# luigifreda/plvs

Measured on AMD Instinct MI355X. Metric: Mvoxels/sec TSDF integrate (chisel 5 cm / 5 m, 640x480 RGB-D), higher is better.
Workload: dtype f32; 1 GPU; configs[2] stand-in, STREAMING: see DESIGN.md 4.1 / 4.6; mode=order-free (fixed-point sums; sdf / weight within tolerance), longest_voxel_run=25008, parallelism=chunk-hash shard x1

## Files before the change

include/plvs_hip.h:

```cpp
#ifndef PLVS_HIP_H_
#define PLVS_HIP_H_

#include <stddef.h>
#include <stdint.h>

#ifdef __cplusplus
extern "C" {
#endif

#define PLVS_OK 0
#define PLVS_ERR_INVALID_ARG (-1)
#define PLVS_ERR_HIP (-2)
#define PLVS_ERR_NO_DEVICE (-3)
#define PLVS_ERR_CAPACITY (-4)
#define PLVS_ERR_EMPTY (-5)
#define PLVS_ERR_HALO (-6)
#define PLVS_ERR_COMM_FATAL (-7)

const char* plvs_hip_last_error(void);
int plvs_hip_abi_version(void);
int plvs_hip_device_count(int* count);
int plvs_hip_set_device(int device);
int plvs_hip_synchronize(void);
int plvs_hip_release_thread_buffers(void);
// ... 227 lines not shown
  float dist[8];
  int32_t ndist;
  float mbf;
  float bounds4[4];
  float grid_w_inv, grid_h_inv;
  float min_line_length_3d;
  int32_t use_median_depth;
  float median_fallback;
} plvs_rgbd_calib;
typedef struct plvs_rgbd_frame {
  int32_t kp_cap, line_cap;
  plvs_keypoint* kps;
  plvs_keypoint* kps_un;
  uint8_t* desc;
  float* u_right;
  float* depth;
  int32_t* cell_start;
  int32_t* cell_items;
  plvs_keyline* keylines;
  plvs_keyline* keylines_un;
  uint8_t* line_desc;
  float* u_right_start;
  float* depth_start;
  float* u_right_end;
  float* depth_end;
  int32_t n_kp, mono_index, n_lines, n_items;
  float median_depth;
} plvs_rgbd_frame;
int plvs_hip_frame_rgbd_dev(plvs_orb* orb, plvs_lines* lines, const uint8_t* d_image, int w, int hh, int stride, const float* d_depth,
                            int depth_pitch, const plvs_rgbd_calib* calib, plvs_rgbd_frame* frame, void* stream);

int plvs_hip_frame_compute_stereo_line_matches(const plvs_keyline* keylines_un, const uint8_t* desc, int n,
                                               const plvs_keyline* keylines_right_un, const uint8_t* desc_right, int n_right,
                                               const float* line_level_sigma2, int n_levels, const float* K4, float mbf,
                                               float line_stereo_max_dist, float min_line_length_3d, float nn_ratio,
                                               int check_orientation, int descriptor_dist, float* u_right_start, float* depth_start,
                                               float* u_right_end, float* depth_end, int* n_stereo, void* stream);
int plvs_hip_frame_compute_stereo_line_matches_debug(const plvs_keyline* keylines_un, const uint8_t* desc, int n,
                                                     const plvs_keyline* keylines_right_un, const uint8_t* desc_right, int n_right,
                                                     const float* line_level_sigma2, int n_levels, const float* K4, float mbf,
                                                     float line_stereo_max_dist, float min_line_length_3d, float nn_ratio,
                                                     int check_orientation, int descriptor_dist, float* u_right_start,
                                                     float* depth_start, float* u_right_end, float* depth_end, int* n_stereo,
                                                     int32_t* holders4, void* stream);

struct plvs_stereo;
typedef struct plvs_stereo_calib {
  float K4[4];
  float dist[8];
  int32_t ndist;
  float mbf;
  float bounds4[4];
  float grid_w_inv, grid_h_inv;
  float min_line_length_3d;
  float line_stereo_max_dist;
  float nn_ratio;
  int32_t check_orientation;
  int32_t descriptor_dist;
  int32_t n_line_levels;
  const float* line_level_sigma2;
} plvs_stereo_calib;
typedef struct plvs_stereo_frame {
  int32_t kp_cap, kp_right_cap, line_cap, line_right_cap;
  plvs_keypoint* kps;
  plvs_keypoint* kps_un;
  uint8_t* desc;
  float* u_right;
  float* depth;
  int32_t* cell_start;
  int32_t* cell_items;
  plvs_keypoint* kps_right;
  uint8_t* desc_right;
  plvs_keyline* keylines;
  plvs_keyline* keylines_un;
  uint8_t* line_desc;
  float* u_right_start;
  float* depth_start;
  float* u_right_end;
  float* depth_end;
  plvs_keyline* keylines_right;
  plvs_keyline* keylines_right_un;
  uint8_t* line_desc_right;
  int32_t n_kp, mono_index, n_kp_right, mono_index_right, n_lines, n_lines_right, n_items;
  int32_t n_stereo_points, n_stereo_lines;
} plvs_stereo_frame;
int plvs_hip_frame_stereo_dev(plvs_orb* orb_left, plvs_orb* orb_right, plvs_lines* lines_left, plvs_lines* lines_right,
                              struct plvs_stereo* stereo, const uint8_t* d_left, const uint8_t* d_right, int w, int hh, int stride,
                              const plvs_stereo_calib* calib, plvs_stereo_frame* frame, void* stream);

int plvs_hip_selftest_rcp(int exponent, uint32_t* mismatches);
int plvs_hip_selftest_walk_math(uint32_t seed, uint32_t* mismatches_sqrt_div);
int plvs_hip_selftest_radix_sort(uint32_t n, int bit_lo, int bit_hi, int wide_values, uint32_t seed, uint32_t* mismatches2);

typedef struct plvs_tsdf_chisel_params {
  float resolution;
  float trunc_quad;
  float trunc_linear;
  float trunc_const;
  float trunc_scale;
  float weight;
  int32_t max_chunks;
  int32_t shard_rank;
  int32_t shard_count;
  int32_t order_free;
} plvs_tsdf_chisel_params;

typedef struct plvs_tsdf_chisel plvs_tsdf_chisel;

int plvs_hip_tsdf_chisel_default_params(float resolution, plvs_tsdf_chisel_params* p);
int plvs_hip_tsdf_chisel_create(const plvs_tsdf_chisel_params* p, plvs_tsdf_chisel** out);
int plvs_hip_tsdf_chisel_destroy(plvs_tsdf_chisel* h);
int plvs_hip_tsdf_chisel_clear(plvs_tsdf_chisel* h);

int plvs_hip_tsdf_chisel_integrate(plvs_tsdf_chisel* h, const float* xyz, const uint8_t* rgb,
                                   const uint32_t* kfid, int n, const float* Twc);

int plvs_hip_tsdf_chisel_queue(plvs_tsdf_chisel* h, const float* xyz, const uint8_t* rgb, const uint32_t* kfid, int n,
                               const float* Twc);
int plvs_hip_tsdf_chisel_flush(plvs_tsdf_chisel* h);
int plvs_hip_tsdf_chisel_queued(plvs_tsdf_chisel* h, int* nclouds);
int plvs_hip_tsdf_chisel_integrate_batch_dev(plvs_tsdf_chisel* h, const float* d_xyz,
                                             const uint8_t* d_rgb, const uint32_t* d_kfid,
                                             const int32_t* offsets, int nclouds,
                                             const float* d_Twc, void* stream);

typedef struct plvs_depth_batch {
  const float* d_depth;
  const uint8_t* d_bgr;
  size_t depth_image_stride, bgr_image_stride;
  int depth_pitch, bgr_pitch;
  int width, height, step;
  const float* d_grid_points;
  double min_depth, max_depth;
  const uint32_t* d_kfid;
} plvs_depth_batch;
int plvs_hip_tsdf_chisel_integrate_depth_batch_dev(plvs_tsdf_chisel* h, const plvs_depth_batch* in, int nclouds,
                                                   const float* d_Twc, void* stream);

int plvs_hip_tsdf_chisel_integrate_world_normals(plvs_tsdf_chisel* h, const float* xyz, const uint8_t* rgb,
                                                 const uint32_t* kfid, const float* normals, int n, const float* Twc);
int plvs_hip_tsdf_chisel_integrate_world_normals_dev(plvs_tsdf_chisel* h, const float* d_xyz, const uint8_t* d_rgb,
                                                     const uint32_t* d_kfid, const float* d_normals, int n,
                                                     const float* d_Twc, void* stream);

typedef struct plvs_tsdf_stats {
  int64_t visits;
  int64_t points;
  int32_t new_chunks;
  int32_t updated_chunks;
  int32_t voxels;
  int32_t max_run;
} plvs_tsdf_stats;
int plvs_hip_tsdf_chisel_last_stats(plvs_tsdf_chisel* h, plvs_tsdf_stats* s);

int plvs_hip_tsdf_chisel_set_apply_parts(plvs_tsdf_chisel* h, int part_segments, int min_segments);

int plvs_hip_tsdf_chisel_set_profiling(plvs_tsdf_chisel* h, int enable);
int plvs_hip_tsdf_chisel_stage_ms(plvs_tsdf_chisel* h, double* ms, int cap, int* nstages,
                                  int64_t* calls);
const char* plvs_hip_tsdf_chisel_stage_name(int i);
const char* plvs_hip_tsdf_chisel_stage_name_of(plvs_tsdf_chisel* h, int i);

int plvs_hip_tsdf_chisel_num_chunks(plvs_tsdf_chisel* h, int* n);
int plvs_hip_tsdf_chisel_chunk_ids(plvs_tsdf_chisel* h, int32_t* ids_xyz, int cap, int* n);
int plvs_hip_tsdf_chisel_updated_chunk_ids(plvs_tsdf_chisel* h, int32_t* ids_xyz, int cap, int* n);
int plvs_hip_tsdf_chisel_updated_chunk_ids_dev(plvs_tsdf_chisel* h, int32_t* d_ids_xyz, int cap,
                                               int* n, void* stream);
int plvs_hip_tsdf_chisel_download_chunk(plvs_tsdf_chisel* h, int cx, int cy, int cz, float* sdf,
                                        float* weight, uint32_t* kfid, uint32_t* rgbw);

int plvs_hip_tsdf_chisel_carve(plvs_tsdf_chisel* h, const float* depth, int width, int height, float fx,
                               float fy, float cx, float cy, float near_dist, float far_dist,
                               const float* Twc, float carving_dist, int* carved_chunks);
int plvs_hip_tsdf_chisel_carve_dev(plvs_tsdf_chisel* h, const float* d_depth, int width, int height,
                                   float fx, float fy, float cx, float cy, float near_dist,
                                   float far_dist, const float* Twc, float carving_dist, void* stream,
                                   int* carved_chunks);

int plvs_hip_tsdf_chisel_shard_walk(plvs_tsdf_chisel* h, const float* d_xyz, const int32_t* offsets, int nclouds,
                                    const float* d_Twc, int64_t* send_counts, void* stream);
int plvs_hip_tsdf_chisel_shard_pack(plvs_tsdf_chisel* h, void* d_seg_dst, void* d_rec_dst, void* d_run_dst,
                                    void* stream);
int plvs_hip_tsdf_chisel_shard_apply(plvs_tsdf_chisel* h, const void* d_seg_src, const void* d_rec_src,
                                     const void* d_run_src, const int64_t* recv_counts, const uint8_t* d_rgb,
                                     const uint32_t* d_kfid, void* stream);
int plvs_hip_tsdf_chisel_shard_saturated(plvs_tsdf_chisel* h, int32_t* d_voxels, int cap, int* n, void* stream);
int plvs_hip_tsdf_chisel_shard_note_saturated(plvs_tsdf_chisel* h, const int32_t* d_voxels, int n, void* stream);
int plvs_hip_tsdf_chisel_shard_saturated_message(plvs_tsdf_chisel* h, int32_t* d_msg, int rows, void* stream);
int plvs_hip_tsdf_chisel_shard_note_gathered(plvs_tsdf_chisel* h, const int32_t* d_gathered, int nranks, int rows,
                                             void* stream);
int plvs_hip_tsdf_chisel_integrate_sharded(plvs_tsdf_chisel* h, void* rccl_comm, const float* d_xyz,
                                           const uint8_t* d_rgb, const uint32_t* d_kfid, const int32_t* offsets,
                                           int nclouds, const float* d_Twc, void* stream);
int plvs_hip_exchange_abort_on_fatal(int enable);

int plvs_hip_tsdf_exchange_block_lists(void* rccl_comm, const int32_t* d_local_ids, int local_count, int cap,
                                       int32_t* d_all_ids, int32_t* d_all_counts, void* stream);
int plvs_hip_rccl_world_size(void* rccl_comm, int* world);
typedef struct plvs_block_directory plvs_block_directory;
int plvs_hip_block_directory_create(int max_blocks, plvs_block_directory** out);
int plvs_hip_block_directory_destroy(plvs_block_directory* d);
int plvs_hip_block_directory_merge(plvs_block_directory* d, const int32_t* d_all_ids, const int32_t* d_counts, int world,
                                   int cap, void* stream);
int plvs_hip_block_directory_count(plvs_block_directory* d, int* n);
int plvs_hip_block_directory_list(plvs_block_directory* d, int32_t* ids_xyz, int32_t* owners, int cap, int* n);

typedef struct plvs_stereo plvs_stereo;
int plvs_hip_stereo_create(plvs_orb* left, plvs_orb* right, plvs_stereo** out);
int plvs_hip_stereo_destroy(plvs_stereo* s);
int plvs_hip_stereo_matches(plvs_stereo* s, const plvs_keypoint* keys_left, const uint8_t* desc_left,
                            int n_left, const plvs_keypoint* keys_right, const uint8_t* desc_right,
                            int n_right, float mb, float mbf, float* u_right, float* depth,
                            int* n_matched);

int plvs_hip_tsdf_chisel_mesh_chunks(plvs_tsdf_chisel* h, const int32_t* chunk_ids_xyz, int nchunks,
                                     float* vertices, float* normals, float* colors, uint32_t* kfids,
                                     int capacity, int32_t* chunk_first, int* nvertices);

typedef struct plvs_tsdf_deform_stats {
  int32_t new_chunks;
  int64_t moved;
  int64_t discarded;
  int64_t undefined;
} plvs_tsdf_deform_stats;
int plvs_hip_tsdf_chisel_enable_deform(plvs_tsdf_chisel* h);
int plvs_hip_tsdf_chisel_deform(plvs_tsdf_chisel* h, const uint32_t* kfids, const float* Rt, int n_map,
                                plvs_tsdf_deform_stats* stats);
int plvs_hip_tsdf_chisel_chunk_order(plvs_tsdf_chisel* h, int32_t* ids_xyz, int cap, int* n);
int plvs_hip_tsdf_chisel_deform_mesh(float* vertices, float* normals, const uint32_t* vertex_kfid, int n,
                                     const uint32_t* kfids, const float* Rt, int n_map);
int plvs_hip_tsdf_chisel_deform_mesh_dev(float* d_vertices, float* d_normals, const uint32_t* d_vertex_kfid, int n,
                                         const uint32_t* d_kfids, const float* d_Rt, int n_map, void* stream);

int plvs_hip_tsdf_chisel_upload_chunk(plvs_tsdf_chisel* h, int cx, int cy, int cz, const float* sdf, const float* weight,
                                      const uint32_t* kfid, const uint32_t* rgbw);

int plvs_hip_tsdf_chisel_mesh_probe(plvs_tsdf_chisel* h, const int32_t* chunk_ids_xyz, int nchunks, int* nmissing);
int plvs_hip_tsdf_chisel_halo_gather(plvs_tsdf_chisel* h, void* rccl_comm, const int32_t* chunk_ids_xyz, int nchunks,
                                     int* fetched, void* stream);
int plvs_hip_tsdf_chisel_halo_missing(plvs_tsdf_chisel* h, int32_t* ids_xyz, int cap, int* n);
int plvs_hip_tsdf_chisel_halo_lookup(plvs_tsdf_chisel* h, const int32_t* d_ids_xyz, int n, uint32_t* d_found, void* stream);
int plvs_hip_tsdf_chisel_halo_export(plvs_tsdf_chisel* h, const int32_t* d_ids_xyz, const uint32_t* d_found, int n,
                                     uint32_t* d_payload, void* stream);
int plvs_hip_tsdf_chisel_halo_import(plvs_tsdf_chisel* h, const int32_t* d_ids_xyz, const uint32_t* d_found,
                                     const uint32_t* d_payload, int n, int nfound, void* stream);
int plvs_hip_tsdf_chisel_halo_clear(plvs_tsdf_chisel* h);

typedef struct plvs_elas plvs_elas;
typedef struct {
  int32_t subsampling;
  int32_t grid_size;
  int32_t match_texture;
  float beta;
  float gamma;
  float sigma;
  float sradius;
  int32_t disp_min, disp_max;
  int32_t candidate_stepsize;
  int32_t support_texture;
  int32_t lr_threshold;
  float support_threshold;
  float speckle_sim_threshold;
  int32_t speckle_size;
  int32_t ipol_gap_width;
  int32_t add_corners;
} plvs_elas_params;
int plvs_hip_elas_create(const plvs_elas_params* params, plvs_elas** out);
int plvs_hip_elas_destroy(plvs_elas* e);
int plvs_hip_elas_compute_disparity(plvs_elas* e, const int32_t* support, int n_support, const void* tri, int n_tri,
                                    const int32_t* disparity_grid, const int32_t* grid_dims, const uint8_t* I1_desc,
                                    const uint8_t* I2_desc, int width, int height, int right_image, float* D);
int plvs_hip_elas_adaptive_mean(plvs_elas* e, float* D, int width, int height);
int plvs_hip_elas_support_candidates(plvs_elas* e, const uint8_t* I1_desc, const uint8_t* I2_desc, int width, int height,
                                     int16_t* D_can);
int plvs_hip_elas_set_images(plvs_elas* e, const uint8_t* I1, const uint8_t* I2, int width, int height, int stride);
int plvs_hip_elas_download_descriptors(plvs_elas* e, uint8_t* I1_desc, uint8_t* I2_desc);
int plvs_hip_elas_left_right_check(plvs_elas* e, float* D1, float* D2, int width, int height);
int plvs_hip_elas_remove_small_segments(plvs_elas* e, float* D, int width, int height);
int plvs_hip_elas_gap_interpolation(plvs_elas* e, float* D, int width, int height);
int plvs_hip_elas_postprocess(plvs_elas* e, int width, int height, int postprocess_only_left, int filter_adaptive_mean,
                              float* D1, float* D2);
int plvs_hip_elas_depth_dev(plvs_elas* e, float bf, int step, float* d_depth, int width, int height, void* stream);
int plvs_hip_elas_triangulate(const int32_t* support, int n_support, int right_image, void* tri, int cap, int* n_tri);
int plvs_hip_elas_process(plvs_elas* e, const uint8_t* I1, const uint8_t* I2, const int32_t* dims, int postprocess_only_left,
                          int filter_adaptive_mean, float* D1, float* D2);
int plvs_hip_elas_support_points(plvs_elas* e, const int16_t* D_can, int width, int height, int32_t* support, int cap,
                                 int* n_support);
int plvs_hip_elas_disparity_planes(plvs_elas* e, const int32_t* support, int n_support, void* tri, int n_tri);
int plvs_hip_elas_create_grid(plvs_elas* e, const int32_t* support, int n_support, int width, int height, int right_image,
                              int32_t* disparity_grid, int32_t* grid_dims);

typedef struct plvs_sgm plvs_sgm;
int plvs_hip_sgm_create(int width, int height, int disparity_size, int p1, int p2, float uniqueness,
                        plvs_sgm** out);
int plvs_hip_sgm_destroy(plvs_sgm* s);
int plvs_hip_sgm_execute(plvs_sgm* s, const uint8_t* left, const uint8_t* right, uint8_t* disparity);
int plvs_hip_sgm_execute_dev(plvs_sgm* s, const uint8_t* d_left, const uint8_t* d_right,
                             uint8_t* d_disparity, void* stream);
int plvs_hip_sgm_download(plvs_sgm* s, int which, void* out);


typedef struct plvs_point_surfel {
  float x, y, z;
  uint32_t kfid;
  float normal_x, normal_y, normal_z, normal_pad;
  uint8_t b, g, r, a;
// ... 273 lines not shown
```

plvs_amd/csrc/tsdf_chisel.hip:

```cpp
#include "tsdf_chisel_handle.hpp"
#include "tsdf_chisel_halo.hpp"
#include "tsdf_chisel_ordered.hpp"
#include "tsdf_chisel_order_free.hpp"
#include "tsdf_chisel_carve.hpp"
#include "tsdf_chisel_shard.hpp"
#include "tsdf_chisel_deform.hpp"
#include "tsdf_chisel_scan.hpp"

namespace {

__global__ void pool_init(float* __restrict__ sdf, size_t n) {
  const size_t i = (size_t)blockIdx.x * blockDim.x + threadIdx.x;
  const size_t stride = (size_t)gridDim.x * blockDim.x;
  for (size_t j = i; j < n; j += stride) sdf[j] = 99999.0f;
}

__global__ void selftest_sort_fill(uint32_t* __restrict__ keys, uint32_t* __restrict__ v32, unsigned long long* __restrict__ v64,
                                   uint32_t n, int bits, uint32_t seed) {
  const uint32_t i = blockIdx.x * blockDim.x + threadIdx.x;
  if (i >= n) return;
  uint32_t x = (i + 1u) * 2654435761u + seed;
  x ^= x << 13; x ^= x >> 17; x ^= x << 5;
  x ^= x << 13; x ^= x >> 17; x ^= x << 5;
  keys[i] = bits >= 32 ? x : (x & ((1u << bits) - 1u));
  if (v32) v32[i] = i;
  if (v64) v64[i] = ((unsigned long long)~i << 32) | i;
}
__global__ void selftest_sort_check(const uint32_t* __restrict__ keys_in, const uint32_t* __restrict__ keys,
                                    const uint32_t* __restrict__ v32, const unsigned long long* __restrict__ v64, uint32_t n,
                                    int bit_lo, int bit_hi, uint32_t* __restrict__ mismatches) {
  const uint32_t i = blockIdx.x * blockDim.x + threadIdx.x;
  if (i >= n) return;
  const uint32_t mask = (bit_hi - bit_lo >= 32 ? 0xFFFFFFFFu : ((1u << (bit_hi - bit_lo)) - 1u)) << bit_lo;
  const uint32_t pos = v32 ? v32[i] : (uint32_t)v64[i];
  if (pos >= n || keys_in[pos] != keys[i] || (v64 && (uint32_t)(v64[i] >> 32) != ~pos)) atomicAdd(&mismatches[1], 1u);
  if (i + 1 < n) {
    const uint32_t a = keys[i] & mask, b = keys[i + 1] & mask;
    const uint32_t pn = v32 ? v32[i + 1] : (uint32_t)v64[i + 1];
    if (a > b || (a == b && pos >= pn)) atomicAdd(&mismatches[0], 1u);
  }
}

__global__ void selftest_rcp_kernel(int exponent, uint32_t* __restrict__ mismatches) {
  const uint32_t m = blockIdx.x * blockDim.x + threadIdx.x;
  const float b = __uint_as_float(((uint32_t)(exponent + 127) << 23) | m);
  if (__float_as_uint(rcp_rn(b)) != __float_as_uint(1.0f / b)) atomicAdd(mismatches, 1u);
}

}

__global__ __launch_bounds__(256) void grid_cloud_mark(GridSrc g, int nclouds, uint32_t* __restrict__ flag) {
  const size_t i = (size_t)blockIdx.x * 256 + threadIdx.x, ngrid = (size_t)g.gw * g.gh;
  if (i >= ngrid * (size_t)nclouds) return;
  const uint32_t c = (uint32_t)(i / ngrid), r = (uint32_t)(i - (size_t)c * ngrid), m = r / g.gw, n = r - m * g.gw;
  const float d = g.depth[(size_t)c * g.image_stride + (size_t)(m * g.step) * g.pitch + n * g.step];
  flag[i] = (((double)d > g.min_depth) && ((double)d < g.max_depth)) ? 1u : 0u;
}
__global__ __launch_bounds__(256) void grid_cloud_emit(GridSrc g, int nclouds, const uint32_t* __restrict__ pos ,
                                                       const uint8_t* __restrict__ bgr, const uint32_t* __restrict__ kfid_of_image,
                                                       float* __restrict__ xyz, uint8_t* __restrict__ rgb,
                                                       uint32_t* __restrict__ kfid, uint32_t* __restrict__ offsets) {
  const size_t i = (size_t)blockIdx.x * 256 + threadIdx.x, ngrid = (size_t)g.gw * g.gh, cells = ngrid * (size_t)nclouds;
  if (i > cells) return;
  if (i == cells || i % ngrid == 0) offsets[i / ngrid] = pos[i];
  if (i == cells || pos[i + 1] == pos[i]) return;
  const uint32_t c = (uint32_t)(i / ngrid), r = (uint32_t)(i - (size_t)c * ngrid), m = r / g.gw, n = r - m * g.gw;
  const float d = g.depth[(size_t)c * g.image_stride + (size_t)(m * g.step) * g.pitch + n * g.step];
  const float2 cam = reinterpret_cast<const float2*>(g.cam)[r];
  const size_t o = pos[i];
  xyz[3 * o] = cam.x * d;
  xyz[3 * o + 1] = cam.y * d;
  xyz[3 * o + 2] = d;
  const uint8_t* px = bgr + (size_t)c * g.bgr_image_stride + (size_t)(m * g.step) * g.bgr_pitch + (size_t)(n * g.step) * 3u;
  rgb[3 * o] = px[0];
  rgb[3 * o + 1] = px[1];
  rgb[3 * o + 2] = px[2];
  kfid[o] = kfid_of_image ? kfid_of_image[c] : 0u;
}

extern "C" {

int plvs_hip_selftest_rcp(int exponent, uint32_t* mismatches) {
  PLVS_REQUIRE(mismatches && exponent > -126 && exponent < 127, "bad argument");
  uint32_t* d = nullptr;
  PLVS_HIP_TRY(hipMalloc((void**)&d, sizeof(uint32_t)));
  PLVS_HIP_TRY(hipMemset(d, 0, sizeof(uint32_t)));
  hipLaunchKernelGGL(selftest_rcp_kernel, dim3((1u << 23) / 256), dim3(256), 0, nullptr, exponent, d);
  hipError_t e = hipMemcpy(mismatches, d, sizeof(uint32_t), hipMemcpyDeviceToHost);
  (void)hipFree(d);
  PLVS_HIP_TRY(e);
  return PLVS_OK;
}

int plvs_hip_selftest_radix_sort(uint32_t n, int bit_lo, int bit_hi, int wide_values, uint32_t seed, uint32_t* mismatches2) {
  PLVS_REQUIRE(mismatches2 && n > 0 && bit_lo >= 0 && bit_hi > bit_lo && bit_hi <= 32, "bad argument");
  plvs::DevBuf<uint32_t> k_in, k0, k1, v0, v1, scratch, bad;
  plvs::DevBuf<unsigned long long> w0, w1;
  const bool bound_mode = wide_values == 2;
  if (bound_mode) wide_values = 0;
  const uint32_t n_alloc = bound_mode ? n + n / 2 + 4097u : n;
  PLVS_HIP_TRY(k_in.reserve(n_alloc));
  PLVS_HIP_TRY(k0.reserve(n_alloc));
  PLVS_HIP_TRY(k1.reserve(n_alloc));
  if (wide_values) {
    PLVS_HIP_TRY(w0.reserve(n));
    PLVS_HIP_TRY(w1.reserve(n));
  } else {
    PLVS_HIP_TRY(v0.reserve(n_alloc));
    PLVS_HIP_TRY(v1.reserve(n_alloc));
  }
  PLVS_HIP_TRY(scratch.reserve(radix_scratch_words(n_alloc) + 1));
  PLVS_HIP_TRY(bad.reserve(2));
  PLVS_HIP_TRY(hipMemset(bad.p, 0, 2 * sizeof(uint32_t)));
  const dim3 grid(ceil_div((size_t)n, 256)), block(256);
  hipLaunchKernelGGL(selftest_sort_fill, grid, block, 0, nullptr, k0.p, v0.p, w0.p, n, bit_hi, seed);
  PLVS_HIP_TRY(hipMemcpyAsync(k_in.p, k0.p, (size_t)n * sizeof(uint32_t), hipMemcpyDeviceToDevice, nullptr));
  bool second = false;
  if (bound_mode) {
    PLVS_HIP_TRY(hipMemsetAsync(k0.p + n, 0x5A, (size_t)(n_alloc - n) * sizeof(uint32_t), nullptr));
    uint32_t* d_n = scratch.p + radix_scratch_words(n_alloc);
    PLVS_HIP_TRY(hipMemcpyAsync(d_n, &n, sizeof(uint32_t), hipMemcpyHostToDevice, nullptr));
    PLVS_HIP_TRY(hipStreamSynchronize(nullptr));
    PLVS_HIP_TRY(radix_sort_pairs_bound(k0.p, v0.p, k1.p, v1.p, n_alloc, d_n, bit_lo, bit_hi, scratch.p, nullptr, &second));
  } else if (wide_values) PLVS_HIP_TRY(radix_sort_pairs_u64(k0.p, w0.p, k1.p, w1.p, n, bit_lo, bit_hi, scratch.p, nullptr, &second));
  else PLVS_HIP_TRY(radix_sort_pairs(k0.p, v0.p, k1.p, v1.p, n, bit_lo, bit_hi, scratch.p, nullptr, &second));
  hipLaunchKernelGGL(selftest_sort_check, grid, block, 0, nullptr, k_in.p, second ? k1.p : k0.p,
                     wide_values ? (const uint32_t*)nullptr : (second ? v1.p : v0.p),
                     wide_values ? (second ? w1.p : w0.p) : (const unsigned long long*)nullptr, n, bit_lo, bit_hi, bad.p);
  hipError_t e = hipMemcpy(mismatches2, bad.p, 2 * sizeof(uint32_t), hipMemcpyDeviceToHost);
  k_in.release(); k0.release(); k1.release(); v0.release(); v1.release(); w0.release(); w1.release(); scratch.release(); bad.release();
  PLVS_HIP_TRY(e);
  return PLVS_OK;
}

#ifdef PLVS_WALK_PROF
int plvs_hip_debug_walk_prof(unsigned long long* out16, int reset) {
  if (out16) PLVS_HIP_TRY(hipMemcpyFromSymbol(out16, HIP_SYMBOL(g_walk_prof), 16 * sizeof(unsigned long long)));
  if (reset) {
    unsigned long long z[16] = {};
    PLVS_HIP_TRY(hipMemcpyToSymbol(HIP_SYMBOL(g_walk_prof), z, sizeof z));
  }
  return PLVS_OK;
}
#endif

int plvs_hip_selftest_walk_math(uint32_t seed, uint32_t* mismatches_sqrt_div) {
  PLVS_REQUIRE(mismatches_sqrt_div, "null argument");
  uint32_t* d = nullptr;
  PLVS_HIP_TRY(hipMalloc((void**)&d, 2 * sizeof(uint32_t)));
  PLVS_HIP_TRY(hipMemset(d, 0, 2 * sizeof(uint32_t)));
  hipLaunchKernelGGL(selftest_walk_math_kernel, dim3(16384), dim3(256), 0, nullptr, seed, d);
  hipError_t e = hipMemcpy(mismatches_sqrt_div, d, 2 * sizeof(uint32_t), hipMemcpyDeviceToHost);
  (void)hipFree(d);
  PLVS_HIP_TRY(e);
  return PLVS_OK;
}

int plvs_hip_tsdf_chisel_default_params(float resolution, plvs_tsdf_chisel_params* p) {
  PLVS_REQUIRE(p, "params is null");
  PLVS_REQUIRE(resolution > 0.0f, "resolution must be positive");
  p->resolution = resolution;
  p->trunc_quad = 0.0019f;
  p->trunc_linear = -0.00152f;
  p->trunc_const = 0.001504f;
  p->trunc_scale = 6.0f;
  p->weight = 1.0f;
  p->max_chunks = 32768;
  p->shard_rank = 0;
  p->shard_count = 1;
  p->order_free = 0;
  return PLVS_OK;
}

int plvs_hip_tsdf_chisel_create(const plvs_tsdf_chisel_params* p, plvs_tsdf_chisel** out) {
  PLVS_REQUIRE(p && out, "null argument");
  PLVS_REQUIRE(p->resolution > 0.0f, "resolution must be positive");
  PLVS_REQUIRE(p->max_chunks > 0 && p->max_chunks <= (1 << 20), "max_chunks must be in (0, 2^20]");
  PLVS_REQUIRE(p->shard_count <= 1 || (p->shard_rank >= 0 && p->shard_rank < p->shard_count),
               "shard_rank out of range");
  plvs_tsdf_chisel* h = new plvs_tsdf_chisel();
  h->prm = *p;
  Params& P = h->P;
  P.resolution = p->resolution;
  P.round_to_voxel = 1.0f / p->resolution;
  P.half_voxel = p->resolution * 0.5f;
  P.rounding = 1.0f / ((float)16 * p->resolution);
  P.diag = (float)(2.0 * std::sqrt((double)3.0f) * (double)p->resolution);
  P.tq = p->trunc_quad; P.tl = p->trunc_linear; P.tc = p->trunc_const; P.ts = p->trunc_scale;
  P.weight = p->weight;
  P.shard_rank = p->shard_rank;
  P.shard_count = p->shard_count < 1 ? 1 : p->shard_count;

  uint32_t cap = 1024;
  while (cap < 2u * (uint32_t)p->max_chunks) cap <<= 1;
  h->dir.mask = cap - 1;
  h->dir.max_blocks = p->max_chunks;
  const size_t nvox = (size_t)p->max_chunks * kChunkVox;
#define CREATE_TRY(call)                                                        \
  do {                                                                          \
    hipError_t _e = (call);                                                     \
    if (_e != hipSuccess) {                                                     \
      plvs::set_error("%s failed: %s", #call, hipGetErrorString(_e));          \
      plvs_hip_tsdf_chisel_destroy(h);                                          \
      return PLVS_ERR_HIP;                                                      \
    }                                                                           \
  } while (0)
  CREATE_TRY(hipMalloc((void**)&h->dir.keys, (size_t)cap * sizeof(unsigned long long)));
  CREATE_TRY(hipMalloc((void**)&h->dir.slots, (size_t)cap * sizeof(int32_t)));
  CREATE_TRY(hipMalloc((void**)&h->dir.slot_ids, (size_t)p->max_chunks * 3 * sizeof(int32_t)));
  CREATE_TRY(hipMalloc((void**)&h->sdf, nvox * sizeof(float)));
  CREATE_TRY(hipMalloc((void**)&h->weight, nvox * sizeof(float)));
  CREATE_TRY(hipMalloc((void**)&h->kfid, nvox * sizeof(uint32_t)));
  CREATE_TRY(hipMalloc((void**)&h->rgbw, nvox * sizeof(uint32_t)));
  CREATE_TRY(hipMalloc((void**)&h->d_ctr, sizeof(Counters)));
  CREATE_TRY(hipHostMalloc((void**)&h->h_ctr, sizeof(Counters), hipHostMallocCoherent));
  CREATE_TRY(hipMalloc((void**)&h->d_wctr, 2 * sizeof(WalkCounters)));
  CREATE_TRY(hipHostMalloc((void**)&h->h_wctr, 2 * sizeof(WalkCounters), hipHostMallocCoherent));
  CREATE_TRY(hipHostMalloc((void**)&h->h_seq, 64, hipHostMallocCoherent));
  h->h_seq[0] = 0u;
  {
    const double wu_max = (double)p->weight / (2.0 * (double)P.diag), wuu_max = 0.5 * (double)p->weight;
    h->scale_u = (float)std::exp2(std::floor(std::log2(1073741824.0 / (kWalkRays * wuu_max))));
    h->scale_w = (float)std::exp2(std::floor(std::log2(1073741824.0 / (kWalkRays * wu_max))));
  }
  {
    int least = 0, greatest = 0;
    CREATE_TRY(hipDeviceGetStreamPriorityRange(&least, &greatest));
    CREATE_TRY(hipStreamCreateWithPriority(&h->side, hipStreamNonBlocking, greatest));
  }
  CREATE_TRY(hipEventCreateWithFlags(&h->ev_fork, hipEventDisableTiming));
  CREATE_TRY(hipEventCreateWithFlags(&h->ev_join, hipEventDisableTiming));
  CREATE_TRY(hipEventCreateWithFlags(&h->ev_seg, hipEventDisableTiming));
  CREATE_TRY(hipEventCreateWithFlags(&h->ev_zero, hipEventDisableTiming));
#undef CREATE_TRY
  *out = h;
  int rc = plvs_hip_tsdf_chisel_clear(h);
  if (rc != PLVS_OK) {
    plvs_hip_tsdf_chisel_destroy(h);
    *out = nullptr;
  }
  return rc;
}

int plvs_hip_tsdf_chisel_destroy(plvs_tsdf_chisel* h) {
  if (!h) return PLVS_OK;
  if (h->ext != nullptr && h->ext_free != nullptr) h->ext_free(h->ext);
  deform_state_free(h);
  (void)hipFree(h->dir.keys);
  (void)hipFree(h->dir.slots);
  (void)hipFree(h->dir.slot_ids);
  (void)hipFree(h->sdf);
  (void)hipFree(h->weight);
  (void)hipFree(h->kfid);
  (void)hipFree(h->rgbw);
  (void)hipFree(h->d_ctr);
  if (h->h_ctr) (void)hipHostFree(h->h_ctr);
  (void)hipFree(h->d_wctr);
  if (h->h_wctr) (void)hipHostFree(h->h_wctr);
  if (h->h_seq) (void)hipHostFree(h->h_seq);
  if (h->h_offsets) (void)hipHostFree(h->h_offsets);
  (void)hipFree(h->gdir.keys);
  (void)hipFree(h->gdir.slots);
  (void)hipFree(h->miss_keys);
  (void)hipFree(h->miss_ids);
  (void)hipFree(h->miss_count);
  (void)hipFree(h->xdir.keys);
  (void)hipFree(h->xdir.slots);
  (void)hipFree(h->xdir.slot_ids);
  (void)hipFree(h->d_xcount);
  (void)hipFree(h->x_sat);
  if (h->h_sh_counts) (void)hipHostFree(h->h_sh_counts);
  if (h->h_sh_ctl) (void)hipHostFree(h->h_sh_ctl);
  if (h->h_sh_off) (void)hipHostFree(h->h_sh_off);
  h->q_xyz.release(); h->q_rgb.release(); h->q_kfid.release();
  h->w_rec.release(); h->w_seg.release(); h->w_sorted_seg.release(); h->w_seg_ticket.release(); h->w_chunk_nseg.release();
  h->w_chunk_off.release(); h->w_chunk_fill.release(); h->w_active_off.release(); h->w_masks.release();
  h->w_dummy.release(); h->w_runkey.release(); h->w_run_cnt.release(); h->w_run_off.release(); h->w_val0.release();
  h->w_val1.release(); h->w_seg_cnt.release(); h->w_tile_visits.release(); h->w_deferred.release(); h->w_part_off.release(); h->w_multi_idx.release();
  h->pa_wuu.release(); h->pa_w.release(); h->pa_last.release(); h->pa_cnt.release(); h->pa_done.release();
  h->sh_nrec.release(); h->sh_owner.release(); h->halo_row.release();
  h->sh_ctl.release(); h->sh_seg_reg.release(); h->sh_rec_reg.release(); h->sh_src_off.release(); h->sh_slot_owner.release(); h->sh_run_ctr.release(); h->sh_vkey.release(); h->sh_sat.release(); h->sh_wait.release(); h->sh_run_first.release();
  if (h->ev_fork) (void)hipEventDestroy(h->ev_fork);
  if (h->ev_join) (void)hipEventDestroy(h->ev_join);
  if (h->ev_seg) (void)hipEventDestroy(h->ev_seg);
  if (h->ev_zero) (void)hipEventDestroy(h->ev_zero);
  h->w_rseg.release(); h->w_rpre.release(); h->w_run_matrix.release(); h->w_active_idx.release(); h->w_item_base.release();
  h->w_item_cnt.release(); h->w_item_part0.release(); h->w_part_item.release(); h->w_phist.release();
  h->w_row_heads.release(); h->w_row_tot.release();
  if (h->side) (void)hipStreamDestroy(h->side);
  for (int i = 0; i <= kNumStages; ++i)
    if (h->ev[i]) (void)hipEventDestroy(h->ev[i]);
  h->counts.release();
  h->rec.release(); h->rec_t.release(); h->recc_t.release();
  h->dkey0.release(); h->dkey1.release(); h->didx0.release(); h->didx1.release();
  h->last_pt.release(); h->run_cnt.release(); h->run_dst.release();
  h->tile_first.release(); h->block_first.release(); h->tile_state.release();
  h->heads.release(); h->updated.release(); h->scratch.release(); h->poses.release();
  h->offsets.release(); h->st_xyz.release(); h->st_Twc.release(); h->st_nrm.release(); h->st_rgb.release();
  h->st_kfid.release();
  h->st_pos.release(); h->st_scan.release(); h->st_off.release();
  delete h;
  return PLVS_OK;
}

int plvs_hip_tsdf_chisel_clear(plvs_tsdf_chisel* h) {
  if (h) {
    h->q_offsets.clear();
    h->q_Twc.clear();
  }
  PLVS_REQUIRE(h, "null handle");
  {
    int rc = halo_drop(h, nullptr);
    if (rc != PLVS_OK) return rc;
  }
  {
    int rc = shard_state_clear(h);
    if (rc != PLVS_OK) return rc;
  }
  const size_t cap = (size_t)h->dir.mask + 1;
  const size_t nvox = (size_t)h->prm.max_chunks * kChunkVox;
  PLVS_HIP_TRY(hipMemset(h->dir.keys, 0xFF, cap * sizeof(unsigned long long)));
  PLVS_HIP_TRY(hipMemset(h->dir.slots, 0xFF, cap * sizeof(int32_t)));
  PLVS_HIP_TRY(hipMemset(h->weight, 0, nvox * sizeof(float)));
  PLVS_HIP_TRY(hipMemset(h->kfid, 0, nvox * sizeof(uint32_t)));
  PLVS_HIP_TRY(hipMemset(h->rgbw, 0, nvox * sizeof(uint32_t)));
  PLVS_HIP_TRY(hipMemset(h->d_ctr, 0, sizeof(Counters)));
  hipLaunchKernelGGL(pool_init, dim3(2048), dim3(256), 0, nullptr, h->sdf, nvox);
  PLVS_KERNEL_CHECK();
  PLVS_HIP_TRY(hipDeviceSynchronize());
  h->num_chunks = 0;
  h->walk.small_runs_known = false;
  h->poisoned = false;
  h->stats = plvs_tsdf_stats{};
  h->last_updated = 0;
  deform_state_clear(h);
  return PLVS_OK;
}

}

static int integrate_batch_core(plvs_tsdf_chisel* h, const float* d_xyz, const uint8_t* d_rgb, const uint32_t* d_kfid,
                                const int32_t* offsets, int nclouds, const float* d_Twc, void* stream,
                                const float* d_normals) {
  PLVS_REQUIRE(h, "null handle");
  PLVS_REQUIRE(!h->poisoned, "handle is in a failed state (clear it)");
  PLVS_REQUIRE(offsets && nclouds >= 0, "bad offsets");
  hipStream_t s = static_cast<hipStream_t>(stream);
  h->stats = plvs_tsdf_stats{};
  h->last_updated = 0;
  int n = 0;
  int rc = check_offsets(offsets, nclouds, &n);
  if (rc != PLVS_OK || nclouds == 0) return rc;
  h->stats.points = n;
  if (n == 0) return PLVS_OK;
  PLVS_REQUIRE(d_xyz && d_rgb && d_Twc, "null device pointer");
  if ((rc = halo_drop(h, s)) != PLVS_OK) return rc;
  PLVS_HIP_TRY(h->offsets.reserve(2 * ((size_t)nclouds + 1)));
  PLVS_HIP_TRY(h->poses.reserve((size_t)nclouds));
  if (h->prm.order_free != 0 && d_normals == nullptr) return integrate_walk_acc(h, d_xyz, d_rgb, d_kfid, n, nclouds, offsets, d_Twc, s);
  return integrate_ordered(h, d_xyz, d_rgb, d_kfid, n, nclouds, offsets, d_Twc, s, d_normals);
}

static int integrate_batch_impl(plvs_tsdf_chisel* h, const float* d_xyz, const uint8_t* d_rgb, const uint32_t* d_kfid,
                                const int32_t* offsets, int nclouds, const float* d_Twc, void* stream,
                                const float* d_normals) {
  PLVS_REQUIRE(h, "null handle");
  const bool track = h->dfm != nullptr && !h->poisoned && offsets && nclouds >= 1 && offsets[nclouds] - offsets[0] > 0 && d_xyz &&
                     d_Twc;
  if (track) {
    int rc = halo_drop(h, static_cast<hipStream_t>(stream));
    if (rc == PLVS_OK) rc = deform_track_begin(h, d_xyz, d_normals, offsets[nclouds] - offsets[0], nclouds, d_Twc, static_cast<hipStream_t>(stream));
    if (rc != PLVS_OK) return rc;
  }
  int rc = integrate_batch_core(h, d_xyz, d_rgb, d_kfid, offsets, nclouds, d_Twc, stream, d_normals);
  if (track && rc == PLVS_OK) rc = deform_track_end(h, static_cast<hipStream_t>(stream));
  return rc;
}

extern "C" {

int plvs_hip_tsdf_chisel_integrate_batch_dev(plvs_tsdf_chisel* h, const float* d_xyz,
                                             const uint8_t* d_rgb, const uint32_t* d_kfid,
                                             const int32_t* offsets, int nclouds,
                                             const float* d_Twc, void* stream) {
  PLVS_FLUSH_QUEUE(h);
  return integrate_batch_impl(h, d_xyz, d_rgb, d_kfid, offsets, nclouds, d_Twc, stream, nullptr);
}

int plvs_hip_tsdf_chisel_integrate_depth_batch_dev(plvs_tsdf_chisel* h, const plvs_depth_batch* in, int nclouds,
                                                   const float* d_Twc, void* stream) {
  PLVS_FLUSH_QUEUE(h);
  PLVS_REQUIRE(h && in, "null argument");
  PLVS_REQUIRE(!h->poisoned, "handle is in a failed state (clear it)");
  PLVS_REQUIRE(nclouds >= 0, "bad image count");
  h->stats = plvs_tsdf_stats{};
  h->last_updated = 0;
  if (nclouds == 0) return PLVS_OK;
  PLVS_REQUIRE(in->d_depth && in->d_bgr && in->d_grid_points && d_Twc, "null device pointer");
  PLVS_REQUIRE(in->width > 0 && in->height > 0 && in->step > 0, "image size / step");
  PLVS_REQUIRE(in->depth_pitch >= in->width && in->bgr_pitch >= 3 * in->width, "row pitch smaller than a row");
  PLVS_REQUIRE(in->depth_image_stride >= (size_t)in->depth_pitch * (size_t)(in->height - 1) + (size_t)in->width &&
               in->bgr_image_stride >= (size_t)in->bgr_pitch * (size_t)(in->height - 1) + 3 * (size_t)in->width,
               "image stride smaller than an image");
  hipStream_t s = static_cast<hipStream_t>(stream);
  GridSrc g{};
  g.depth = in->d_depth;
  g.cam = in->d_grid_points;
  g.image_stride = in->depth_image_stride;
  g.pitch = (uint32_t)in->depth_pitch;
  g.step = (uint32_t)in->step;
  g.gw = (uint32_t)((in->width + in->step - 1) / in->step);
  g.gh = (uint32_t)((in->height + in->step - 1) / in->step);
  g.ntx = (g.gw + kGridTileW - 1) / kGridTileW;
  g.nty = (g.gh + kGridTileH - 1) / kGridTileH;
  g.inv_ntx = 1.0f / (float)g.ntx;
  g.inv_nty = 1.0f / (float)g.nty;
  g.key_bits = 1;
  while ((1ull << g.key_bits) < (unsigned long long)g.gw * g.gh) ++g.key_bits;
  g.min_depth = in->min_depth;
  g.max_depth = in->max_depth;
  g.bgr_image_stride = in->bgr_image_stride;
  g.bgr_pitch = (uint32_t)in->bgr_pitch;
  PLVS_REQUIRE(g.key_bits < 31 && (unsigned long long)nclouds <= (1ull << (32 - g.key_bits)),
               "too many images in one call for the order keys (split the batch)");
  const size_t ngrid = (size_t)g.gw * g.gh;
  h->stats.points = 0;
  {
    int rc = halo_drop(h, s);
    if (rc != PLVS_OK) return rc;
  }
  const bool walk2d = h->prm.order_free != 0 && std::max(1, h->prm.shard_count) == 1 && h->dfm == nullptr;
  if (walk2d) {
    std::vector<int32_t> zeros((size_t)nclouds + 1, 0);
    PLVS_HIP_TRY(h->offsets.reserve(2 * ((size_t)nclouds + 1)));
    PLVS_HIP_TRY(h->poses.reserve((size_t)nclouds));
    return integrate_walk_acc(h, nullptr, in->d_bgr, in->d_kfid, 0, nclouds, zeros.data(), d_Twc, s, &g);
  }
  const size_t cells = ngrid * (size_t)nclouds;
  PLVS_REQUIRE(cells < 0x7FFFFFFFull, "too many grid pixels in one call (split the batch)");
  plvs::DevBuf<uint32_t>&pos = h->st_pos, &scan_scratch = h->st_scan, &d_off = h->st_off;
  PLVS_HIP_TRY(pos.reserve(cells + 1));
// ... 54 lines not shown
int plvs_hip_tsdf_chisel_queue(plvs_tsdf_chisel* h, const float* xyz, const uint8_t* rgb, const uint32_t* kfid, int n,
                               const float* Twc) {
  PLVS_REQUIRE(h, "null handle");
  PLVS_REQUIRE(n >= 0 && Twc, "bad arguments");
  if (n == 0) return PLVS_OK;
  PLVS_REQUIRE(xyz && rgb, "null cloud pointer");
  const bool first = h->q_offsets.empty();
  PLVS_REQUIRE(first || h->q_kfid_given == (kfid != nullptr), "queued clouds must all carry key-frame ids, or none");
  const size_t at = first ? 0 : (size_t)h->q_offsets.back();
  PLVS_REQUIRE(at + (size_t)n < 0x7FFFFFFFull, "too many queued points");
  PLVS_HIP_TRY(grow_keep(h->q_xyz, 3 * at, 3 * (at + (size_t)n)));
  PLVS_HIP_TRY(grow_keep(h->q_rgb, 3 * at, 3 * (at + (size_t)n)));
  PLVS_HIP_TRY(hipMemcpy(h->q_xyz.p + 3 * at, xyz, (size_t)n * 3 * sizeof(float), hipMemcpyHostToDevice));
  PLVS_HIP_TRY(hipMemcpy(h->q_rgb.p + 3 * at, rgb, (size_t)n * 3, hipMemcpyHostToDevice));
  if (kfid) {
    PLVS_HIP_TRY(grow_keep(h->q_kfid, at, at + (size_t)n));
    PLVS_HIP_TRY(hipMemcpy(h->q_kfid.p + at, kfid, (size_t)n * sizeof(uint32_t), hipMemcpyHostToDevice));
  }
  if (first) h->q_offsets.push_back(0);
  h->q_kfid_given = kfid != nullptr;
  h->q_offsets.push_back((int32_t)(at + (size_t)n));
  h->q_Twc.insert(h->q_Twc.end(), Twc, Twc + 12);
  return PLVS_OK;
}

int plvs_hip_tsdf_chisel_queued(plvs_tsdf_chisel* h, int* nclouds) {
  PLVS_REQUIRE(h && nclouds, "null argument");
  *nclouds = h->q_offsets.empty() ? 0 : (int)h->q_offsets.size() - 1;
  return PLVS_OK;
}

int plvs_hip_tsdf_chisel_flush(plvs_tsdf_chisel* h) {
  PLVS_REQUIRE(h, "null handle");
  if (h->q_offsets.empty()) return PLVS_OK;
  const int nclouds = (int)h->q_offsets.size() - 1;
  std::vector<int32_t> offsets;
  std::vector<float> Twc;
  offsets.swap(h->q_offsets);
  Twc.swap(h->q_Twc);
  PLVS_HIP_TRY(h->st_Twc.reserve((size_t)12 * nclouds));
  PLVS_HIP_TRY(hipMemcpy(h->st_Twc.p, Twc.data(), (size_t)12 * nclouds * sizeof(float), hipMemcpyHostToDevice));
  int rc = plvs_hip_tsdf_chisel_integrate_batch_dev(h, h->q_xyz.p, h->q_rgb.p, h->q_kfid_given ? h->q_kfid.p : nullptr,
                                                    offsets.data(), nclouds, h->st_Twc.p, nullptr);
  if (rc != PLVS_OK) {
    char own[400];
    snprintf(own, sizeof own, "%s", plvs::last_error_buf());
    plvs::set_error("%s — raised by the flush of %d queued key-frame cloud%s (plvs_hip_tsdf_chisel_queue): NONE of them was "
                    "integrated and they are dropped; queue them again after clearing / enlarging the map", own, nclouds,
                    nclouds == 1 ? "" : "s");
    return rc;
  }
  PLVS_HIP_TRY(hipDeviceSynchronize());
  return PLVS_OK;
}
int plvs_hip_tsdf_chisel_integrate(plvs_tsdf_chisel* h, const float* xyz, const uint8_t* rgb,
                                   const uint32_t* kfid, int n, const float* Twc) {
  PLVS_REQUIRE(h, "null handle");
  PLVS_REQUIRE(n >= 0 && Twc, "bad arguments");
  PLVS_FLUSH_QUEUE(h);
  if (n == 0) {
    h->stats = plvs_tsdf_stats{};
    h->last_updated = 0;
    return PLVS_OK;
  }
  PLVS_REQUIRE(xyz && rgb, "null cloud pointer");
  PLVS_HIP_TRY(h->st_xyz.reserve((size_t)n * 3));
  PLVS_HIP_TRY(h->st_rgb.reserve((size_t)n * 3));
  PLVS_HIP_TRY(h->st_Twc.reserve(12));
  PLVS_HIP_TRY(hipMemcpy(h->st_xyz.p, xyz, (size_t)n * 3 * sizeof(float), hipMemcpyHostToDevice));
  PLVS_HIP_TRY(hipMemcpy(h->st_rgb.p, rgb, (size_t)n * 3, hipMemcpyHostToDevice));
  PLVS_HIP_TRY(hipMemcpy(h->st_Twc.p, Twc, 12 * sizeof(float), hipMemcpyHostToDevice));
  const uint32_t* dk = nullptr;
  if (kfid) {
    PLVS_HIP_TRY(h->st_kfid.reserve((size_t)n));
    PLVS_HIP_TRY(hipMemcpy(h->st_kfid.p, kfid, (size_t)n * sizeof(uint32_t), hipMemcpyHostToDevice));
    dk = h->st_kfid.p;
  }
  const int32_t offsets[2] = {0, n};
  int rc = plvs_hip_tsdf_chisel_integrate_batch_dev(h, h->st_xyz.p, h->st_rgb.p, dk, offsets, 1,
                                                    h->st_Twc.p, nullptr);
  if (rc != PLVS_OK) return rc;
  PLVS_HIP_TRY(hipDeviceSynchronize());
  return PLVS_OK;
}

int plvs_hip_tsdf_chisel_set_apply_parts(plvs_tsdf_chisel* h, int part_segments, int min_segments) {
  PLVS_REQUIRE(h && part_segments >= 1 && min_segments >= 1, "bad argument");
  h->part_segs = (uint32_t)part_segments;
  h->part_min = (uint32_t)min_segments;
  return PLVS_OK;
}

int plvs_hip_tsdf_chisel_set_profiling(plvs_tsdf_chisel* h, int enable) {
  PLVS_REQUIRE(h, "null handle");
  if (enable && !h->ev[0])
    for (int i = 0; i <= kNumStages; ++i) PLVS_HIP_TRY(hipEventCreate(&h->ev[i]));
  h->profiling = enable != 0;
  for (int i = 0; i < kNumStages; ++i) h->stage_ms[i] = 0.0;
  h->prof_calls = 0;
  return PLVS_OK;
}

int plvs_hip_tsdf_chisel_stage_ms(plvs_tsdf_chisel* h, double* ms, int cap, int* nstages,
                                  int64_t* calls) {
  PLVS_REQUIRE(h && nstages, "null argument");
  *nstages = h->stage_set == 1 ? kWalkStages : kNumStages;
  if (calls) *calls = h->prof_calls;
  for (int i = 0; i < kNumStages && i < cap; ++i) ms[i] = h->stage_ms[i];
  return PLVS_OK;
}

const char* plvs_hip_tsdf_chisel_stage_name(int i) {
  return (i >= 0 && i < kNumStages) ? kStageNames[i] : "";
}

const char* plvs_hip_tsdf_chisel_stage_name_of(plvs_tsdf_chisel* h, int i) {
  if (h == nullptr || i < 0) return "";
  if (h->stage_set == 1) return i < kWalkStages ? kWalkStageNames[i] : "";
  return i < kNumStages ? kStageNames[i] : "";
}

__global__ void gather_slot_ids(const uint32_t* __restrict__ slots, int n,
                                const int32_t* __restrict__ slot_ids, int32_t* __restrict__ out) {
  const int i = blockIdx.x * blockDim.x + threadIdx.x;
  if (i < n) {
    const uint32_t s = slots[i];
    out[3 * i] = slot_ids[3 * s];
    out[3 * i + 1] = slot_ids[3 * s + 1];
    out[3 * i + 2] = slot_ids[3 * s + 2];
  }
}

int plvs_hip_tsdf_chisel_updated_chunk_ids_dev(plvs_tsdf_chisel* h, int32_t* d_ids_xyz, int cap,
                                               int* n, void* stream) {
  PLVS_FLUSH_QUEUE(h);
  PLVS_REQUIRE(h && n, "null argument");
  *n = (int)h->last_updated;
  const int m = (int)h->last_updated < cap ? (int)h->last_updated : cap;
  if (m <= 0) return PLVS_OK;
  PLVS_REQUIRE(d_ids_xyz, "null output");
  hipLaunchKernelGGL(gather_slot_ids, dim3(ceil_div((size_t)m, 256)), dim3(256), 0,
                     static_cast<hipStream_t>(stream), h->updated.p, m, h->dir.slot_ids, d_ids_xyz);
  PLVS_KERNEL_CHECK();
  return PLVS_OK;
}

int plvs_hip_tsdf_chisel_last_stats(plvs_tsdf_chisel* h, plvs_tsdf_stats* s) {
  PLVS_FLUSH_QUEUE(h);
  PLVS_REQUIRE(h && s, "null argument");
  *s = h->stats;
  return PLVS_OK;
}

int plvs_hip_tsdf_chisel_num_chunks(plvs_tsdf_chisel* h, int* n) {
  PLVS_FLUSH_QUEUE(h);
  PLVS_REQUIRE(h && n, "null argument");
  *n = h->num_chunks;
  return PLVS_OK;
}

int plvs_hip_tsdf_chisel_chunk_ids(plvs_tsdf_chisel* h, int32_t* ids_xyz, int cap, int* n) {
  PLVS_FLUSH_QUEUE(h);
  PLVS_REQUIRE(h && n, "null argument");
  *n = h->num_chunks;
  const int m = h->num_chunks < cap ? h->num_chunks : cap;
  if (m > 0) {
    PLVS_REQUIRE(ids_xyz, "null output");
    PLVS_HIP_TRY(hipMemcpy(ids_xyz, h->dir.slot_ids, (size_t)m * 3 * sizeof(int32_t),
                           hipMemcpyDeviceToHost));
  }
  return PLVS_OK;
}

int plvs_hip_tsdf_chisel_updated_chunk_ids(plvs_tsdf_chisel* h, int32_t* ids_xyz, int cap, int* n) {
  PLVS_FLUSH_QUEUE(h);
  PLVS_REQUIRE(h && n, "null argument");
  *n = (int)h->last_updated;
  const int m = (int)h->last_updated < cap ? (int)h->last_updated : cap;
  if (m <= 0) return PLVS_OK;
  PLVS_REQUIRE(ids_xyz, "null output");
  uint32_t* slots = new uint32_t[h->last_updated];
  int32_t* all = new int32_t[(size_t)h->num_chunks * 3];
  hipError_t e1 = hipMemcpy(slots, h->updated.p, (size_t)h->last_updated * sizeof(uint32_t),
                            hipMemcpyDeviceToHost);
  hipError_t e2 = hipMemcpy(all, h->dir.slot_ids, (size_t)h->num_chunks * 3 * sizeof(int32_t),
                            hipMemcpyDeviceToHost);
  if (e1 == hipSuccess && e2 == hipSuccess)
    for (int i = 0; i < m; ++i) memcpy(ids_xyz + 3 * i, all + 3 * (size_t)slots[i], 3 * sizeof(int32_t));
  delete[] slots;
  delete[] all;
  PLVS_HIP_TRY(e1);
  PLVS_HIP_TRY(e2);
  return PLVS_OK;
}

int plvs_hip_tsdf_chisel_download_chunk(plvs_tsdf_chisel* h, int cx, int cy, int cz, float* sdf,
                                        float* weight, uint32_t* kfid, uint32_t* rgbw) {
  PLVS_FLUSH_QUEUE(h);
  PLVS_REQUIRE(h && sdf && weight && kfid && rgbw, "null argument");
  int32_t* all = new int32_t[(size_t)(h->num_chunks > 0 ? h->num_chunks : 1) * 3];
  hipError_t e = hipSuccess;
  if (h->num_chunks > 0)
    e = hipMemcpy(all, h->dir.slot_ids, (size_t)h->num_chunks * 3 * sizeof(int32_t),
                  hipMemcpyDeviceToHost);
  int slot = -1;
  if (e == hipSuccess)
    for (int i = 0; i < h->num_chunks; ++i)
      if (all[3 * i] == cx && all[3 * i + 1] == cy && all[3 * i + 2] == cz) { slot = i; break; }
  delete[] all;
  PLVS_HIP_TRY(e);
  if (slot < 0) {
    plvs::set_error("chunk (%d,%d,%d) does not exist", cx, cy, cz);
    return PLVS_ERR_INVALID_ARG;
  }
  const size_t off = (size_t)slot * kChunkVox;
  PLVS_HIP_TRY(hipMemcpy(sdf, h->sdf + off, kChunkVox * sizeof(float), hipMemcpyDeviceToHost));
  PLVS_HIP_TRY(hipMemcpy(weight, h->weight + off, kChunkVox * sizeof(float), hipMemcpyDeviceToHost));
  PLVS_HIP_TRY(hipMemcpy(kfid, h->kfid + off, kChunkVox * sizeof(uint32_t), hipMemcpyDeviceToHost));
  PLVS_HIP_TRY(hipMemcpy(rgbw, h->rgbw + off, kChunkVox * sizeof(uint32_t), hipMemcpyDeviceToHost));
  return PLVS_OK;
}

}

namespace plvs {
namespace tsdf {

bool chisel_map_view(plvs_tsdf_chisel* h, ChiselMapView* v) {
  if (h == nullptr || v == nullptr || h->poisoned) return false;
  v->resolution = h->P.resolution;
  v->dir = h->dir;
  v->sdf = h->sdf;
  v->weight = h->weight;
  v->kfid = h->kfid;
  v->rgbw = h->rgbw;
  v->num_chunks = h->num_chunks;
  v->shard_count = h->P.shard_count;
  v->shard_rank = h->P.shard_rank;
  v->ext = &h->ext;
  v->ext_free = &h->ext_free;
  if (h->P.shard_count > 1) {
    if (h->miss_keys == nullptr) {
      const size_t want = std::max<size_t>(std::min<size_t>((size_t)h->prm.max_chunks * (size_t)h->P.shard_count, (size_t)1 << 22),
                                           (size_t)1 << 18);
      size_t cap = 1024;
      while (cap < 2 * want) cap <<= 1;
      if (hipMalloc(&h->miss_keys, cap * sizeof(unsigned long long)) != hipSuccess) return false;
      if (hipMalloc(&h->miss_ids, want * 3 * sizeof(int32_t)) != hipSuccess) return false;
      if (hipMalloc(&h->miss_count, sizeof(uint32_t)) != hipSuccess) return false;
      h->miss_cap = (uint32_t)want;
      h->miss_mask = (uint32_t)(cap - 1);
    }
    if (hipMemsetAsync(h->miss_keys, 0xFF, ((size_t)h->miss_mask + 1) * sizeof(unsigned long long), nullptr) != hipSuccess) return false;
    if (hipMemsetAsync(h->miss_count, 0, sizeof(uint32_t), nullptr) != hipSuccess) return false;
    v->ghost = h->gdir;
    v->miss_keys = h->miss_keys;
    v->miss_mask = h->miss_mask;
    v->miss_ids = h->miss_ids;
    v->miss_count = h->miss_count;
    v->miss_cap = h->miss_cap;
  }
  return true;
}

}
}

__global__ void chunk_slot_of(Directory dir, int x, int y, int z, int32_t* __restrict__ num_chunks, uint32_t* __restrict__ err,
                              int32_t* __restrict__ slot_out) {
  if (threadIdx.x == 0 && blockIdx.x == 0) *slot_out = dir_find_or_insert(dir, x, y, z, num_chunks, err);
}

extern "C" {

int plvs_hip_tsdf_chisel_upload_chunk(plvs_tsdf_chisel* h, int cx, int cy, int cz, const float* sdf, const float* weight,
                                      const uint32_t* kfid, const uint32_t* rgbw) {
  PLVS_FLUSH_QUEUE(h);
  PLVS_REQUIRE(h && sdf && weight && kfid && rgbw, "null argument");
  PLVS_REQUIRE(!h->poisoned, "handle is in a failed state (clear it)");
  if (std::max(1, h->prm.shard_count) > 1)
    PLVS_REQUIRE(shard_of(chunk_hash(cx, cy, cz), h->prm.shard_count) == h->prm.shard_rank, "the chunk belongs to another rank");
  int rc = halo_drop(h, nullptr);
  if (rc != PLVS_OK) return rc;
  PLVS_HIP_TRY(hipMemset(&h->d_ctr->err, 0, sizeof(uint32_t)));
  int32_t* d_slot = reinterpret_cast<int32_t*>(&h->d_ctr->total_visits);
  hipLaunchKernelGGL(chunk_slot_of, dim3(1), dim3(64), 0, nullptr, h->dir, cx, cy, cz, &h->d_ctr->num_chunks, &h->d_ctr->err,
                     d_slot);
  PLVS_KERNEL_CHECK();
  rc = read_counters(h, nullptr);
  if (rc != PLVS_OK) return rc;
  if (h->h_ctr->err) {
    h->poisoned = true;
    plvs::set_error("upload_chunk: %s", (h->h_ctr->err & kErrPoolFull) ? "chunk pool full (raise max_chunks)" : "chunk id out of range");
    return PLVS_ERR_CAPACITY;
  }
  const int slot = (int)h->h_ctr->total_visits;
  h->num_chunks = h->h_ctr->num_chunks;
  if (h->dfm) deform_note_created(h, cx, cy, cz);
  const size_t off = (size_t)slot * kChunkVox;
  PLVS_HIP_TRY(hipMemcpy(h->sdf + off, sdf, kChunkVox * sizeof(float), hipMemcpyHostToDevice));
  PLVS_HIP_TRY(hipMemcpy(h->weight + off, weight, kChunkVox * sizeof(float), hipMemcpyHostToDevice));
  PLVS_HIP_TRY(hipMemcpy(h->kfid + off, kfid, kChunkVox * sizeof(uint32_t), hipMemcpyHostToDevice));
  PLVS_HIP_TRY(hipMemcpy(h->rgbw + off, rgbw, kChunkVox * sizeof(uint32_t), hipMemcpyHostToDevice));
  return PLVS_OK;
}

// ... 2 lines not shown
```

plvs_amd/csrc/tsdf_chisel_handle.hpp:

```cpp
#pragma once
#include <vector>

#include "common.hpp"
#include "device_utils.hpp"
#include "tsdf_chisel_core.hpp"
#include "tsdf_directory.hpp"
#include "tsdf_chisel_view.hpp"
#include "tsdf_walk.hpp"
#include "tsdf_walk_plan.hpp"

using namespace plvs;
using namespace plvs::chisel;
using namespace plvs::tsdf;

namespace {

constexpr int kNumStages = 6;
const char* const kStageNames[kNumStages] = {"ray_count", "scan", "ray_tiles", "sort_runs",
                                             "gather_runs", "chain_runs"};
constexpr int kWalkStages = 4;
const char* const kWalkStageNames[kWalkStages] = {"walk_tiles", "sort_segments", "apply_chunks", "fold_colours"};

struct Counters {
  uint32_t total_visits;
  int32_t num_chunks;
  uint32_t err;
  uint32_t num_heads;
  uint32_t num_updated;
  uint32_t max_run;
  uint32_t num_desc;
};

__global__ void pose_prep(const float* __restrict__ Twc, int nclouds, Pose* __restrict__ poses) {
  const int c = blockIdx.x * blockDim.x + threadIdx.x;
  if (c < nclouds) make_pose(Twc + 12 * c, &poses[c]);
}

__global__ void publish_counters(const WalkCounters* __restrict__ wctr, const Counters* __restrict__ ctr,
                                 WalkCounters* __restrict__ host_wctr, Counters* __restrict__ host_ctr,
                                 uint32_t* __restrict__ host_seq = nullptr, uint32_t seq = 0u) {
  if (wctr) {
    const uint32_t* a = reinterpret_cast<const uint32_t*>(wctr);
    uint32_t* b = reinterpret_cast<uint32_t*>(host_wctr);
    for (int k = threadIdx.x; k < (int)(2 * sizeof(WalkCounters) / sizeof(uint32_t)); k += blockDim.x) b[k] = a[k];
  }
  if (ctr) {
    const uint32_t* c = reinterpret_cast<const uint32_t*>(ctr);
    uint32_t* d = reinterpret_cast<uint32_t*>(host_ctr);
    for (int k = threadIdx.x; k < (int)(sizeof(Counters) / sizeof(uint32_t)); k += blockDim.x) d[k] = c[k];
  }
  __threadfence_system();
  if (host_seq != nullptr) {
    __syncthreads();
    if (threadIdx.x == 0) __hip_atomic_store(host_seq, seq, __ATOMIC_RELEASE, __HIP_MEMORY_SCOPE_SYSTEM);
  }
}

__global__ void publish_words(const uint32_t* __restrict__ a, uint32_t* __restrict__ ha, int na, const uint32_t* __restrict__ b,
                              uint32_t* __restrict__ hb, int nb, const uint32_t* __restrict__ c, uint32_t* __restrict__ hc, int nc) {
  for (int k = threadIdx.x; k < na; k += blockDim.x) ha[k] = a[k];
  for (int k = threadIdx.x; k < nb; k += blockDim.x) hb[k] = b[k];
  for (int k = threadIdx.x; k < nc; k += blockDim.x) hc[k] = c[k];
  __threadfence_system();
}

}

struct ChiselDeformState;

struct plvs_tsdf_chisel {
  plvs_tsdf_chisel_params prm;
  Params P;
  Directory dir;
  float* sdf = nullptr;
  float* weight = nullptr;
  uint32_t* kfid = nullptr;
  uint32_t* rgbw = nullptr;
  Counters* d_ctr = nullptr;
  Counters* h_ctr = nullptr;
  int num_chunks = 0;
  bool poisoned = false;
  DevBuf<uint32_t> counts, heads, updated, scratch;
  DevBuf<float2> rec, rec_t;
  DevBuf<uint32_t> recc_t;
  DevBuf<uint32_t> dkey0, dkey1, run_cnt, run_dst, last_pt;
  DevBuf<unsigned long long> didx0, didx1;
  DevBuf<uint32_t> tile_first, block_first;
  DevBuf<unsigned long long> tile_state;
  DevBuf<Pose> poses;
  ChiselDeformState* dfm = nullptr;
  void* ext = nullptr;
  void (*ext_free)(void*) = nullptr;
  Directory gdir{};
  int ghost_count = 0;
  long long ghost_entries = 0;
  DevBuf<uint32_t> halo_row;
  unsigned long long* miss_keys = nullptr;
  int32_t* miss_ids = nullptr;
  uint32_t* miss_count = nullptr;
  uint32_t miss_cap = 0, miss_mask = 0;
  DevBuf<int32_t> offsets;
  DevBuf<float> st_xyz, st_Twc, st_nrm;
  DevBuf<uint8_t> st_rgb;
  DevBuf<uint32_t> st_kfid;
  DevBuf<uint32_t> st_pos, st_scan, st_off;
  plvs_tsdf_stats stats{};
  uint32_t last_updated = 0;
  DevBuf<float> q_xyz;
  DevBuf<uint8_t> q_rgb;
  DevBuf<uint32_t> q_kfid;
  std::vector<int32_t> q_offsets;
  std::vector<float> q_Twc;
  bool q_kfid_given = false;
  WalkCounters* d_wctr = nullptr;
  WalkCounters* h_wctr = nullptr;
  uint32_t* h_seq = nullptr;
  uint32_t seq_next = 0;
  double wait_ema_us[3][3] = {{0.0, 0.0, 0.0}, {0.0, 0.0, 0.0}, {0.0, 0.0, 0.0}};
  DevBuf<uint4> w_rec, w_seg, w_sorted_seg;
  DevBuf<uint32_t> w_seg_ticket;
  DevBuf<uint4> w_rseg, w_rpre;
  DevBuf<uint32_t> w_run_matrix, w_active_idx, w_item_base, w_item_cnt, w_item_part0, w_part_item, w_phist, w_row_heads, w_row_tot;
  hipEvent_t ev_zero = nullptr;
  hipEvent_t ev_seg = nullptr;
  int last_chain = 0;
  bool last_chain_skipped = false;
  DevBuf<uint32_t> w_chunk_nseg, w_chunk_off, w_chunk_fill, w_active_off, w_masks, w_dummy, w_seg_cnt, w_tile_visits, w_deferred;
  DevBuf<uint32_t> w_part_off, w_multi_idx;
  DevBuf<long long> pa_wuu;
  DevBuf<unsigned long long> pa_w;
  DevBuf<uint32_t> pa_last, pa_cnt, pa_done;
  uint32_t multi_cap = 0;
  uint32_t part_segs = kPartSegs, part_min = kPartMin;
  plvs::tsdf::WalkHistory walk;
  DevBuf<uint32_t> w_runkey, w_run_cnt, w_run_off, w_val0, w_val1;
  int32_t* h_offsets = nullptr;
  size_t h_offsets_cap = 0;
  uint32_t run_r1_log2 = 11;
  float scale_u = 1.f, scale_w = 1.f;
  int stage_set = 0;
  Directory xdir{};
  int32_t* d_xcount = nullptr;
  uint32_t* x_sat = nullptr;
  DevBuf<uint32_t> sh_ctl;
  uint32_t* h_sh_ctl = nullptr;
  uint32_t* h_sh_off = nullptr;
  DevBuf<uint4> sh_seg_reg, sh_rec_reg;
  DevBuf<uint32_t> sh_nrec, sh_owner, sh_slot_owner, sh_src_off, sh_run_ctr, sh_vkey, sh_sat;
  DevBuf<uint4> sh_run_first;
  uint32_t sh_nt = 0, sh_runs = 0, sh_nsat = 0;
  DevBuf<int32_t> sh_wait;
  uint32_t sh_wait_first = 0, sh_wait_count = 0;
  long long* h_sh_counts = nullptr;
  int sh_n = 0, sh_nclouds = 0;
  uint32_t sh_ntiles = 0;
  std::vector<int32_t> sh_tiletab;
  int sh_phase = 0;
  plvs_tsdf_stats sh_stats{};
  hipStream_t side = nullptr;
  hipEvent_t ev_fork = nullptr, ev_join = nullptr;
  bool profiling = false;
  hipEvent_t ev[kNumStages + 1] = {};
  double stage_ms[kNumStages] = {};
  int64_t prof_calls = 0;
};

extern "C" int plvs_hip_tsdf_chisel_flush(plvs_tsdf_chisel* h);
#define PLVS_FLUSH_QUEUE(h)                                        \
  do {                                                             \
    if ((h) && !(h)->q_offsets.empty()) {                          \
      const int rc_flush_ = plvs_hip_tsdf_chisel_flush(h);         \
      if (rc_flush_ != PLVS_OK) return rc_flush_;                  \
    }                                                              \
  } while (0)


static int read_counters(plvs_tsdf_chisel* h, hipStream_t s) {
  hipLaunchKernelGGL(publish_counters, dim3(1), dim3(64), 0, s, (const WalkCounters*)nullptr, h->d_ctr, (WalkCounters*)nullptr,
                     h->h_ctr);
  PLVS_KERNEL_CHECK();
  PLVS_HIP_TRY(hipStreamSynchronize(s));
  return PLVS_OK;
}

static inline void cpu_relax() {
#if defined(__x86_64__) || defined(__i386__)
  __builtin_ia32_pause();
#elif defined(__aarch64__) || defined(__arm__)
  __asm__ __volatile__("yield");
#endif
}

static int wait_published(plvs_tsdf_chisel* h, uint32_t seq, hipStream_t q, int kind = 0, int size_class = 0) {
  double& ema = h->wait_ema_us[kind][size_class];
  static const int spin_us = plvs::env_int("PLVS_TSDF_SPIN_US", 400, 0, 10000000);
  if (spin_us > 0 && h->h_seq != nullptr) {
    const volatile uint32_t* const word = h->h_seq;
    timespec t0, t1;
    clock_gettime(CLOCK_MONOTONIC, &t0);
    auto elapsed_us = [&]() {
      clock_gettime(CLOCK_MONOTONIC, &t1);
      return (double)(t1.tv_sec - t0.tv_sec) * 1e6 + (double)(t1.tv_nsec - t0.tv_nsec) * 1e-3;
    };
    bool done = *word == seq;
    if (!done && ema > 200.0) {
      timespec nap;
      const double us = std::min(std::min(ema - 120.0, 0.7 * ema), 5000.0);
      nap.tv_sec = 0;
      nap.tv_nsec = (long)(us * 1e3);
      nanosleep(&nap, nullptr);
      done = *word == seq;
    }
    const double spin_from = done ? 0.0 : elapsed_us();
    for (uint32_t spins = 0; !done; ++spins) {
      done = *word == seq;
      if (done) break;
      cpu_relax();
      if ((spins & 255u) == 255u && elapsed_us() - spin_from > (double)spin_us) break;
    }
    if (done) {
      __atomic_thread_fence(__ATOMIC_ACQUIRE);
      ema = 0.75 * ema + 0.25 * elapsed_us();
      return PLVS_OK;
    }
    ema = 0.75 * ema + 0.25 * (elapsed_us() + 200.0);
  }
  PLVS_HIP_TRY(hipStreamSynchronize(q));
  return PLVS_OK;
}

static int read_walk_counters(plvs_tsdf_chisel* h, hipStream_t s, int size_class = 0, int kind = 0) {
  const uint32_t seq = ++h->seq_next;
  hipLaunchKernelGGL(publish_counters, dim3(1), dim3(64), 0, s, h->d_wctr, h->d_ctr, h->h_wctr, h->h_ctr, h->h_seq, seq);
  PLVS_KERNEL_CHECK();
  return wait_published(h, seq, s, kind, size_class);
}


static int poisoned(plvs_tsdf_chisel* h) {
  h->poisoned = true;
  return PLVS_ERR_CAPACITY;
}

static int walk_fail(plvs_tsdf_chisel* h, uint32_t err) {
  plvs::set_error("tsdf_chisel integrate: %s%s(err=%u)", (err & kErrPoolFull) ? "chunk pool full (raise max_chunks) " : "",
                  (err & kErrCoordRange) ? "voxel coordinates beyond +-2^20 (outside the supported map extent) " : "", err);
  return poisoned(h);
}


static hipError_t stage_mark(plvs_tsdf_chisel* h, int i, hipStream_t q) {
  return h->profiling ? hipEventRecord(h->ev[i], q) : hipSuccess;
}

static hipError_t stage_elapsed(float* ms, hipEvent_t a, hipEvent_t b) {
  hipError_t e = hipEventElapsedTime(ms, a, b);
  if (e == hipErrorNotReady) {
    (void)hipGetLastError();
    e = hipEventSynchronize(a);
    if (e == hipSuccess) e = hipEventSynchronize(b);
    if (e == hipSuccess) e = hipEventElapsedTime(ms, a, b);
  }
  return e;
}

static int add_stage_times(plvs_tsdf_chisel* h, int first, int n) {
  for (int i = first; i < first + n; ++i) {
    float ms = 0.f;
    PLVS_HIP_TRY(stage_elapsed(&ms, h->ev[i], h->ev[i + 1]));
    h->stage_ms[i] += ms;
  }
  return PLVS_OK;
}
```

plvs_amd/csrc/tsdf_chisel_order_free.hpp:

```cpp
#pragma once
#include "tsdf_chisel_handle.hpp"

namespace {

__global__ void walk_prologue(const float* __restrict__ Twc, int nclouds, Pose* __restrict__ poses,
                              const int32_t* __restrict__ host_offsets, int32_t* __restrict__ offsets,
                              WalkCounters* __restrict__ wctr, Counters* __restrict__ ctr, uint32_t* __restrict__ chunk_nseg,
                              int nseg, int ntile_first = 0) {
  const int i0 = blockIdx.x * blockDim.x + threadIdx.x, stride = gridDim.x * blockDim.x;
  for (int c = i0; c < nclouds; c += stride) make_pose(Twc + 12 * c, &poses[c]);
  for (int c = i0; c < 2 * (nclouds + 1) + ntile_first; c += stride) offsets[c] = host_offsets[c];
  for (int k = i0; k < nseg; k += stride) chunk_nseg[k] = 0u;
  uint32_t* w = reinterpret_cast<uint32_t*>(wctr);
  for (int k = i0; k < (int)(2 * sizeof(WalkCounters) / sizeof(uint32_t)); k += stride) w[k] = 0u;
  if (i0 == 0) {
    ctr->total_visits = 0;
    ctr->err = 0;
    ctr->num_heads = 0;
    ctr->num_updated = 0;
    ctr->max_run = 0;
    ctr->num_desc = 0;
  }
}

// ... 77 lines not shown
template <bool kScatter>
static void launch_seg_pass(plvs_tsdf_chisel* h, const SegSrc& src, hipStream_t q) {
  hipLaunchKernelGGL((seg_pass<kScatter>), dim3(ceil_div(src.slots, kSegSpan)), dim3(256), 0, q, h->w_seg.p, src.seg_cap,
                     src.ntiles, src.seg_cnt, h->w_chunk_nseg.p, h->w_chunk_off.p, h->w_chunk_fill.p, h->w_sorted_seg.p,
                     h->d_wctr);
}
static SegPlace seg_place_args(const plvs_tsdf_chisel* h, uint32_t seg_cap) {
  return SegPlace{h->w_seg_ticket.p, h->w_chunk_off.p, h->w_sorted_seg.p, (uint32_t)std::min<size_t>(h->w_sorted_seg.cap / 2, 0xFFFFFFFFu),
                  seg_cap};
}
static void launch_seg_place(plvs_tsdf_chisel* h, const SegSrc& src, hipStream_t q) {
  const SegPlace a = seg_place_args(h, src.seg_cap);
  hipLaunchKernelGGL(seg_place, dim3(ceil_div(src.slots, 256)), dim3(256), 0, q, h->w_seg.p, a.ticket, src.seg_cap, src.ntiles,
                     src.seg_cnt, a.chunk_off, a.sorted, a.sorted_cap, h->d_wctr);
}

struct SegScan {
  const int32_t* num_chunks;
  int chunk_cap;
  const uint32_t *tile_visits, *run_cnt;
  uint32_t ntiles;
  uint32_t* active_idx;
};
static void launch_seg_scan(plvs_tsdf_chisel* h, const SegScan& a, hipStream_t q) {
  hipLaunchKernelGGL(seg_scan, dim3(1), dim3(1024), 0, q, h->w_chunk_nseg.p, h->w_chunk_off.p, h->w_chunk_fill.p, h->updated.p,
                     h->w_active_off.p, h->d_wctr, a.num_chunks, a.chunk_cap, a.tile_visits, a.run_cnt, a.ntiles,
                     h->w_part_off.p, h->w_multi_idx.p, h->multi_cap, h->part_segs, h->part_min, a.active_idx);
}

static void sort_segments(plvs_tsdf_chisel* h, const SegSrc& src, const SegScan& scan, hipStream_t q) {
  launch_seg_pass<false>(h, src, q);
  launch_seg_scan(h, scan, q);
  launch_seg_pass<true>(h, src, q);
}

template <bool kWide, bool kEmit>
static void launch_apply(plvs_tsdf_chisel* h, const uint4* rec, const uint32_t* d_kfid, const EmitOut& emit, uint32_t last_shift,
                         hipStream_t q) {
  hipLaunchKernelGGL((apply_chunks<kWide, kEmit>), dim3(4096), dim3(kApplyThreads), 0, q, h->w_sorted_seg.p, h->updated.p,
                     h->w_active_off.p, h->w_part_off.p, h->w_multi_idx.p, h->part_segs,
                     PartAcc{h->pa_wuu.p, h->pa_w.p, h->pa_last.p, h->pa_cnt.p, h->pa_done.p}, rec,
                     kEmit ? 0.0 : 1.0 / (double)h->scale_u, kEmit ? 0.0 : 1.0 / (double)h->scale_w, d_kfid,
                     kEmit ? (float*)nullptr : h->sdf, kEmit ? (float*)nullptr : h->weight, kEmit ? (uint32_t*)nullptr : h->kfid,
                     h->d_wctr, emit, last_shift);
}

struct WalkScratch {
  size_t rec_own, seg_own, rec_spill, seg_spill;
};
static WalkScratch walk_scratch(const plvs_tsdf_chisel* h, uint32_t ntiles) {
  WalkScratch w;
  w.rec_own = (size_t)ntiles * kRecStride;
  w.seg_own = (size_t)ntiles * kWalkChunks;
  w.rec_spill = std::max<size_t>(h->w_rec.cap > w.rec_own ? h->w_rec.cap - w.rec_own : 0, (size_t)1 << 16);
  w.seg_spill = std::max<size_t>(h->w_seg.cap / 2 > w.seg_own ? h->w_seg.cap / 2 - w.seg_own : 0, (size_t)1 << 12);
  return w;
}
static int reserve_walk_scratch(plvs_tsdf_chisel* h, uint32_t ntiles, const WalkScratch& w) {
  if (h->w_rec.cap < w.rec_own + w.rec_spill) PLVS_HIP_TRY(h->w_rec.reserve(2 * w.rec_own + w.rec_spill));
  if (h->w_seg.cap < 2 * (w.seg_own + w.seg_spill)) PLVS_HIP_TRY(h->w_seg.reserve(2 * (2 * w.seg_own + w.seg_spill)));
  PLVS_HIP_TRY(h->w_sorted_seg.reserve(h->w_seg.cap));
  PLVS_HIP_TRY(h->w_seg_ticket.reserve(h->w_seg.cap / 2));
  const size_t run_slots = (size_t)ntiles << h->run_r1_log2;
  if (h->w_runkey.cap < run_slots) {
    PLVS_HIP_TRY(h->w_runkey.reserve(2 * run_slots));
    PLVS_HIP_TRY(h->w_masks.reserve(2 * run_slots * kMaskWords));
  }
  PLVS_HIP_TRY(h->w_masks.reserve(run_slots * kMaskWords));
  return PLVS_OK;
}
static AccOut walk_out(const plvs_tsdf_chisel* h, const WalkScratch& w, uint32_t* chunk_nseg) {
  return AccOut{h->w_rec.p, (uint32_t)std::min<size_t>(w.rec_own + w.rec_spill, 0xFFFFFFFFu), h->w_seg.p,
                (uint32_t)std::min<size_t>(w.seg_own + w.seg_spill, 0xFFFFFFFFu), h->w_seg_cnt.p, h->w_tile_visits.p, chunk_nseg,
                chunk_nseg ? h->w_seg_ticket.p : nullptr};
}
static bool grow_walk_scratch(plvs_tsdf_chisel* h, uint32_t ntiles, WalkScratch& w) {
  w.rec_spill = std::max<size_t>(w.rec_spill, (size_t)h->h_wctr->rec_top * 2);
  w.seg_spill = std::max<size_t>(w.seg_spill, (size_t)h->h_wctr->seg_top * 2);
  while ((1u << h->run_r1_log2) < h->h_wctr->run_need) ++h->run_r1_log2;
  return ((size_t)ntiles << h->run_r1_log2) < 0xFFFFFFFFull;
}


struct WalkCall {
  const float* d_xyz;
  const uint8_t* d_rgb;
  const uint32_t* d_kfid;
  int n, nclouds;
  uint32_t ntiles;
  int max_chunks;
  const GridSrc* gsrc;
  const GridSrc* d_grid;
  size_t seg_slots;
  AccOut out;
  RunOut runs;
  const uint32_t* last_count;
  uint32_t collect_seq;
};

template <int E>
static void launch_walk_fast(plvs_tsdf_chisel* h, const WalkCall& c, const WalkPass& pass, hipStream_t s) {
  uint32_t* const counts[3] = {&h->d_wctr->ndeferred, &h->d_wctr->ndeferred2, &h->d_wctr->ndeferred3};
  const uint32_t* const list = pass.src < 0 ? nullptr : h->w_deferred.p + (size_t)pass.src * c.ntiles;
  const uint32_t* const nlist = pass.src < 0 ? nullptr : counts[pass.src];
  const auto kernel = c.d_grid ? walk_fast<E, true> : walk_fast<E, false>;
  hipLaunchKernelGGL(kernel, dim3(pass.grid), dim3(kWalkRays), 0, s, h->P, h->scale_u, h->scale_w, c.d_xyz, c.n, h->offsets.p,
                     c.nclouds, h->poses.p, h->dir, &h->d_ctr->num_chunks, h->d_wctr, h->rgbw, (const uint32_t*)nullptr, c.out,
                     c.runs, TileMap{1u, 0u, 1u}, kRecStride, list, nlist, h->w_deferred.p + (size_t)pass.dst * c.ntiles,
                     counts[pass.dst], c.d_grid);
}

static void launch_walk_passes(plvs_tsdf_chisel* h, const WalkPlan& plan, const WalkCall& c, hipStream_t s) {
  for (int i = 0; i < plan.npasses; ++i) {
    const WalkPass& pass = plan.pass[i];
    if (pass.entries == kPlanSmallClass) launch_walk_fast<kFastEntriesSmall>(h, c, pass, s);
    else if (pass.entries == kFastEntries) launch_walk_fast<kFastEntries>(h, c, pass, s);
    else launch_walk_fast<kFastEntriesBig>(h, c, pass, s);
  }
  hipLaunchKernelGGL((walk_tiles<true, true>), dim3(kDeferGrid), dim3(kWalkRays), 0, s, h->P, h->scale_u, h->scale_w, c.d_xyz,
                     c.n, h->offsets.p, c.nclouds, h->poses.p, h->dir, &h->d_ctr->num_chunks, h->d_wctr, h->rgbw,
                     (const uint32_t*)nullptr, c.out, c.runs, TileMap{1u, 0u, 1u}, c.ntiles,
                     (const uint32_t*)(h->w_deferred.p + (size_t)plan.last_list * c.ntiles), c.last_count, kRecStride,
                     plan.pieces, c.d_grid);
}

static int segments_and_apply(plvs_tsdf_chisel* h, const WalkPlan& plan, const WalkCall& c, hipStream_t q) {
  launch_seg_scan(h, SegScan{&h->d_ctr->num_chunks, c.max_chunks, h->w_tile_visits.p, h->w_run_cnt.p, c.ntiles,
                             plan.collect_ready ? h->w_active_idx.p : nullptr}, q);
  if (plan.collect_ready) {
    const bool queued = plan.chain == kChainCollected;
    PLVS_HIP_TRY(hipStreamWaitEvent(q, h->ev_zero, 0));
    hipLaunchKernelGGL(runs_count, dim3(plan.collect_blocks), dim3(kSegSpan), 0, q, h->w_seg.p, h->w_rseg.p, c.ntiles, h->w_seg_cnt.p,
                       h->w_active_idx.p, plan.collect_rows, plan.collect_blocks, h->w_run_matrix.p, h->w_rpre.p, h->d_wctr, c.last_count,
                       seg_place_args(h, c.out.seg_cap));
    hipLaunchKernelGGL(runs_rowscan, dim3(std::min<uint32_t>(ceil_div(plan.collect_rows, 4), 1024u)), dim3(256), 0, q,
                       h->w_run_matrix.p, plan.collect_rows, plan.collect_blocks, h->d_wctr, h->w_item_cnt.p);
    hipLaunchKernelGGL(rows_place, dim3(1), dim3(1024), 0, q, h->w_item_cnt.p, plan.collect_rows, plan.collect_bound,
                       (uint32_t)std::min<size_t>(plan.parts_cap, 0xFFFFFFFFu), h->d_wctr,
                       h->w_item_base.p, h->w_item_part0.p, h->w_part_item.p, reinterpret_cast<const uint32_t*>(h->d_ctr),
                       reinterpret_cast<uint32_t*>(h->h_wctr), reinterpret_cast<uint32_t*>(h->h_ctr),
                       (uint32_t)(sizeof(Counters) / sizeof(uint32_t)), queued ? h->h_seq : (uint32_t*)nullptr,
                       queued ? c.collect_seq : 0u);
    PLVS_HIP_TRY(hipEventRecord(h->ev_seg, q));
  }
  if (!plan.collect_ready) launch_seg_place(h, SegSrc{c.seg_slots, c.out.seg_cap, c.ntiles, h->w_seg_cnt.p}, q);
  PLVS_HIP_TRY(stage_mark(h, 2, q));
  launch_apply<false, false>(h, h->w_rec.p, c.d_kfid, EmitOut{}, c.gsrc ? c.gsrc->key_bits : 0u, q);
  PLVS_KERNEL_CHECK();
  PLVS_HIP_TRY(stage_mark(h, 3, q));
  return PLVS_OK;
}

static int launch_fold(plvs_tsdf_chisel* h, const WalkCall& c, uint32_t D, const uint32_t* skeys, const uint32_t* sval,
                       const uint32_t* skip, hipStream_t q) {
  const RunSrc rsrc{h->w_masks.p, (uint32_t)kMaskWords, h->run_r1_log2, TileMap{1u, 0u}, h->offsets.p, c.nclouds,
                    reinterpret_cast<const uint32_t*>(h->offsets.p) + 2 * ((size_t)c.nclouds + 1)};
  const auto kernel = c.gsrc ? fold_colours_masks<true> : fold_colours_masks<false>;
  hipLaunchKernelGGL(kernel, dim3(std::min<size_t>(ceil_div(D, kFoldWaves), 8192)), dim3(64 * kFoldWaves), 0, q, skeys, sval,
                     &h->d_wctr[1].num_desc, rsrc, h->heads.p, c.d_rgb, h->rgbw, &h->d_wctr[1].num_heads, (uint32_t*)nullptr,
                     (uint32_t*)nullptr, skip, c.gsrc ? *c.gsrc : GridSrc{});
  PLVS_KERNEL_CHECK();
  return PLVS_OK;
}

template <int BITS>
static void launch_sort_medium(plvs_tsdf_chisel* h, uint32_t ntiles, int passes, const RunGuard* guard, hipStream_t q) {
  hipLaunchKernelGGL(sort_runs_medium<BITS>, dim3(1), dim3(1024), 0, q, h->w_runkey.p, h->w_run_cnt.p, ntiles, h->run_r1_log2,
                     h->d_wctr + 1, h->dkey0.p, h->w_val0.p, h->dkey1.p, h->w_val1.p, h->w_run_off.p, h->heads.p, passes,
                     guard ? guard->limit : 0xFFFFFFFFu, &h->d_ctr->num_chunks, guard ? guard->chunk_limit : 0,
                     guard ? guard->skip : (uint32_t*)nullptr);
}

static int colour_chain(plvs_tsdf_chisel* h, const WalkCall& c, uint32_t D, int chunks, const RunGuard* guard, hipStream_t q) {
  const uint32_t* skeys = h->dkey0.p;
  const uint32_t* sval = h->w_val0.p;
  switch (sort_kind(D, c.ntiles)) {
    case kSortSmall:
      hipLaunchKernelGGL(sort_runs_small, dim3(1), dim3(1024), 0, q, h->w_runkey.p, h->w_run_cnt.p, c.ntiles,
                         h->run_r1_log2, h->d_wctr + 1, h->dkey0.p, h->w_val0.p, h->heads.p, guard ? guard->skip : (uint32_t*)nullptr);
      break;
    case kSortMedium: {
      PLVS_HIP_TRY(h->dkey0.reserve(D));
      PLVS_HIP_TRY(h->dkey1.reserve(D));
      PLVS_HIP_TRY(h->w_val0.reserve(D));
      PLVS_HIP_TRY(h->w_val1.reserve(D));
      PLVS_HIP_TRY(h->heads.reserve(D));
      const int key_bits = voxel_key_bits(chunks);
      const bool ten = key_bits <= 20;
      const int passes = ten ? 2 : (key_bits + 7) / 8;
      if (ten) launch_sort_medium<10>(h, c.ntiles, passes, guard, q);
      else launch_sort_medium<8>(h, c.ntiles, passes, guard, q);
      skeys = (passes & 1) ? h->dkey1.p : h->dkey0.p;
      sval = (passes & 1) ? h->w_val1.p : h->w_val0.p;
      break;
    }
    case kSortGeneral: {
      int rc = sort_runs(h, D, c.ntiles, chunks, q, &skeys, &sval, guard);
      if (rc != PLVS_OK) return rc;
      PLVS_HIP_TRY(h->heads.reserve(D));
      PLVS_HIP_TRY(h->w_dummy.reserve((size_t)c.max_chunks + 1));
      hipLaunchKernelGGL(voxel_heads, dim3(ceil_div(D, 256 * kHeadTiles)), dim3(256), 0, q, skeys, D, h->heads.p, h->w_dummy.p,
                         h->d_wctr + 1, guard ? (const uint32_t*)&h->d_wctr[1].num_desc : (const uint32_t*)nullptr);
      break;
    }
  }
  return launch_fold(h, c, D, skeys, sval, guard ? (const uint32_t*)guard->skip : (const uint32_t*)nullptr, q);
}

static int collect_chain(plvs_tsdf_chisel* h, const WalkPlan& plan, const WalkCall& c, uint32_t D, hipStream_t q) {
  const uint32_t rows = plan.collect_rows, blocks = plan.collect_blocks;
  PLVS_HIP_TRY(hipStreamWaitEvent(q, h->ev_seg, 0));
  hipLaunchKernelGGL(runs_scatter, dim3(blocks * (kSegSpan / 256)), dim3(256), 0, q, h->w_seg.p, h->w_rseg.p, c.ntiles, h->w_seg_cnt.p,
                     h->w_active_idx.p, rows, blocks, h->w_run_matrix.p, h->w_rpre.p, h->w_item_base.p, h->d_wctr, h->w_val0.p);
  const unsigned part_grid = (unsigned)std::min<size_t>(plan.parts_cap, 4096);
  hipLaunchKernelGGL(parts_count, dim3(part_grid), dim3(256), 0, q, h->w_part_item.p, h->w_item_part0.p, h->w_item_base.p,
                     h->w_item_cnt.p, h->w_runkey.p, h->d_wctr, h->w_val0.p, h->dkey0.p, h->w_phist.p);
  hipLaunchKernelGGL(rows_heads, dim3(std::min<uint32_t>(ceil_div(rows, 4), 1024u)), dim3(256), 0, q, h->w_item_part0.p,
                     h->w_item_cnt.p, h->w_phist.p, h->d_wctr, rows, h->w_row_heads.p, h->w_row_tot.p);
  hipLaunchKernelGGL(parts_place, dim3(part_grid), dim3(512), 0, q, h->w_part_item.p, h->w_item_part0.p, h->w_item_base.p,
                     h->w_item_cnt.p, h->w_phist.p, h->d_wctr, h->dkey0.p, h->w_val0.p, h->dkey1.p, h->w_val1.p, h->heads.p,
                     h->w_row_heads.p, rows, h->w_row_tot.p);
  return launch_fold(h, c, D, h->dkey1.p, h->w_val1.p, &h->d_wctr[1].skip, q);
}

static int reserve_collect(plvs_tsdf_chisel* h, const WalkPlan& plan, const WalkScratch& w, int max_chunks) {
  const uint32_t rows = plan.collect_rows;
  PLVS_HIP_TRY(h->w_rseg.reserve(h->w_seg.cap));
  PLVS_HIP_TRY(h->w_rpre.reserve(w.seg_own));
  PLVS_HIP_TRY(h->w_active_idx.reserve((size_t)max_chunks));
  PLVS_HIP_TRY(h->w_run_matrix.reserve((size_t)rows * plan.collect_blocks));
  PLVS_HIP_TRY(h->w_item_base.reserve(rows));
  PLVS_HIP_TRY(h->w_item_cnt.reserve(rows));
  PLVS_HIP_TRY(h->w_item_part0.reserve(rows));
  PLVS_HIP_TRY(h->w_row_heads.reserve(rows));
  PLVS_HIP_TRY(h->w_row_tot.reserve((size_t)rows * kSlabVox));
  PLVS_HIP_TRY(h->dkey0.reserve(plan.collect_bound));
  PLVS_HIP_TRY(h->dkey1.reserve(plan.collect_bound));
  PLVS_HIP_TRY(h->w_val0.reserve(plan.collect_bound));
  PLVS_HIP_TRY(h->w_val1.reserve(plan.collect_bound));
  PLVS_HIP_TRY(h->heads.reserve(plan.collect_bound));
  PLVS_HIP_TRY(h->w_part_item.reserve(plan.parts_cap));
  PLVS_HIP_TRY(h->w_phist.reserve(plan.parts_cap * kSlabVox));
  PLVS_HIP_TRY(hipMemsetAsync(h->w_run_matrix.p, 0, (size_t)rows * plan.collect_blocks * sizeof(uint32_t), h->side));
  PLVS_HIP_TRY(hipEventRecord(h->ev_zero, h->side));
  return PLVS_OK;
}

constexpr size_t kGridWords = (sizeof(GridSrc) + 3) / 4;
static_assert(sizeof(GridSrc) % 4 == 0 && alignof(GridSrc) <= 8, "GridSrc travels as words behind the offsets");
static int fill_call_tables(plvs_tsdf_chisel* h, const int32_t* offsets, int nclouds, const GridSrc* gsrc, uint32_t* ntiles_out,
                            size_t* table_words_out) {
  size_t tiles_of_call = 0;
  for (int c = 0; c < nclouds; ++c) tiles_of_call += ((size_t)(offsets[c + 1] - offsets[c]) + kWalkRays - 1) / kWalkRays;
  const size_t grid_tiles = gsrc ? (size_t)nclouds * gsrc->ntx * gsrc->nty : 0;
  if (gsrc) PLVS_REQUIRE(grid_tiles < 0x7FFFFFFFull, "too many images in one call");
  const size_t table_words = 2 * ((size_t)nclouds + 1) + 2 * tiles_of_call + (gsrc ? kGridWords : 0);
  if (h->h_offsets_cap < table_words) {
    if (h->h_offsets) (void)hipHostFree(h->h_offsets);
    h->h_offsets = nullptr;
    h->h_offsets_cap = 0;
    PLVS_HIP_TRY(hipHostMalloc((void**)&h->h_offsets, (2 * table_words + 64) * sizeof(int32_t)));
    h->h_offsets_cap = 2 * table_words + 64;
  }
  const uint32_t cloud_tiles = plvs::tsdf::fill_tile_table(offsets, nclouds, h->h_offsets, kWalkRays);
  const uint32_t ntiles = gsrc ? (uint32_t)grid_tiles : cloud_tiles;
  int32_t* tf = h->h_offsets + 2 * ((size_t)nclouds + 1);
  if (gsrc) memcpy(tf, gsrc, sizeof(GridSrc));
  size_t t = 0;
  for (int c = 0; c < nclouds; ++c)
    for (int32_t p = offsets[c]; p < offsets[c + 1]; p += kWalkRays) {
      tf[ntiles + t] = c;
      tf[t++] = p;
    }
  *ntiles_out = ntiles;
  *table_words_out = table_words;
  return PLVS_OK;
}

static int reserve_call(plvs_tsdf_chisel* h, uint32_t ntiles, size_t table_words) {
  const size_t max_chunks = (size_t)h->prm.max_chunks;
  PLVS_HIP_TRY(h->offsets.reserve(table_words));
  PLVS_HIP_TRY(h->tile_state.reserve((size_t)ntiles + 1));
  int rc = reserve_chunk_tables(h, max_chunks, std::min<uint32_t>((uint32_t)max_chunks, 64u));
  if (rc != PLVS_OK) return rc;
  PLVS_HIP_TRY(h->w_seg_cnt.reserve(ntiles));
  PLVS_HIP_TRY(h->w_tile_visits.reserve(ntiles));
  PLVS_HIP_TRY(h->w_deferred.reserve(3 * (size_t)ntiles));
  PLVS_HIP_TRY(h->w_run_cnt.reserve(ntiles));
  PLVS_HIP_TRY(h->dkey0.reserve(kSmallRuns));
  PLVS_HIP_TRY(h->w_val0.reserve(kSmallRuns));
  PLVS_HIP_TRY(h->heads.reserve(kSmallRuns));
  PLVS_HIP_TRY(h->w_run_off.reserve((size_t)ntiles + 1));
  PLVS_HIP_TRY(h->scratch.reserve(scan_scratch_words(ntiles)));
  return PLVS_OK;
}

static int finish_call(plvs_tsdf_chisel* h, uint32_t ntiles, int chunks_before, const timespec& t0, bool trace) {
  const WalkCounters& c = *h->h_wctr;
  h->num_chunks = h->h_ctr->num_chunks;
  adapt_after_call(h->walk, WalkOutcome{h->h_wctr[1].num_desc, c.ndeferred, c.ndeferred2, c.over_small}, ntiles);
  if (trace) {
    timespec t1;
    clock_gettime(CLOCK_MONOTONIC, &t1);
    fprintf(stderr, "[tsdf_chisel] %.0f us ", (double)(t1.tv_sec - t0.tv_sec) * 1e6 + (double)(t1.tv_nsec - t0.tv_nsec) * 1e-3);
    fprintf(stderr, "[tsdf_chisel] tiles %u deferred %u split %u visits %llu runs %u updated %u parts %u multi %u "
            "rec_top %u seg_top %u voxels %u max_run %u chunks %d chain %d%s\n", ntiles, c.ndeferred * 1000u + c.ndeferred2 + c.ndeferred3 * 1000000u, c.split_tiles,
            (unsigned long long)c.total_visits, h->h_wctr[1].num_desc, c.num_updated, c.num_parts, c.num_multi, c.rec_top,
            c.seg_top, c.num_heads, c.max_run, h->num_chunks, h->last_chain, h->last_chain_skipped ? " REPEATED" : "");
  }
  h->stats.visits = (int64_t)c.total_visits;
  h->stats.new_chunks = h->num_chunks - chunks_before;
  h->stats.updated_chunks = (int32_t)c.num_updated;
  h->stats.voxels = (int32_t)c.num_heads;
  h->stats.max_run = (int32_t)c.max_run;
  h->last_updated = c.num_updated;
  const uint32_t max_chunks = (uint32_t)h->prm.max_chunks;
  const uint32_t want = std::min<uint32_t>(max_chunks, std::max(c.num_multi + c.num_multi / 2, 2u * c.num_updated));
  if (want > h->multi_cap) {
    int rc = ensure_part_acc(h, std::min<uint32_t>(max_chunks, std::max(want, 2u * h->multi_cap)));
    if (rc != PLVS_OK) return rc;
  }
  if (h->profiling) {
    int rc = add_stage_times(h, 0, kWalkStages);
    if (rc != PLVS_OK) return rc;
    h->prof_calls++;
  }
  return PLVS_OK;
}

static int integrate_walk_acc(plvs_tsdf_chisel* h, const float* d_xyz, const uint8_t* d_rgb, const uint32_t* d_kfid,
                              int n, int nclouds, const int32_t* offsets, const float* d_Twc, hipStream_t s,
                              const GridSrc* gsrc = nullptr) {
  static const int collect_mode = plvs::env_int("PLVS_TSDF_COLLECT", 1, 0, 2);
  static const int max_row_chunks = plvs::env_int("PLVS_TSDF_COLLECT_MAX_ROWS", 0, 0, 1 << 20);
  static const bool trace = plvs::env_int("PLVS_HIP_TSDF_TRACE", 0, 0, 1) != 0;
  const int max_chunks = h->prm.max_chunks;
  uint32_t ntiles = 0;
  size_t table_words = 0;
  int rc = fill_call_tables(h, offsets, nclouds, gsrc, &ntiles, &table_words);
  if (rc != PLVS_OK) return rc;
  if ((size_t)ntiles * kRecStride + (1 << 16) >= 0xFFFFFFFFull) {
    plvs::set_error("tsdf_chisel integrate: %d points in one call exceed the record index range (split the batch)", n);
    return PLVS_ERR_CAPACITY;
  }
  if ((rc = reserve_call(h, ntiles, table_words)) != PLVS_OK) return rc;
  WalkScratch scratch = walk_scratch(h, ntiles);
  h->stage_set = 1;
  const int chunks_before = h->num_chunks;
  timespec trace_t0;
  clock_gettime(CLOCK_MONOTONIC, &trace_t0);
  uint32_t* const counts[3] = {&h->d_wctr->ndeferred, &h->d_wctr->ndeferred2, &h->d_wctr->ndeferred3};
  uint32_t* const side_ctr = &h->d_wctr[1].num_desc;
  for (int attempt = 0;; ++attempt) {
    if ((rc = reserve_walk_scratch(h, ntiles, scratch)) != PLVS_OK) return rc;
    const WalkPlan plan = plan_walk_call(WalkPlanInput{ntiles, attempt, max_chunks, chunks_before, h->run_r1_log2, h->walk,
                                                       h->last_updated, collect_mode, max_row_chunks});
    if (plan.collect_ready && (rc = reserve_collect(h, plan, scratch, max_chunks)) != PLVS_OK) return rc;
    hipLaunchKernelGGL(walk_prologue, dim3(ceil_div((size_t)std::max(max_chunks, nclouds + 1), 256)), dim3(256), 0, s, d_Twc,
                       nclouds, h->poses.p, (const int32_t*)h->h_offsets, h->offsets.p, h->d_wctr, h->d_ctr, h->w_chunk_nseg.p,
                       max_chunks, gsrc ? (int)kGridWords : (int)(2 * ntiles));
    PLVS_HIP_TRY(stage_mark(h, 0, s));
    const WalkCall call{d_xyz, d_rgb, d_kfid, n, nclouds, ntiles, max_chunks, gsrc,
                        gsrc ? reinterpret_cast<const GridSrc*>(h->offsets.p + 2 * ((size_t)nclouds + 1)) : nullptr,
                        scratch.seg_own + scratch.seg_spill, walk_out(h, scratch, h->w_chunk_nseg.p),
                        RunOut{h->w_runkey.p, h->w_masks.p, h->w_run_cnt.p, h->run_r1_log2, plan.collect_ready ? h->w_rseg.p : nullptr},
                        counts[plan.last_list], plan.chain == kChainCollected ? ++h->seq_next : 0u};
    launch_walk_passes(h, plan, call, s);
    if (plan.record_fork) PLVS_HIP_TRY(hipEventRecord(h->ev_fork, s));
    PLVS_HIP_TRY(stage_mark(h, 1, s));
    bool collected = false, scanned = false;
    if (plan.chain == kChainPredicted) {
      if (plan.serial_small && (rc = segments_and_apply(h, plan, call, s)) != PLVS_OK) return rc;
      if ((scanned = plan.scan_first))
        PLVS_HIP_TRY(exclusive_scan_u32(h->w_run_cnt.p, h->w_run_off.p, ntiles, side_ctr, h->scratch.p, s));
      const RunGuard guard{plan.run_bound, side_ctr, &h->d_ctr->num_chunks, plan.chunk_bound, &h->d_wctr[0].err,
                           &h->d_wctr[1].skip, 1u, nullptr, 0u};
      if ((rc = colour_chain(h, call, plan.run_bound, plan.chunk_bound, &guard, s)) != PLVS_OK) return rc;
      if (plan.apply_on_side) {
        PLVS_HIP_TRY(hipStreamWaitEvent(h->side, h->ev_fork, 0));
        if ((rc = segments_and_apply(h, plan, call, h->side)) != PLVS_OK) return rc;
      }
    } else {
      if ((rc = segments_and_apply(h, plan, call, s)) != PLVS_OK) return rc;
      const size_t last_count_word = call.last_count - reinterpret_cast<const uint32_t*>(h->d_wctr);
      if (plan.chain == kChainCollected) {
        if ((rc = collect_chain(h, plan, call, plan.collect_bound, h->side)) != PLVS_OK) return rc;
        if ((rc = wait_published(h, call.collect_seq, h->side, 1, plan.size_class)) != PLVS_OK) return rc;
        const uint32_t left_to_walk_tiles = reinterpret_cast<const uint32_t*>(h->h_wctr)[last_count_word];
        collected = !(h->h_wctr[0].err == 0 && (left_to_walk_tiles != 0u || h->h_wctr[0].seg_top != 0u));
        if (!collected) {
          scanned = true;
          PLVS_HIP_TRY(exclusive_scan_u32(h->w_run_cnt.p, h->w_run_off.p, ntiles, side_ctr, h->scratch.p, h->side));
          if ((rc = read_walk_counters(h, h->side, plan.size_class, 2)) != PLVS_OK) return rc;
// ... 42 lines not shown
```

plvs_amd/csrc/tsdf_chisel_shard.hpp:

```cpp
#pragma once
#include "tsdf_chisel_order_free.hpp"
#include "tsdf_chisel_halo.hpp"
#include "tsdf_shard.hpp"

namespace {

__global__ void shard_apply_begin(Counters* ctr, WalkCounters* wctr, int32_t* xcount_sat, uint32_t* __restrict__ chunk_nseg,
                                  uint32_t max_chunks, uint32_t total_seg, uint32_t total_runs) {
  const uint32_t i = blockIdx.x * blockDim.x + threadIdx.x;
  for (uint32_t c = i; c < max_chunks; c += gridDim.x * blockDim.x) chunk_nseg[c] = 0u;
  if (i == 0) {
    ctr->total_visits = 0u;
    ctr->err = 0u; ctr->num_heads = 0u; ctr->num_updated = 0u; ctr->max_run = 0u; ctr->num_desc = 0u;
    wctr[0] = WalkCounters{};
    wctr[1] = WalkCounters{};
    wctr[0].seg_top = total_seg;
    wctr[1].num_desc = total_runs;
    *xcount_sat = 0;
  }
}

}

static int shard_state_init(plvs_tsdf_chisel* h) {
// ... 137 lines not shown
                     (const uint32_t*)&h->d_wctr->ndeferred, (uint32_t)kWalkLimit,
                     1u, (const GridSrc*)nullptr);
  return PLVS_OK;
}

static int shard_walk_plan(plvs_tsdf_chisel* h, const ShardWalk& c, uint32_t* h_plan, hipStream_t s) {
  const int N = c.N;
  const uint32_t nt = c.nt;
  hipLaunchKernelGGL(shard_chunk_totals, dim3(1024), dim3(256), 0, s, h->w_sorted_seg.p, h->updated.p,
                     h->w_active_off.p, h->xdir.slot_ids, N, h->d_wctr, h->sh_nrec.p, h->sh_owner.p, h->sh_slot_owner.p);
  hipLaunchKernelGGL(shard_plan, dim3(1), dim3(1024), 0, s, h->sh_nrec.p, h->sh_owner.p, N, h->d_wctr, h->sh_ctl.p,
                     h->sh_ctl.p + 256);
  PLVS_HIP_TRY(exclusive_scan_u32(h->w_run_cnt.p, h->w_run_off.p, nt, nullptr, h->scratch.p, s));
  hipLaunchKernelGGL(compact_runs, dim3(ceil_div(nt, 4)), dim3(256), 0, s, h->w_runkey.p, h->w_run_cnt.p,
                     h->w_run_off.p, nt, h->run_r1_log2, h->dkey0.p, h->w_val0.p, no_guard());
  hipLaunchKernelGGL(shard_run_count, dim3(2048), dim3(256), 0, s, h->dkey0.p, h->w_val0.p, &h->d_wctr[0].num_desc,
                     h->w_masks.p, h->sh_slot_owner.p, N, h->sh_run_ctr.p, h->sh_run_first.p, h->d_wctr);
  hipLaunchKernelGGL(shard_run_plan, dim3(1), dim3(64), 0, s, h->sh_run_ctr.p, N, h->d_wctr);
  PLVS_KERNEL_CHECK();
  hipLaunchKernelGGL(publish_words, dim3(1), dim3(64), 0, s, (const uint32_t*)(h->sh_ctl.p + 256), h_plan, 2,
                     reinterpret_cast<const uint32_t*>(h->d_wctr), reinterpret_cast<uint32_t*>(h->h_wctr),
                     (int)(sizeof(WalkCounters) / sizeof(uint32_t)), (const uint32_t*)nullptr, (uint32_t*)nullptr, 0);
  PLVS_KERNEL_CHECK();
  PLVS_HIP_TRY(hipStreamSynchronize(s));
  return PLVS_OK;
}

static int shard_walk_aggregate(plvs_tsdf_chisel* h, const uint32_t* h_plan, hipStream_t s) {
  PLVS_HIP_TRY(h->sh_seg_reg.reserve(2 * (size_t)h_plan[0] + 2));
  PLVS_HIP_TRY(h->sh_rec_reg.reserve(2 * (size_t)h_plan[1] + 2));
  uint32_t* const ctl = h->sh_ctl.p;
  launch_apply<false, true>(h, h->w_rec.p, nullptr,
                            EmitOut{h->xdir.slot_ids, h->sh_owner.p, ctl, ctl + 64, ctl + 128, ctl + 192, h->sh_seg_reg.p,
                                    h->sh_rec_reg.p}, 0u, s);
  PLVS_KERNEL_CHECK();
  hipLaunchKernelGGL(publish_words, dim3(1), dim3(256), 0, s, (const uint32_t*)h->sh_ctl.p, h->h_sh_ctl, 256,
                     (const uint32_t*)h->sh_run_ctr.p, h->h_sh_ctl + 256, 64, (const uint32_t*)nullptr, (uint32_t*)nullptr, 0);
  PLVS_KERNEL_CHECK();
  PLVS_HIP_TRY(hipStreamSynchronize(s));
  return PLVS_OK;
}

static int shard_walk_finish(plvs_tsdf_chisel* h, const ShardWalk& c, int64_t* send_counts) {
  for (int p = 0; p < c.N; ++p) {
    h->h_sh_counts[3 * p] = (long long)h->h_sh_ctl[128 + p];
    h->h_sh_counts[3 * p + 1] = (long long)h->h_sh_ctl[192 + p];
    h->h_sh_counts[3 * p + 2] = (long long)h->h_sh_ctl[256 + p];
  }
  if (h->h_wctr->num_multi > h->multi_cap) {
    int rc = ensure_part_acc(h, (uint32_t)std::min<size_t>(c.xmax, (size_t)h->h_wctr->num_multi + h->h_wctr->num_multi / 2));
    if (rc != PLVS_OK) return rc;
  }
  h->sh_runs = h->h_wctr->num_desc;
  for (int p = 0; p < 3 * c.N; ++p) send_counts[p] = (int64_t)h->h_sh_counts[p];
  h->sh_stats.visits = (int64_t)h->h_wctr->total_visits;
  return PLVS_OK;
}


struct ShardApply {
  const void *d_seg_src, *d_rec_src, *d_run_src;
  const uint8_t* d_rgb;
  const uint32_t* d_kfid;
  int N, max_chunks;
  size_t tseg, trec, trun;
  int chunks_before;
  uint32_t* d_src_off;
};

static int shard_apply_check(plvs_tsdf_chisel* h, const int64_t* recv_counts, ShardApply* c) {
  const int N = c->N;
  PLVS_REQUIRE(h->h_sh_off != nullptr, "shard_apply follows shard_walk");
  uint32_t* const src_off = h->h_sh_off + 128;
  size_t tseg = 0, trec = 0, trun = 0;
  for (int q = 0; q < N; ++q) {
    PLVS_REQUIRE(recv_counts[3 * q] >= 0 && recv_counts[3 * q + 1] >= 0 && recv_counts[3 * q + 2] >= 0, "negative receive count");
    src_off[q] = (uint32_t)tseg;
    src_off[N + 1 + q] = (uint32_t)trec;
    tseg += (size_t)recv_counts[3 * q];
    trec += (size_t)recv_counts[3 * q + 1];
    trun += (size_t)recv_counts[3 * q + 2];
  }
  src_off[N] = (uint32_t)tseg;
  src_off[2 * N + 1] = (uint32_t)trec;
  PLVS_REQUIRE(tseg < 0x7FFFFFFFull && trec < 0xFFFFFFFFull && trun < 0x7FFFFFFFull,
               "receive buffers beyond the index range (split the batch)");
  c->tseg = tseg;
  c->trec = trec;
  c->trun = trun;
  return PLVS_OK;
}

static int shard_apply_reserve(plvs_tsdf_chisel* h, const ShardApply& c) {
  const uint32_t total = (uint32_t)c.tseg;
  PLVS_HIP_TRY(h->sh_src_off.reserve(128 + 132));
  PLVS_HIP_TRY(h->w_seg.reserve(2 * (size_t)total));
  PLVS_HIP_TRY(h->w_sorted_seg.reserve(2 * (size_t)total));
  return reserve_chunk_tables(h, (size_t)c.max_chunks,
                              std::min<uint32_t>((uint32_t)c.max_chunks, total / std::max(1u, h->part_min) + 1u));
}

static int shard_apply_sort(plvs_tsdf_chisel* h, ShardApply& c, hipStream_t s) {
  const uint32_t total = (uint32_t)c.tseg;
  c.chunks_before = h->num_chunks;
  c.d_src_off = h->sh_src_off.p + 128;
  PLVS_HIP_TRY(hipMemcpyAsync(c.d_src_off, h->h_sh_off + 128, 2 * ((size_t)c.N + 1) * sizeof(uint32_t), hipMemcpyHostToDevice, s));
  hipLaunchKernelGGL(shard_apply_begin, dim3(ceil_div((size_t)c.max_chunks, 1024)), dim3(256), 0, s, h->d_ctr, h->d_wctr,
                     h->d_xcount + 2, h->w_chunk_nseg.p, (uint32_t)c.max_chunks, total, (uint32_t)c.trun);
  PLVS_HIP_TRY(stage_mark(h, 0, s));
  PLVS_HIP_TRY(stage_mark(h, 1, s));
  hipLaunchKernelGGL(shard_translate, dim3(ceil_div((size_t)total, 256)), dim3(256), 0, s,
                     static_cast<const uint4*>(c.d_seg_src), total, c.d_src_off, c.N, h->dir, &h->d_ctr->num_chunks,
                     &h->d_wctr[0].err, h->w_seg.p);
  sort_segments(h, SegSrc{(size_t)total, total, 0u, nullptr},
                SegScan{&h->d_ctr->num_chunks, c.max_chunks, nullptr, nullptr, 0u, nullptr}, s);
  PLVS_HIP_TRY(stage_mark(h, 2, s));
  return PLVS_OK;
}

static int shard_apply_colours(plvs_tsdf_chisel* h, const ShardApply& c, hipStream_t s) {
  const uint32_t R = (uint32_t)c.trun;
  const uint32_t* runs = static_cast<const uint32_t*>(c.d_run_src);
  PLVS_HIP_TRY(h->dkey0.reserve(R));
  PLVS_HIP_TRY(h->dkey1.reserve(R));
  PLVS_HIP_TRY(h->w_val0.reserve(R));
  PLVS_HIP_TRY(h->w_val1.reserve(R));
  PLVS_HIP_TRY(h->sh_vkey.reserve(R));
  PLVS_HIP_TRY(h->heads.reserve(R));
  PLVS_HIP_TRY(h->sh_sat.reserve(R));
  PLVS_HIP_TRY(h->w_dummy.reserve((size_t)c.max_chunks + 1));
  PLVS_HIP_TRY(h->scratch.reserve(radix_scratch_words(R)));
  uint32_t* const err = &h->d_wctr[0].err;
  hipLaunchKernelGGL(shard_run_translate, dim3(ceil_div((size_t)R, 256)), dim3(256), 0, s, runs, R, h->dir, err,
                     h->sh_vkey.p, h->dkey0.p, h->w_val0.p);
  int tile_bits = 1;
  while ((1ull << tile_bits) < (unsigned long long)h->sh_ntiles) ++tile_bits;
  bool second = false;
  PLVS_HIP_TRY(radix_sort_pairs(h->dkey0.p, h->w_val0.p, h->dkey1.p, h->w_val1.p, R, 0, tile_bits, h->scratch.p, s, &second));
  uint32_t* order = second ? h->w_val1.p : h->w_val0.p;
  uint32_t* other = second ? h->w_val0.p : h->w_val1.p;
  uint32_t* k_in = second ? h->dkey0.p : h->dkey1.p;
  uint32_t* k_out = second ? h->dkey1.p : h->dkey0.p;
  hipLaunchKernelGGL(shard_gather_keys, dim3(ceil_div((size_t)R, 256)), dim3(256), 0, s, h->sh_vkey.p, order, R, k_in);
  const long long slot_bound = std::min<long long>(c.max_chunks, (long long)c.chunks_before + (long long)c.tseg);
  PLVS_HIP_TRY(radix_sort_pairs(k_in, order, k_out, other, R, 0, voxel_key_bits(slot_bound), h->scratch.p, s, &second));
  const uint32_t* skeys = second ? k_out : k_in;
  const uint32_t* sval = second ? other : order;
  hipLaunchKernelGGL(voxel_heads, dim3(ceil_div(R, 256 * kHeadTiles)), dim3(256), 0, s, skeys, R, h->heads.p,
                     h->w_dummy.p, h->d_wctr + 1);
  hipLaunchKernelGGL(fold_colours_masks<false>, dim3(std::min<size_t>(ceil_div(R, kFoldWaves), 8192)), dim3(64 * kFoldWaves), 0, s,
                     skeys, sval, &h->d_wctr[1].num_desc,
                     RunSrc{runs, kWireRun, 0u, TileMap{1u, 0u}, h->offsets.p, h->sh_nclouds, nullptr}, h->heads.p, c.d_rgb,
                     h->rgbw, &h->d_wctr[1].num_heads, h->sh_sat.p, reinterpret_cast<uint32_t*>(h->d_xcount + 2),
                     (const uint32_t*)nullptr, GridSrc{});
  PLVS_KERNEL_CHECK();
  return PLVS_OK;
}

static int shard_apply_finish(plvs_tsdf_chisel* h, const ShardApply& c, hipStream_t s) {
  hipLaunchKernelGGL(publish_words, dim3(1), dim3(64), 0, s, reinterpret_cast<const uint32_t*>(h->d_xcount + 2),
                     reinterpret_cast<uint32_t*>(h->h_sh_counts), 1, (const uint32_t*)nullptr, (uint32_t*)nullptr, 0,
                     (const uint32_t*)nullptr, (uint32_t*)nullptr, 0);
  int rc = read_walk_counters(h, s);
  if (rc != PLVS_OK) return rc;
  if (h->h_wctr->err) return walk_fail(h, h->h_wctr->err);
  h->sh_nsat = (uint32_t)(*reinterpret_cast<int32_t*>(h->h_sh_counts));
  h->num_chunks = h->h_ctr->num_chunks;
  h->stats.new_chunks = h->num_chunks - c.chunks_before;
  h->stats.updated_chunks = (int32_t)h->h_wctr->num_updated;
  h->stats.voxels = (int32_t)h->h_wctr->num_heads;
  h->stats.max_run = (int32_t)h->h_wctr->max_run;
  h->last_updated = h->h_wctr->num_updated;
  if (h->profiling) {
    if ((rc = add_stage_times(h, 0, kWalkStages)) != PLVS_OK) return rc;
    h->prof_calls++;
  }
  return PLVS_OK;
}

extern "C" {

int plvs_hip_tsdf_chisel_shard_walk(plvs_tsdf_chisel* h, const float* d_xyz, const int32_t* offsets, int nclouds,
                                    const float* d_Twc, int64_t* send_counts, void* stream) {
  PLVS_REQUIRE(h && send_counts, "null argument");
  PLVS_REQUIRE(!h->poisoned, "handle is in a failed state (clear it)");
  PLVS_REQUIRE(h->prm.order_free != 0 && h->prm.shard_count >= 1 && h->prm.shard_count <= 64,
               "the ray-sharded integrate needs order_free = 1 and 1 <= shard_count <= 64");
  PLVS_REQUIRE(offsets && nclouds >= 0, "bad offsets");
  hipStream_t s = static_cast<hipStream_t>(stream);
  ShardWalk c{};
  c.d_xyz = d_xyz;
  int rc = shard_walk_begin(h, offsets, nclouds, send_counts, s, &c);
  if (rc != PLVS_OK || c.nt == 0) return rc;
  PLVS_REQUIRE(d_xyz && d_Twc, "null device pointer");
  h->sh_nt = c.nt;
  if ((rc = shard_walk_reserve(h, c, d_Twc, s)) != PLVS_OK) return rc;
  uint32_t* const h_plan = reinterpret_cast<uint32_t*>(h->h_sh_counts + 3 * 64);
  for (int attempt = 0;; ++attempt) {
    if ((rc = shard_walk_launch(h, c, s)) != PLVS_OK) return rc;
    sort_segments(h, SegSrc{c.scratch.seg_own + c.scratch.seg_spill, c.out.seg_cap, c.nt, h->w_seg_cnt.p},
                  SegScan{h->d_xcount, (int)c.xmax, h->w_tile_visits.p, h->w_run_cnt.p, c.nt, nullptr}, s);
    if ((rc = shard_walk_plan(h, c, h_plan, s)) != PLVS_OK) return rc;
    const uint32_t err = h->h_wctr->err;
    if (err & kErrPoolFull) {
      plvs::set_error("tsdf_chisel shard_walk: the walk directory is full (max_chunks x shard_count chunks)");
      return poisoned(h);
    }
    if (err & ~kErrScratch) return walk_fail(h, err);
    if (!(err & kErrScratch)) break;
    if (attempt >= 8 || !grow_walk_scratch(h, c.nt, c.scratch)) return walk_fail(h, err);
  }
  if ((rc = shard_walk_aggregate(h, h_plan, s)) != PLVS_OK) return rc;
  return shard_walk_finish(h, c, send_counts);
}

int plvs_hip_tsdf_chisel_shard_pack(plvs_tsdf_chisel* h, void* d_seg_dst, void* d_rec_dst, void* d_run_dst, void* stream) {
  PLVS_REQUIRE(h, "null handle");
  PLVS_REQUIRE(h->sh_phase == 1, "shard_pack follows shard_walk");
  hipStream_t s = static_cast<hipStream_t>(stream);
  h->sh_phase = 2;
  const int N = std::max(1, h->prm.shard_count);
  long long nseg = 0;
  for (int p = 0; p < N; ++p) nseg += h->h_sh_counts ? h->h_sh_counts[3 * p] : 0;
  if (nseg == 0) return PLVS_OK;
  PLVS_REQUIRE(d_seg_dst && d_rec_dst && (h->sh_runs == 0 || d_run_dst), "null send buffer");
  uint32_t* const dst_off = h->h_sh_off;
  for (int p = 0; p < 128; ++p) dst_off[p] = 0;
  for (int p = 1; p < N; ++p) {
    dst_off[p] = dst_off[p - 1] + (uint32_t)h->h_sh_counts[3 * (p - 1)];
    dst_off[64 + p] = dst_off[64 + p - 1] + (uint32_t)h->h_sh_counts[3 * (p - 1) + 1];
  }
  PLVS_HIP_TRY(h->sh_src_off.reserve(128 + 132));
  PLVS_HIP_TRY(hipMemcpyAsync(h->sh_src_off.p, dst_off, 128 * sizeof(uint32_t), hipMemcpyHostToDevice, s));
  hipLaunchKernelGGL(shard_copy_regions, dim3(512), dim3(256), 0, s, h->sh_seg_reg.p, h->sh_rec_reg.p, h->sh_ctl.p,
                     h->sh_src_off.p, N, static_cast<uint4*>(d_seg_dst), static_cast<uint4*>(d_rec_dst));
  if (h->sh_runs > 0)
    hipLaunchKernelGGL(shard_run_pack, dim3(std::min<size_t>(ceil_div((size_t)h->sh_runs, kRunSpan), 4096)), dim3(256), 0, s,
                       h->dkey0.p, h->w_val0.p, &h->d_wctr[0].num_desc, h->w_masks.p, h->sh_run_first.p, h->run_r1_log2,
                       shard_tile_map(h), h->xdir.slot_ids, h->sh_slot_owner.p, h->sh_run_ctr.p + 64, h->sh_run_ctr.p + 128, static_cast<uint32_t*>(d_run_dst));
  PLVS_KERNEL_CHECK();
  return PLVS_OK;
}

int plvs_hip_tsdf_chisel_shard_apply(plvs_tsdf_chisel* h, const void* d_seg_src, const void* d_rec_src,
                                     const void* d_run_src, const int64_t* recv_counts, const uint8_t* d_rgb,
                                     const uint32_t* d_kfid, void* stream) {
  PLVS_REQUIRE(h && recv_counts, "null argument");
  PLVS_REQUIRE(!h->poisoned, "handle is in a failed state (clear it)");
  PLVS_REQUIRE(h->sh_phase == 2, "shard_apply follows shard_pack");
  hipStream_t s = static_cast<hipStream_t>(stream);
  int rc = halo_drop(h, s);
  if (rc != PLVS_OK) return rc;
  h->sh_phase = 0;
  h->sh_nsat = 0;
  ShardApply c{d_seg_src, d_rec_src, d_run_src, d_rgb, d_kfid, std::max(1, h->prm.shard_count), h->prm.max_chunks};
  if ((rc = shard_apply_check(h, recv_counts, &c)) != PLVS_OK) return rc;
  h->stats = h->sh_stats;
  h->last_updated = 0;
  h->stage_set = 1;
  if (c.tseg == 0) return PLVS_OK;
  PLVS_REQUIRE(d_seg_src && d_rec_src && d_rgb && (c.trun == 0 || d_run_src), "null device pointer");
  if ((rc = shard_apply_reserve(h, c)) != PLVS_OK) return rc;
  if ((rc = shard_apply_sort(h, c, s)) != PLVS_OK) return rc;
  launch_apply<true, false>(h, static_cast<const uint4*>(d_rec_src), d_kfid, EmitOut{}, 0u, s);
  PLVS_KERNEL_CHECK();
  PLVS_HIP_TRY(stage_mark(h, 3, s));
  if (c.trun > 0 && (rc = shard_apply_colours(h, c, s)) != PLVS_OK) return rc;
  PLVS_HIP_TRY(stage_mark(h, 4, s));
  return shard_apply_finish(h, c, s);
}

int plvs_hip_tsdf_chisel_shard_saturated(plvs_tsdf_chisel* h, int32_t* d_voxels, int cap, int* n, void* stream) {
  PLVS_REQUIRE(h && n, "null argument");
  *n = (int)h->sh_nsat;
  if (h->sh_nsat == 0) return PLVS_OK;
  if (cap < (int)h->sh_nsat) {
    plvs::set_error("shard_saturated: %u voxels, room for %d", h->sh_nsat, cap);
    return PLVS_ERR_CAPACITY;
  }
  PLVS_REQUIRE(d_voxels, "null output");
  hipStream_t s = static_cast<hipStream_t>(stream);
  hipLaunchKernelGGL(shard_saturated_ids, dim3(ceil_div((size_t)h->sh_nsat, 256)), dim3(256), 0, s, h->sh_sat.p, h->sh_nsat,
                     h->dir.slot_ids, d_voxels);
  PLVS_KERNEL_CHECK();
  return PLVS_OK;
}

int plvs_hip_tsdf_chisel_shard_saturated_message(plvs_tsdf_chisel* h, int32_t* d_msg, int rows, void* stream) {
  PLVS_REQUIRE(h && d_msg && rows > 0, "bad argument");
  hipStream_t s = static_cast<hipStream_t>(stream);
  if (h->sh_nsat > 0) {
    const size_t need = 4 * ((size_t)h->sh_wait_first + h->sh_wait_count + h->sh_nsat);
    if (need > h->sh_wait.cap) {
      DevBuf<int32_t> grown;
      PLVS_HIP_TRY(grown.reserve(need));
      if (h->sh_wait_count)
        PLVS_HIP_TRY(hipMemcpyAsync(grown.p, h->sh_wait.p + 4 * (size_t)h->sh_wait_first, 16 * (size_t)h->sh_wait_count,
                                    hipMemcpyDeviceToDevice, s));
      PLVS_HIP_TRY(hipStreamSynchronize(s));
      h->sh_wait.release();
      h->sh_wait = grown;
      h->sh_wait_first = 0;
    }
    hipLaunchKernelGGL(shard_saturated_ids, dim3(ceil_div((size_t)h->sh_nsat, 256)), dim3(256), 0, s, h->sh_sat.p, h->sh_nsat,
                       h->dir.slot_ids, h->sh_wait.p + 4 * ((size_t)h->sh_wait_first + h->sh_wait_count));
    h->sh_wait_count += h->sh_nsat;
    h->sh_nsat = 0;
// ... 39 lines not shown
```

plvs_amd/csrc/tsdf_walk.hpp:

```cpp
#pragma once
#include <hip/hip_runtime.h>

#include <cstdint>

#include "tsdf_chisel_core.hpp"
#include "tsdf_directory.hpp"
#include "tsdf_tiles.hpp"
#include "tsdf_walk_table.hpp"

namespace {

using namespace plvs::chisel;
using plvs::tsdf::cloud_of;
using plvs::tsdf::tile_span;
using plvs::tsdf::tile_span_tables;
using plvs::tsdf::TileSpan;
using plvs::tsdf::kCoordBias;
using plvs::tsdf::kErrCoordRange;
using plvs::tsdf::kErrDirectoryMiss;
using plvs::tsdf::kErrPoolFull;
using plvs::tsdf::home_bucket;
using plvs::tsdf::next_bucket;

constexpr int kWalkRays = 512;
constexpr int kMaskWords = kWalkRays / 32;
#ifndef PLVS_WALK_ENTRIES
#define PLVS_WALK_ENTRIES 4096
#endif
constexpr int kWalkEntries = PLVS_WALK_ENTRIES;
constexpr int kWalkLimit = kWalkEntries * 7 / 8;
constexpr int kWalkWindow = kWalkLimit / 2;
constexpr int kWalkChunks = 64;
constexpr uint32_t kErrScratch = 8u;

#ifdef PLVS_WALK_PROF
__device__ unsigned long long g_walk_prof[16];
__device__ unsigned long long g_apply_items[8192][4];
#define WALK_PROF_BEGIN()                                         \
  long long prof_t = (long long)clock64();                        \
  unsigned long long prof_acc[9] = {0, 0, 0, 0, 0, 0, 0, 0, 0}
#define WALK_PROF(k)                                               \
  do {                                                             \
    const long long now = (long long)clock64();                    \
    prof_acc[k] += (unsigned long long)(now - prof_t);             \
    prof_t = now;                                                  \
  } while (0)
#define WALK_PROF_END()                                            \
  do {                                                             \
    if (threadIdx.x == 0)                                          \
      for (int k = 0; k < 9; ++k) atomicAdd(&g_walk_prof[k], prof_acc[k]); \
  } while (0)
#else
#define WALK_PROF_BEGIN() do {} while (0)
#define WALK_PROF(k) do {} while (0)
#define WALK_PROF_END() do {} while (0)
#endif

struct WalkCounters {
  unsigned long long total_visits;
  uint32_t err;
  uint32_t num_heads;
  uint32_t num_updated;
  uint32_t max_run;
  uint32_t num_desc;
  uint32_t run_need;
  uint32_t rec_top, seg_top;
  uint32_t ncold;
  uint32_t split_tiles;
  uint32_t num_parts;
  uint32_t num_multi;
  uint32_t ndeferred;
  uint32_t ndeferred2;
  uint32_t over_small;
  uint32_t skip;
  uint32_t collect_top;
  uint32_t collect_parts;
  uint32_t ndeferred3;
};

constexpr int kLogLen = 16;
constexpr int kSlabs = 8;
constexpr int kSlabVox = kChunkVox / kSlabs;

struct SubTile {
  uint16_t lo, hi;
  uint32_t vlo, vhi;
  int32_t cloud;
};

constexpr uint32_t kKeyEmpty = 0xFFFFFFFFu;
constexpr int kBuckets = kWalkEntries / 4;
constexpr int kOriginBias = 512;

constexpr int log2_of(int v) { return v <= 1 ? 0 : 1 + log2_of(v / 2); }
struct WalkShared {
  static constexpr int kEntries = kWalkEntries, kBucketCount = kWalkEntries / 4, kLogLen = ::kLogLen;
  alignas(16) uint32_t ekey[kWalkEntries];
  int32_t org[3];
  uint32_t cand[kWalkRays / 64];
  int32_t worg[kWalkRays / 64][3];
  uint32_t run_total, vis_total;
  uint32_t ccode[kWalkChunks];
  int32_t cslot[kWalkChunks];
  uint32_t ccnt[kWalkChunks * kSlabs];
  uint16_t cbase[kWalkChunks * kSlabs];
  uint32_t rbase;
  SubTile stack[16];
  int sp;
  uint32_t nent;
  uint32_t overflow;
  uint32_t wsum[kWalkRays / 64];
  uint32_t next, nrays;
};
template <int E>
struct FastShared {
  static constexpr int kEntries = E, kBucketCount = E / 4, kLogLen = E == 1536 ? ::kLogLen - 1 : ::kLogLen;
  static_assert(E % kWalkRays == 0 && E >= 1024, "every thread owns E / kWalkRays entries (and a bucket four)");
  alignas(16) uint32_t ekey[E];
  uint32_t cand[kWalkRays / 64];
  int32_t worg[kWalkRays / 64][3];
  uint32_t run_total, vis_total;
  uint32_t ccode[kWalkChunks];
  int32_t cslot[kWalkChunks];
  uint32_t ccnt[kWalkChunks * kSlabs];
  uint16_t cbase[kWalkChunks * kSlabs];
  uint32_t rcnt[kWalkChunks * kSlabs];
  uint16_t rcbase[kWalkChunks * kSlabs];
  uint32_t any_cold;
  uint32_t nent, overflow;
};


__device__ __forceinline__ bool rel_key(int vx, int vy, int vz, int ox, int oy, int oz, uint32_t* key) {
  const uint32_t dx = (uint32_t)(vx - ox), dy = (uint32_t)(vy - oy), dz = (uint32_t)(vz - oz);
  *key = dx | (dy << 10) | (dz << 20);
  return ((dx | dy | dz) >> 10) == 0u;
}
__device__ __forceinline__ int origin_of(int v) { return (v - kOriginBias) & ~15; }
constexpr uint32_t kChunkCodeMask = 0x3F0FC3F0u;
__device__ __forceinline__ uint32_t chunk_code(uint32_t key) { return key & kChunkCodeMask; }
__device__ __forceinline__ uint32_t voxel_in_chunk(uint32_t key) {
  return (key & 15u) | ((key >> 6) & 0xF0u) | ((key >> 12) & 0xF00u);
}
__device__ __forceinline__ void chunk_of_code(uint32_t code, int ox, int oy, int oz, int* cx, int* cy, int* cz) {
  *cx = (ox >> 4) + (int)((code >> 4) & 63u);
  *cy = (oy >> 4) + (int)((code >> 14) & 63u);
  *cz = (oz >> 4) + (int)((code >> 24) & 63u);
}
constexpr uint32_t kKeyMul = plvs::tsdf::kTableKeyMul, kKeyMulInv = plvs::tsdf::kTableKeyMulInv;
__device__ __forceinline__ uint32_t table_key(uint32_t key) { return key * kKeyMul; }
__device__ __forceinline__ uint32_t voxel_key(uint32_t tkey) { return tkey * kKeyMulInv; }
template <class SH>
__device__ __forceinline__ uint32_t key_bucket(uint32_t tkey) { return home_bucket<SH::kBucketCount>(tkey); }

__device__ __forceinline__ uint32_t wave_scan_incl(uint32_t x) {
  x += (uint32_t)__builtin_amdgcn_update_dpp(0, (int)x, 0x111, 0xf, 0xf, false);
  x += (uint32_t)__builtin_amdgcn_update_dpp(0, (int)x, 0x112, 0xf, 0xf, false);
  x += (uint32_t)__builtin_amdgcn_update_dpp(0, (int)x, 0x114, 0xf, 0xf, false);
  x += (uint32_t)__builtin_amdgcn_update_dpp(0, (int)x, 0x118, 0xf, 0xf, false);
  x += (uint32_t)__builtin_amdgcn_update_dpp(0, (int)x, 0x142, 0xa, 0xf, false);
  x += (uint32_t)__builtin_amdgcn_update_dpp(0, (int)x, 0x143, 0xc, 0xf, false);
  return x;
}
__device__ __forceinline__ uint32_t wave_sum(uint32_t x) {
  return (uint32_t)__builtin_amdgcn_readlane((int)wave_scan_incl(x), 63);
}

__device__ __forceinline__ int bucket_match(const uint4 k4, uint32_t want) {
  const bool c0 = k4.x == want, c1 = k4.y == want, c2 = k4.z == want, c3 = k4.w == want;
  const int j = c3 ? 3 : (c2 ? 2 : (c1 ? 1 : 0));
  return (c0 | c1 | c2 | c3) ? j : -1;
}

constexpr int kProbeCap = plvs::tsdf::kTableProbeCap;
template <class SH>
// ... 2074 lines not shown
    const uint32_t r = r0 + tid;
    const uint32_t T = r < nrows ? item_cnt[r] : 0u, np = (T + kCollectPart - 1u) / kCollectPart;
    const uint32_t ti = wave_scan_incl(T), pi = wave_scan_incl(np);
    if (lane == 63) { wt[wid] = ti; wp[wid] = pi; }
    __syncthreads();
    uint32_t tb = ct, pb = cp, tt = 0, pt = 0;
#pragma unroll
    for (uint32_t w = 0; w < 16; ++w) {
      if (w < wid) { tb += wt[w]; pb += wp[w]; }
      tt += wt[w];
      pt += wp[w];
    }
    if (r < nrows) {
      const uint32_t p0 = pb + pi - np;
      item_base[r] = tb + ti - T;
      item_part0[r] = p0;
      for (uint32_t i = 0; i < np && p0 + i < parts_cap; ++i) part_item[p0 + i] = r;
    }
    __syncthreads();
    if (tid == 0) { ct += tt; cp += pt; }
    __syncthreads();
  }
  if (tid == 0 && go) {
    ctr[1].collect_top = ct;
    ctr[1].collect_parts = cp;
    if (ct > run_bound || cp > parts_cap) ctr[1].skip = 1u;
  }
  if (host_seq != nullptr) {
    __syncthreads();
    const uint32_t* a = reinterpret_cast<const uint32_t*>(ctr);
    for (uint32_t k = tid; k < (uint32_t)(2 * sizeof(WalkCounters) / sizeof(uint32_t)); k += 1024) host_a[k] = a[k];
    for (uint32_t k = tid; k < nb; k += 1024) host_b[k] = pub_b[k];
    __threadfence_system();
    __syncthreads();
    if (tid == 0) __hip_atomic_store(host_seq, seq, __ATOMIC_RELEASE, __HIP_MEMORY_SCOPE_SYSTEM);
  }
}

__global__ __launch_bounds__(256) void runs_scatter(const uint4* __restrict__ seg, const uint4* __restrict__ rseg, uint32_t ntiles,
                                                    const uint32_t* __restrict__ seg_cnt, const uint32_t* __restrict__ active_idx,
                                                    uint32_t rows_cap, uint32_t nblocks, const uint32_t* __restrict__ M,
                                                    const uint4* __restrict__ rpre, const uint32_t* __restrict__ item_base,
                                                    const WalkCounters* __restrict__ ctr, uint32_t* __restrict__ tv) {
  if (ctr[1].skip != 0u) return;
  const uint32_t lane = threadIdx.x & 63;
  const uint32_t j = blockIdx.x * 256u + threadIdx.x;
  const uint32_t tile = j / kWalkChunks, block = j / (uint32_t)kSegSpan;
  uint32_t f[kSlabs], c[kSlabs], at[kSlabs];
#pragma unroll
  for (int s = 0; s < kSlabs; ++s) f[s] = c[s] = at[s] = 0u;
  uint4 r0 = make_uint4(0u, 0u, 0u, 0u);
  if (tile < ntiles && (j % kWalkChunks) < seg_cnt[tile]) r0 = rseg[2 * (size_t)j];
  if (r0.y != 0u) {
    const uint4 r1 = rseg[2 * (size_t)j + 1], pre = rpre[j];
    const uint32_t row0 = active_idx[seg[2 * (size_t)j].x] * (uint32_t)kSlabs;
#pragma unroll
    for (int s = 0; s < kSlabs; ++s) slab_runs(r0, r1, s, &f[s], &c[s]);
    const uint4 ib0 = *reinterpret_cast<const uint4*>(item_base + row0), ib1 = *reinterpret_cast<const uint4*>(item_base + row0 + 4);
    const uint32_t ib[kSlabs] = {ib0.x, ib0.y, ib0.z, ib0.w, ib1.x, ib1.y, ib1.z, ib1.w};
    uint32_t m[kSlabs];
#pragma unroll
    for (int s = 0; s < kSlabs; ++s) m[s] = c[s] ? M[(size_t)(row0 + (uint32_t)s) * nblocks + block] : 0u;
#pragma unroll
    for (int s = 0; s < kSlabs; ++s) at[s] = ib[s] + m[s] + suboffset_of(pre, s);
  }
#pragma unroll
  for (int s = 0; s < kSlabs; ++s) {
    const bool big = c[s] >= 32u;
    if (!big)
      for (uint32_t k = 0; k < c[s]; ++k) tv[at[s] + k] = f[s] + k;
    unsigned long long todo = __ballot(big);
    while (todo) {
      const int src = __ffsll((long long)todo) - 1;
      todo &= todo - 1ull;
      const uint32_t bp = (uint32_t)__shfl((int)at[s], src), bf = (uint32_t)__shfl((int)f[s], src);
      const uint32_t bc = (uint32_t)__shfl((int)c[s], src);
      for (uint32_t k = lane; k < bc; k += 64) tv[bp + k] = bf + k;
    }
  }
}

constexpr int kCollectFlight = 4;
__global__ __launch_bounds__(256) void parts_count(const uint32_t* __restrict__ part_item, const uint32_t* __restrict__ item_part0,
                                                   const uint32_t* __restrict__ item_base, const uint32_t* __restrict__ item_cnt,
                                                   const uint32_t* __restrict__ runkey, const WalkCounters* __restrict__ ctr,
                                                   const uint32_t* __restrict__ tv, uint32_t* __restrict__ tk,
                                                   uint32_t* __restrict__ phist) {
  __shared__ uint32_t hist[kSlabVox];
  if (ctr[1].skip != 0u) return;
  const uint32_t tid = threadIdx.x, nparts = ctr[1].collect_parts;
  for (uint32_t p = blockIdx.x; p < nparts; p += gridDim.x) {
    const uint32_t row = part_item[p], lo = (p - item_part0[row]) * kCollectPart, hi = min(item_cnt[row], lo + kCollectPart);
    const uint32_t base = item_base[row];
    for (uint32_t k = tid; k < (uint32_t)kSlabVox; k += 256) hist[k] = 0u;
    __syncthreads();
    for (uint32_t e0 = lo; e0 < hi; e0 += 256 * kCollectFlight) {
      uint32_t slot[kCollectFlight], k[kCollectFlight];
#pragma unroll
      for (int b = 0; b < kCollectFlight; ++b) {
        const uint32_t e = e0 + 256u * (uint32_t)b + tid;
        slot[b] = e < hi ? tv[base + e] : 0xFFFFFFFFu;
      }
#pragma unroll
      for (int b = 0; b < kCollectFlight; ++b) k[b] = slot[b] != 0xFFFFFFFFu ? runkey[slot[b]] : 0u;
#pragma unroll
      for (int b = 0; b < kCollectFlight; ++b) {
        if (slot[b] == 0xFFFFFFFFu) continue;
        tk[base + e0 + 256u * (uint32_t)b + tid] = k[b];
        atomicAdd(&hist[k[b] % (uint32_t)kSlabVox], 1u);
      }
    }
    __syncthreads();
    for (uint32_t k = tid; k < (uint32_t)kSlabVox; k += 256) phist[(size_t)p * kSlabVox + k] = hist[k];
    __syncthreads();
  }
}

__global__ __launch_bounds__(256) void rows_heads(const uint32_t* __restrict__ item_part0, const uint32_t* __restrict__ item_cnt,
                                                  uint32_t* __restrict__ phist, const WalkCounters* __restrict__ ctr,
                                                  uint32_t rows_cap, uint32_t* __restrict__ row_heads,
                                                  uint32_t* __restrict__ row_tot) {
  if (ctr[1].skip != 0u) return;
  const uint32_t lane = threadIdx.x & 63, wid = threadIdx.x >> 6;
  const uint32_t nrows = min(rows_cap, ctr->num_updated * (uint32_t)kSlabs);
  for (uint32_t row = blockIdx.x * 4u + wid; row < nrows; row += gridDim.x * 4u) {
    const uint32_t T = item_cnt[row], P = (T + kCollectPart - 1u) / kCollectPart, p0 = item_part0[row];
    uint32_t nz = 0;
    if (P) {
      uint32_t h[kSlabVox / 64];
#pragma unroll
      for (int k = 0; k < kSlabVox / 64; ++k) h[k] = 0;
      for (uint32_t q = 0; q < P; ++q)
#pragma unroll
        for (int k = 0; k < kSlabVox / 64; ++k) {
          uint32_t* const cell = &phist[(size_t)(p0 + q) * kSlabVox + (uint32_t)k * 64u + lane];
          const uint32_t c = *cell;
          *cell = h[k];
          h[k] += c;
        }
#pragma unroll
      for (int k = 0; k < kSlabVox / 64; ++k) {
        row_tot[(size_t)row * kSlabVox + (uint32_t)k * 64u + lane] = h[k];
        nz += (uint32_t)__popcll(__ballot(h[k] != 0u));
      }
    }
    if (lane == 0) row_heads[row] = nz;
  }
}

__global__ __launch_bounds__(512) void parts_place(const uint32_t* __restrict__ part_item, const uint32_t* __restrict__ item_part0,
                                                   const uint32_t* __restrict__ item_base, const uint32_t* __restrict__ item_cnt,
                                                   const uint32_t* __restrict__ phist, WalkCounters* __restrict__ ctr,
                                                   const uint32_t* __restrict__ tk, const uint32_t* __restrict__ tv,
                                                   uint32_t* __restrict__ ok, uint32_t* __restrict__ ov,
                                                   uint32_t* __restrict__ heads, const uint32_t* __restrict__ row_heads,
                                                   uint32_t rows_cap, const uint32_t* __restrict__ row_tot) {
  constexpr int kWaves = 8, kBatches = kCollectPart / (64 * kWaves);
  __shared__ uint32_t hist[kWaves][kSlabVox];
  __shared__ uint32_t wtot[kWaves], wflag[kWaves], wsum[kWaves];
  static_assert(kSlabVox == 512, "a thread per voxel of the slab");
  if (ctr[1].skip != 0u) return;
  const uint32_t tid = threadIdx.x, lane = tid & 63, wid = tid >> 6;
  const uint32_t nparts = ctr[1].collect_parts;
  const uint32_t nrows = min(rows_cap, ctr->num_updated * (uint32_t)kSlabs);
  for (uint32_t p = blockIdx.x; p < nparts; p += gridDim.x) {
    const uint32_t row = part_item[p], p0 = item_part0[row], pi = p - p0, T = item_cnt[row];
    const uint32_t base = item_base[row], lo = pi * kCollectPart, hi = min(T, lo + kCollectPart);
#pragma unroll
    for (int w = 0; w < kWaves; ++w) hist[w][tid] = 0u;
    __syncthreads();
    const uint32_t wlo = lo + wid * (kCollectPart / kWaves);
    uint32_t k[kBatches], v[kBatches];
#pragma unroll
    for (int b = 0; b < kBatches; ++b) {
      const uint32_t e = wlo + 64u * (uint32_t)b + lane;
      k[b] = e < hi ? tk[base + e] : 0u;
      v[b] = e < hi ? tv[base + e] : 0u;
    }
#pragma unroll
    for (int b = 0; b < kBatches; ++b)
      if (wlo + 64u * (uint32_t)b + lane < hi) atomicAdd(&hist[wid][k[b] % (uint32_t)kSlabVox], 1u);
    __syncthreads();
    {
      uint32_t tot = 0;
#pragma unroll
      for (int w = 0; w < kWaves; ++w) {
        const uint32_t c = hist[w][tid];
        hist[w][tid] = tot;
        tot += c;
      }
      const uint32_t all = row_tot[(size_t)row * kSlabVox + tid], before = phist[(size_t)p * kSlabVox + tid];
      const uint32_t flag = (pi == 0u && all) ? 1u : 0u;
      const uint32_t inc = wave_scan_incl(all), finc = wave_scan_incl(flag);
      uint32_t hsum = 0;
      if (pi == 0u) {
        for (uint32_t r = tid; r < row; r += 512) hsum += row_heads[r];
        uint32_t all_rows = 0;
        if (p == 0u) {
          for (uint32_t r = tid; r < nrows; r += 512) all_rows += row_heads[r];
          all_rows = wave_sum(all_rows);
        }
        hsum = wave_sum(hsum);
        if (lane == 0) wsum[wid] = hsum;
        if (p == 0u && lane == 0 && all_rows) atomicAdd(&ctr[1].num_heads, all_rows);
      }
      if (lane == 63) {
        wtot[wid] = inc;
        wflag[wid] = finc;
      }
      __syncthreads();
      uint32_t wb = 0, fb = 0, hbase = 0;
#pragma unroll
      for (uint32_t w = 0; w < (uint32_t)kWaves; ++w) {
        if (w < wid) {
          wb += wtot[w];
          fb += wflag[w];
        }
        hbase += pi == 0u ? wsum[w] : 0u;
      }
      const uint32_t start = wb + inc - all;
#pragma unroll
      for (int w = 0; w < kWaves; ++w) hist[w][tid] += start + before;
      __syncthreads();
      if (flag) heads[hbase + fb + finc - 1u] = base + start;
    }
#pragma unroll
    for (int b = 0; b < kBatches; ++b) {
      const bool valid = wlo + 64u * (uint32_t)b + lane < hi;
      const uint32_t d = k[b] % (uint32_t)kSlabVox;
      unsigned long long same = __ballot(valid);
#pragma unroll
      for (int bit = 0; bit < 9; ++bit) {
        const unsigned long long bb = __ballot((d >> bit) & 1u);
        same &= ((d >> bit) & 1u) ? bb : ~bb;
      }
      if (valid) {
        const uint32_t rank = (uint32_t)__popcll(same & ((1ull << lane) - 1ull));
        const uint32_t pos = hist[wid][d] + rank;
        ok[base + pos] = k[b];
        ov[base + pos] = v[b];
        if ((same >> lane) == 1ull) hist[wid][d] = pos + 1u;
      }
    }
    __syncthreads();
  }
}

template <typename Emit>
__device__ __forceinline__ uint32_t mask_spans(const uint32_t* m, Emit emit) {
  uint32_t n = 0;
  int start = -1;
  auto close = [&](uint32_t end) {
    uint32_t first = (uint32_t)start, len = end - first;
    for (; len > 128u; first += 128u, len -= 128u, ++n) emit(first, 128u);
    emit(first, len);
    ++n;
    start = -1;
  };
#pragma unroll
  for (int w = 0; w < kMaskWords; ++w) {
    const uint32_t bits = m[w];
    uint32_t pos = 0;
    while (pos < 32u) {
      if (start < 0) {
        const uint32_t rest = bits >> pos;
        if (rest == 0u) break;
        pos += (uint32_t)__ffs((int)rest) - 1u;
        start = w * 32 + (int)pos;
      } else {
        const uint32_t rest = ~bits >> pos;
        if (rest == 0u) break;
        pos += (uint32_t)__ffs((int)rest) - 1u;
        close((uint32_t)w * 32u + pos);
      }
    }
  }
  if (start >= 0) close((uint32_t)kMaskWords * 32u);
  return n;
}
struct RunSrc {
  const uint32_t* base;
  uint32_t words, r1_log2;
  TileMap tmap;
  const int32_t* offsets;
  int nclouds;
  const uint32_t* tile_first;
};
constexpr int kFoldGroup = 8;
constexpr int kFoldSteps = 256;
template <bool kGrid>
__global__ __launch_bounds__(64 * kFoldWaves) void fold_colours_masks(
    const uint32_t* __restrict__ skeys, const uint32_t* __restrict__ sorted_val, const uint32_t* __restrict__ nd_dev,
    RunSrc src, const uint32_t* __restrict__ vj0, const uint8_t* __restrict__ rgb, uint32_t* __restrict__ rgbw,
    const uint32_t* __restrict__ num_heads, uint32_t* __restrict__ sat_list, uint32_t* __restrict__ sat_count,
    const uint32_t* __restrict__ skip, const GridSrc grid) {
  if (skip != nullptr && *skip != 0u) return;
  __shared__ uint32_t stage[kFoldWaves][kFoldGroup][kFoldSteps];
  __shared__ float rcp[256];
  __shared__ uint32_t have[kFoldWaves][kFoldGroup];
  for (int k = threadIdx.x; k < 256; k += blockDim.x) rcp[k] = 1.f / (float)(1u + (uint32_t)k);
  __syncthreads();
  const int lane = threadIdx.x & 63, wid = threadIdx.x >> 6;
  const uint32_t nvox = *num_heads, nd = *nd_dev;
  const uint32_t ngroups = (nvox + kFoldGroup - 1) / kFoldGroup, nwaves = gridDim.x * kFoldWaves;
  for (uint32_t grp = blockIdx.x * kFoldWaves + wid; grp < ngroups; grp += nwaves) {
    const uint32_t v0 = grp * kFoldGroup, nv = min((uint32_t)kFoldGroup, nvox - v0);
    uint32_t my_j0 = nd, my_key = 0, my_col = 0xFF000000u;
    if ((uint32_t)lane < nv) {
      my_j0 = vj0[v0 + lane];
      my_key = skeys[my_j0];
      my_col = rgbw[my_key];
    }
    if constexpr (kGrid) {
      const int vl = lane >> 3, sub = lane & 7;
      const uint32_t j0v = (uint32_t)__shfl((int)my_j0, vl), keyv = (uint32_t)__shfl((int)my_key, vl);
      const uint32_t cwv = (uint32_t)__shfl((int)my_col, vl) >> 24;
      const uint32_t needv = cwv >= 254u ? 0u : 254u - cwv;
      uint32_t havev = 0, jn = j0v;
      bool open = (uint32_t)vl < nv && needv > 0u;
      const uint32_t gshift = 8u * (uint32_t)vl;
      auto run_tile = [&](uint32_t j) { return src.tmap.tile_of(sorted_val[j] >> src.r1_log2); };
      auto stage_row = [&](uint32_t bits, const GridTile& t, uint32_t w) {
        const uint32_t cnt = (uint32_t)__popc(bits);
        uint32_t inc = cnt;
#pragma unroll
        for (int d = 1; d < 8; d <<= 1) {
          const uint32_t up = (uint32_t)__shfl_up((int)inc, d, 8);
          if (sub >= d) inc += up;
        }
        uint32_t at = havev + inc - cnt;
        const uint32_t key0 = (t.cloud << grid.key_bits) | ((t.row0 + w) * grid.gw + t.col0);
        while (bits && at < needv) {
          const int bpos = __ffs((int)bits) - 1;
          bits &= bits - 1u;
          stage[wid][vl][at++] = key0 + (uint32_t)bpos;
        }
        havev += (uint32_t)__shfl((int)inc, 7, 8);
      };
      while (__any(open)) {
        const uint32_t j = jn + (uint32_t)sub;
        const uint32_t jc = min(j, nd - 1u), j8 = min(jn + 8u, nd - 1u);
        const uint32_t key_j = skeys[jc], val_j = sorted_val[jc], key_8 = skeys[j8], val_8 = sorted_val[j8];
        const bool mine = open && j < nd && key_j == keyv;
        const uint32_t val = mine ? val_j : 0u;
        const uint32_t gtile = mine ? src.tmap.tile_of(val >> src.r1_log2) : 0u;
        const uint32_t band = mine ? grid_band(grid, gtile) : 0xFFFFFFFFu;
        uint32_t band8 = 0xFFFFFFFEu;
        if (open && jn + 8u < nd && key_8 == keyv) band8 = grid_band(grid, src.tmap.tile_of(val_8 >> src.r1_log2));
        const uint32_t bprev = (uint32_t)__shfl_up((int)band, 1, 8);
        const bool start = mine && (sub == 0 || band != bprev);
        const uint32_t minem = (uint32_t)(__ballot(mine) >> gshift) & 0xFFu, startm = (uint32_t)(__ballot(start) >> gshift) & 0xFFu;
        const uint32_t nvalid = (uint32_t)__popc(minem);
        const bool tail_open = nvalid == 8u && band8 == (uint32_t)__shfl((int)band, 7, 8);
        uint32_t take = tail_open ? 31u - (uint32_t)__clz((int)startm) : nvalid;
        const uint32_t above = startm & ~((2u << sub) - 1u);
        const uint32_t nb = (above ? (uint32_t)__ffs((int)above) - 1u : nvalid) - (uint32_t)sub;
        const uint32_t bigm = (uint32_t)(__ballot(start && (uint32_t)sub < take && nb > 3u) >> gshift) & 0xFFu;
        if (bigm) take = min(take, (uint32_t)__ffs((int)bigm) - 1u);
        if (!open) {
        } else if (minem == 0u) {
          open = false;
        } else if (take > 0u) {
          const bool lead = start && (uint32_t)sub < take;
          const uint32_t val1 = (uint32_t)__shfl_down((int)val, 1, 8), val2 = (uint32_t)__shfl_down((int)val, 2, 8);
          const uint32_t gt1 = (uint32_t)__shfl_down((int)gtile, 1, 8), gt2 = (uint32_t)__shfl_down((int)gtile, 2, 8);
          uint32_t mA[kMaskWords], mB[kMaskWords], mC[kMaskWords];
#pragma unroll
          for (int w = 0; w < kMaskWords; ++w) mA[w] = mB[w] = mC[w] = 0u;
          auto load_mask = [&](uint32_t v, uint32_t* m) {
            const uint4* m4 = reinterpret_cast<const uint4*>(src.base + (size_t)v * src.words);
#pragma unroll
            for (int q = 0; q < kMaskWords / 4; ++q) {
              const uint4 a = m4[q];
              m[4 * q] = a.x; m[4 * q + 1] = a.y; m[4 * q + 2] = a.z; m[4 * q + 3] = a.w;
            }
          };
          if (lead) load_mask(val, mA);
          const bool wide = __any(lead && nb > 1u);
          if (wide) {
            if (lead && nb > 1u) load_mask(val1, mB);
            if (lead && nb > 2u) load_mask(val2, mC);
          }
          uint32_t cnt = 0;
#pragma unroll
          for (int w = 0; w < kMaskWords; ++w) cnt += (uint32_t)__popc(mA[w]);
          if (wide) {
#pragma unroll
            for (int w = 0; w < kMaskWords; ++w) cnt += (uint32_t)(__popc(mB[w]) + __popc(mC[w]));
          }
          uint32_t inc = cnt;
#pragma unroll
          for (int d = 1; d < 8; d <<= 1) {
            const uint32_t up = (uint32_t)__shfl_up((int)inc, d, 8);
            if (sub >= d) inc += up;
          }
          uint32_t at = havev + inc - cnt;
          const GridTile tA = grid_tile_of_band(grid, gtile, band);
          const uint32_t colB = (gt1 - band * grid.ntx) * (uint32_t)kGridTileW, colC = (gt2 - band * grid.ntx) * (uint32_t)kGridTileW;
          uint32_t rowkey = (tA.cloud << grid.key_bits) | (tA.row0 * grid.gw);
          auto put = [&](uint32_t bits, uint32_t key0) {
            while (bits && at < needv) {
              const int bpos = __ffs((int)bits) - 1;
              bits &= bits - 1u;
              stage[wid][vl][at++] = key0 + (uint32_t)bpos;
            }
          };
          if (wide) {
#pragma unroll
            for (int w = 0; w < kMaskWords; ++w) {
              put(mA[w], rowkey + tA.col0);
              put(mB[w], rowkey + colB);
              put(mC[w], rowkey + colC);
              rowkey += grid.gw;
            }
          } else {
#pragma unroll
            for (int w = 0; w < kMaskWords; ++w) {
              put(mA[w], rowkey + tA.col0);
              rowkey += grid.gw;
            }
          }
          havev += (uint32_t)__shfl((int)inc, 7, 8);
          jn += take;
          open = havev < needv && !(take == nvalid && nvalid < 8u);
        } else {
          const uint32_t band0 = (uint32_t)__shfl((int)band, 0, 8);
          uint32_t nbt = 0u;
          for (;; nbt += 8u) {
            const uint32_t jc = jn + nbt + (uint32_t)sub;
            const bool in = jc < nd && skeys[jc] == keyv && grid_band(grid, run_tile(jc)) == band0;
            const uint32_t cm = (uint32_t)(__ballot(in) >> gshift) & 0xFFu;
            if (cm != 0xFFu) {
              nbt += (uint32_t)__popc(cm);
              break;
            }
          }
          for (uint32_t w = 0; w < (uint32_t)kMaskWords && havev < needv; ++w)
            for (uint32_t c0 = 0; c0 < nbt; c0 += 8u) {
              const uint32_t jc = jn + c0 + (uint32_t)sub;
              GridTile t{0u, 0u, 0u};
              uint32_t bits = 0u;
              if (c0 + (uint32_t)sub < nbt) {
                t = grid_tile(grid, run_tile(jc));
                bits = src.base[(size_t)sorted_val[jc] * src.words + w];
              }
              stage_row(bits, t, w);
            }
          jn += nbt;
          open = havev < needv;
        }
      }
      if (sub == 0 && vl < kFoldGroup) have[wid][vl] = min(havev, needv);
    } else {
      const int vl = lane >> 3, sub = lane & 7;
      const uint32_t j0v = (uint32_t)__shfl((int)my_j0, vl), keyv = (uint32_t)__shfl((int)my_key, vl);
      const uint32_t cwv = (uint32_t)__shfl((int)my_col, vl) >> 24;
      const uint32_t needv = cwv >= 254u ? 0u : 254u - cwv;
      uint32_t havev = 0;
      bool open = (uint32_t)vl < nv && needv > 0u;
      for (uint32_t jb = 0; __any(open); jb += 8) {
        const uint32_t j = j0v + jb + (uint32_t)sub;
        const uint32_t jc = min(j, nd - 1u);
        const uint32_t key_j = skeys[jc], val_j = sorted_val[jc];
        const bool mine = open && j < nd && key_j == keyv;
        uint32_t m[kMaskWords];
#pragma unroll
        for (int w = 0; w < kMaskWords; ++w) m[w] = 0;
        size_t p0 = 0;
        uint32_t cnt = 0;
        uint32_t sp[kWireSpans];
#pragma unroll
        for (int q = 0; q < (int)kWireSpans; ++q) sp[q] = kSpanNone;
        const bool wire = src.words == kWireRun;
        if (mine) {
          const uint32_t val = val_j;
          const uint32_t* run = src.base + (size_t)val * src.words;
          uint32_t gt;
          if (wire) {
            const uint2 a = reinterpret_cast<const uint2*>(run)[1], c = reinterpret_cast<const uint2*>(run)[2];
            gt = a.x >> 12;
            sp[0] = a.y & 0xFFFFu; sp[1] = a.y >> 16; sp[2] = c.x & 0xFFFFu; sp[3] = c.x >> 16; sp[4] = c.y & 0xFFFFu; sp[5] = c.y >> 16;
#pragma unroll
            for (int q = 0; q < (int)kWireSpans; ++q) cnt += sp[q] == kSpanNone ? 0u : (sp[q] >> 9) + 1u;
          } else {
            const uint4* m4 = reinterpret_cast<const uint4*>(run);
#pragma unroll
            for (int q = 0; q < kMaskWords / 4; ++q) {
              const uint4 a = m4[q];
              m[4 * q] = a.x; m[4 * q + 1] = a.y; m[4 * q + 2] = a.z; m[4 * q + 3] = a.w;
            }
            gt = src.tmap.tile_of(val >> src.r1_log2);
#pragma unroll
            for (int w = 0; w < kMaskWords; ++w) cnt += (uint32_t)__popc(m[w]);
          }
          p0 = src.tile_first ? (size_t)src.tile_first[gt] : (size_t)tile_span(src.offsets, src.nclouds, gt, kWalkRays).first;
        }
        uint32_t inc = cnt;
#pragma unroll
        for (int d = 1; d < 8; d <<= 1) {
          const uint32_t up = (uint32_t)__shfl_up((int)inc, d, 8);
          if (sub >= d) inc += up;
        }
        uint32_t at = havev + inc - cnt;
        if (wire) {
#pragma unroll
          for (int q = 0; q < (int)kWireSpans; ++q) {
            if (sp[q] == kSpanNone) continue;
            const uint32_t first = sp[q] & 0x1FFu, len = (sp[q] >> 9) + 1u;
            for (uint32_t k = 0; k < len && at < needv; ++k) stage[wid][vl][at++] = (uint32_t)(p0 + (size_t)(first + k));
          }
        } else {
#pragma unroll
          for (int w = 0; w < kMaskWords; ++w) {
            uint32_t bits = m[w];
            while (bits && at < needv) {
              const int bpos = __ffs((int)bits) - 1;
              bits &= bits - 1u;
              stage[wid][vl][at++] = (uint32_t)(p0 + (size_t)(w * 32 + bpos));
            }
          }
        }
        havev += (uint32_t)__shfl((int)inc, 7, 8);
        const uint32_t group_mine = (uint32_t)(__ballot(mine) >> (8 * vl)) & 0xFFu;
        open = open && group_mine == 0xFFu && havev < needv;
      }
      if (sub == 0 && vl < kFoldGroup) have[wid][vl] = min(havev, needv);
    }
    __builtin_amdgcn_wave_barrier();
#pragma unroll
    for (int c = 0; c < kFoldGroup * kFoldSteps / 64 / 8; ++c) {
      uint32_t idx[8], colr[8];
      bool ok[8];
#pragma unroll
      for (int u = 0; u < 8; ++u) {
        const int i = c * 8 + u, v = (i * 64) / kFoldSteps, k = (i * 64) % kFoldSteps + lane;
        ok[u] = (uint32_t)k < have[wid][v];
        idx[u] = ok[u] ? stage[wid][v][k] : 0u;
      }
#pragma unroll
      for (int u = 0; u < 8; ++u) {
        colr[u] = 0;
        if (ok[u]) {
          const uint8_t* px;
          if constexpr (kGrid) {
            const uint32_t r = idx[u] & ((1u << grid.key_bits) - 1u), m = r / grid.gw, n = r - m * grid.gw;
            px = rgb + (size_t)(idx[u] >> grid.key_bits) * grid.bgr_image_stride + (size_t)(m * grid.step) * grid.bgr_pitch +
                 (size_t)(n * grid.step) * 3u;
          } else {
            px = rgb + 3 * (size_t)idx[u];
          }
          colr[u] = colour_roundtrip(px[0]) | (colour_roundtrip(px[1]) << 8) | (colour_roundtrip(px[2]) << 16);
        }
      }
#pragma unroll
      for (int u = 0; u < 8; ++u) {
        const int i = c * 8 + u, v = (i * 64) / kFoldSteps, k = (i * 64) % kFoldSteps + lane;
        if (ok[u]) stage[wid][v][k] = colr[u];
      }
    }
    __builtin_amdgcn_wave_barrier();
    {
      const int fv = lane >> 2, fc = lane & 3;
      const uint32_t col0 = (uint32_t)__shfl((int)my_col, fv);
      const uint32_t key = (uint32_t)__shfl((int)my_key, fv);
      const bool active = (uint32_t)fv < nv && fv < kFoldGroup;
      const uint32_t cw0 = col0 >> 24;
      const uint32_t steps = (active && cw0 < 254u) ? min(have[wid][fv & (kFoldGroup - 1)], 254u - cw0) : 0u;
      uint32_t ch = (col0 >> (8 * fc)) & 255u;
      if (fc < 3) {
        for (uint32_t k = 0; k < steps; ++k) {
          const uint32_t cw = cw0 + k;
          const uint32_t x = (stage[wid][fv & (kFoldGroup - 1)][k] >> (8 * fc)) & 255u;
          ch = (uint32_t)(uint8_t)((float)(cw * ch + x) * rcp[cw]);
        }
      }
      const uint32_t g = (uint32_t)__shfl_down((int)ch, 1), bl = (uint32_t)__shfl_down((int)ch, 2);
      if (active && fc == 0 && cw0 < 254u) {
        rgbw[key] = ch | (g << 8) | (bl << 16) | ((cw0 + steps) << 24);
        if (sat_list && cw0 + steps >= 254u) sat_list[atomicAdd(sat_count, 1u)] = key;
      }
    }
    __builtin_amdgcn_wave_barrier();
  }
}

}
```

Measured before the change: 88520 Mvoxels/s.

## Pass per-voxel run counts and keys to colour fold, skip sorted key writes

The parts_place stage now records, for each voxel head, its run count and voxel key, and in the depth-image path it no longer writes the sorted key array. The fold kernel then bounds each voxel's run by its count instead of comparing sorted keys, and prefetches a sliding window of sorted values (lo/hi/next) that is rotated with lane shuffles. Separately, the grid colour gather replaces three byte loads with one unaligned 4-byte load per pixel. These aim to cut global memory traffic in the fold and placement stages. The cost is two extra head-sized buffers, more register pressure, and a 4-byte read that starts one byte before the pixel; profiling hooks and a debug export are also added.

```diff
diff --git a/include/plvs_hip.h b/include/plvs_hip.h
--- a/include/plvs_hip.h
+++ b/include/plvs_hip.h
@@ -403,6 +403,8 @@
   int32_t max_run;
 } plvs_tsdf_stats;
 int plvs_hip_tsdf_chisel_last_stats(plvs_tsdf_chisel* h, plvs_tsdf_stats* s);
+int plvs_hip_tsdf_chisel_debug_fold_heads(plvs_tsdf_chisel* h, uint32_t* first, uint32_t* count, uint32_t* key, int cap, int* n_heads,
+                                          uint32_t* slots, int slots_cap, int* n_runs, int* tile_shift);
 
 int plvs_hip_tsdf_chisel_set_apply_parts(plvs_tsdf_chisel* h, int part_segments, int min_segments);
 
diff --git a/plvs_amd/csrc/tsdf_chisel.hip b/plvs_amd/csrc/tsdf_chisel.hip
--- a/plvs_amd/csrc/tsdf_chisel.hip
+++ b/plvs_amd/csrc/tsdf_chisel.hip
@@ -139,6 +139,14 @@
   if (reset) {
     unsigned long long z[16] = {};
     PLVS_HIP_TRY(hipMemcpyToSymbol(HIP_SYMBOL(g_walk_prof), z, sizeof z));
+  }
+  return PLVS_OK;
+}
+int plvs_hip_debug_fold_prof(unsigned long long* out40, int reset) {
+  if (out40) PLVS_HIP_TRY(hipMemcpyFromSymbol(out40, HIP_SYMBOL(g_fold_prof), 40 * sizeof(unsigned long long)));
+  if (reset) {
+    unsigned long long z[40] = {};
+    PLVS_HIP_TRY(hipMemcpyToSymbol(HIP_SYMBOL(g_fold_prof), z, sizeof z));
   }
   return PLVS_OK;
 }
@@ -286,7 +294,7 @@
   if (h->ev_zero) (void)hipEventDestroy(h->ev_zero);
   h->w_rseg.release(); h->w_rpre.release(); h->w_run_matrix.release(); h->w_active_idx.release(); h->w_item_base.release();
   h->w_item_cnt.release(); h->w_item_part0.release(); h->w_part_item.release(); h->w_phist.release();
-  h->w_row_heads.release(); h->w_row_tot.release();
+  h->w_row_heads.release(); h->w_row_tot.release(); h->w_head_cnt.release(); h->w_head_key.release();
   if (h->side) (void)hipStreamDestroy(h->side);
   for (int i = 0; i <= kNumStages; ++i)
     if (h->ev[i]) (void)hipEventDestroy(h->ev[i]);
@@ -647,6 +655,32 @@
   return PLVS_OK;
 }
 
+int plvs_hip_tsdf_chisel_debug_fold_heads(plvs_tsdf_chisel* h, uint32_t* first, uint32_t* count, uint32_t* key, int cap, int* n_heads,
+                                          uint32_t* slots, int slots_cap, int* n_runs, int* tile_shift) {
+  PLVS_FLUSH_QUEUE(h);
+  PLVS_REQUIRE(h && n_heads && n_runs && tile_shift, "null argument");
+  *n_heads = -1;
+  *n_runs = 0;
+  *tile_shift = (int)h->run_r1_log2;
+  if (h->last_chain != 2 || h->last_chain_skipped || !h->last_fold_counted) return PLVS_OK;
+  PLVS_HIP_TRY(hipDeviceSynchronize());
+  WalkCounters side;
+  PLVS_HIP_TRY(hipMemcpy(&side, h->d_wctr + 1, sizeof side, hipMemcpyDeviceToHost));
+  *n_heads = (int)side.num_heads;
+  *n_runs = (int)side.num_desc;
+  if (first && count && key && cap >= *n_heads && *n_heads > 0) {
+    PLVS_REQUIRE((size_t)*n_heads <= h->w_head_cnt.cap, "head list longer than its buffers");
+    PLVS_HIP_TRY(hipMemcpy(first, h->heads.p, (size_t)*n_heads * sizeof(uint32_t), hipMemcpyDeviceToHost));
+    PLVS_HIP_TRY(hipMemcpy(count, h->w_head_cnt.p, (size_t)*n_heads * sizeof(uint32_t), hipMemcpyDeviceToHost));
+    PLVS_HIP_TRY(hipMemcpy(key, h->w_head_key.p, (size_t)*n_heads * sizeof(uint32_t), hipMemcpyDeviceToHost));
+  }
+  if (slots && slots_cap >= *n_runs && *n_runs > 0) {
+    PLVS_REQUIRE((size_t)*n_runs <= h->w_val1.cap, "more runs than the slot buffer holds");
+    PLVS_HIP_TRY(hipMemcpy(slots, h->w_val1.p, (size_t)*n_runs * sizeof(uint32_t), hipMemcpyDeviceToHost));
+  }
+  return PLVS_OK;
+}
+
 int plvs_hip_tsdf_chisel_num_chunks(plvs_tsdf_chisel* h, int* n) {
   PLVS_FLUSH_QUEUE(h);
   PLVS_REQUIRE(h && n, "null argument");
diff --git a/plvs_amd/csrc/tsdf_chisel_handle.hpp b/plvs_amd/csrc/tsdf_chisel_handle.hpp
--- a/plvs_amd/csrc/tsdf_chisel_handle.hpp
+++ b/plvs_amd/csrc/tsdf_chisel_handle.hpp
@@ -121,10 +121,12 @@
   DevBuf<uint32_t> w_seg_ticket;
   DevBuf<uint4> w_rseg, w_rpre;
   DevBuf<uint32_t> w_run_matrix, w_active_idx, w_item_base, w_item_cnt, w_item_part0, w_part_item, w_phist, w_row_heads, w_row_tot;
+  DevBuf<uint32_t> w_head_cnt, w_head_key;
   hipEvent_t ev_zero = nullptr;
   hipEvent_t ev_seg = nullptr;
   int last_chain = 0;
   bool last_chain_skipped = false;
+  bool last_fold_counted = false;
   DevBuf<uint32_t> w_chunk_nseg, w_chunk_off, w_chunk_fill, w_active_off, w_masks, w_dummy, w_seg_cnt, w_tile_visits, w_deferred;
   DevBuf<uint32_t> w_part_off, w_multi_idx;
   DevBuf<long long> pa_wuu;
diff --git a/plvs_amd/csrc/tsdf_chisel_order_free.hpp b/plvs_amd/csrc/tsdf_chisel_order_free.hpp
--- a/plvs_amd/csrc/tsdf_chisel_order_free.hpp
+++ b/plvs_amd/csrc/tsdf_chisel_order_free.hpp
@@ -253,13 +253,15 @@
 }
 
 static int launch_fold(plvs_tsdf_chisel* h, const WalkCall& c, uint32_t D, const uint32_t* skeys, const uint32_t* sval,
-                       const uint32_t* skip, hipStream_t q) {
+                       const uint32_t* skip, hipStream_t q, const uint32_t* vcnt = nullptr, const uint32_t* vkey = nullptr) {
   const RunSrc rsrc{h->w_masks.p, (uint32_t)kMaskWords, h->run_r1_log2, TileMap{1u, 0u}, h->offsets.p, c.nclouds,
                     reinterpret_cast<const uint32_t*>(h->offsets.p) + 2 * ((size_t)c.nclouds + 1)};
-  const auto kernel = c.gsrc ? fold_colours_masks<true> : fold_colours_masks<false>;
+  const bool counted = vcnt != nullptr && vkey != nullptr;
+  PLVS_REQUIRE(counted ? c.gsrc != nullptr : skeys != nullptr, "fold: run counts without a depth-image call, or no keys");
+  const auto kernel = counted ? fold_colours_masks<true, true> : (c.gsrc ? fold_colours_masks<true> : fold_colours_masks<false>);
   hipLaunchKernelGGL(kernel, dim3(std::min<size_t>(ceil_div(D, kFoldWaves), 8192)), dim3(64 * kFoldWaves), 0, q, skeys, sval,
                      &h->d_wctr[1].num_desc, rsrc, h->heads.p, c.d_rgb, h->rgbw, &h->d_wctr[1].num_heads, (uint32_t*)nullptr,
-                     (uint32_t*)nullptr, skip, c.gsrc ? *c.gsrc : GridSrc{});
+                     (uint32_t*)nullptr, skip, c.gsrc ? *c.gsrc : GridSrc{}, vcnt, vkey);
   PLVS_KERNEL_CHECK();
   return PLVS_OK;
 }
@@ -310,6 +312,8 @@
 
 static int collect_chain(plvs_tsdf_chisel* h, const WalkPlan& plan, const WalkCall& c, uint32_t D, hipStream_t q) {
   const uint32_t rows = plan.collect_rows, blocks = plan.collect_blocks;
+  const bool counted = c.gsrc != nullptr;
+  h->last_fold_counted = counted;
   PLVS_HIP_TRY(hipStreamWaitEvent(q, h->ev_seg, 0));
   hipLaunchKernelGGL(runs_scatter, dim3(blocks * (kSegSpan / 256)), dim3(256), 0, q, h->w_seg.p, h->w_rseg.p, c.ntiles, h->w_seg_cnt.p,
                      h->w_active_idx.p, rows, blocks, h->w_run_matrix.p, h->w_rpre.p, h->w_item_base.p, h->d_wctr, h->w_val0.p);
@@ -319,9 +323,10 @@
   hipLaunchKernelGGL(rows_heads, dim3(std::min<uint32_t>(ceil_div(rows, 4), 1024u)), dim3(256), 0, q, h->w_item_part0.p,
                      h->w_item_cnt.p, h->w_phist.p, h->d_wctr, rows, h->w_row_heads.p, h->w_row_tot.p);
   hipLaunchKernelGGL(parts_place, dim3(part_grid), dim3(512), 0, q, h->w_part_item.p, h->w_item_part0.p, h->w_item_base.p,
-                     h->w_item_cnt.p, h->w_phist.p, h->d_wctr, h->dkey0.p, h->w_val0.p, h->dkey1.p, h->w_val1.p, h->heads.p,
-                     h->w_row_heads.p, rows, h->w_row_tot.p);
-  return launch_fold(h, c, D, h->dkey1.p, h->w_val1.p, &h->d_wctr[1].skip, q);
+                     h->w_item_cnt.p, h->w_phist.p, h->d_wctr, h->dkey0.p, h->w_val0.p, counted ? (uint32_t*)nullptr : h->dkey1.p,
+                     h->w_val1.p, h->heads.p, h->w_head_cnt.p, h->w_head_key.p, h->updated.p, h->w_row_heads.p, rows, h->w_row_tot.p);
+  if (!counted) return launch_fold(h, c, D, h->dkey1.p, h->w_val1.p, &h->d_wctr[1].skip, q);
+  return launch_fold(h, c, D, nullptr, h->w_val1.p, &h->d_wctr[1].skip, q, h->w_head_cnt.p, h->w_head_key.p);
 }
 
 static int reserve_collect(plvs_tsdf_chisel* h, const WalkPlan& plan, const WalkScratch& w, int max_chunks) {
@@ -340,6 +345,8 @@
   PLVS_HIP_TRY(h->w_val0.reserve(plan.collect_bound));
   PLVS_HIP_TRY(h->w_val1.reserve(plan.collect_bound));
   PLVS_HIP_TRY(h->heads.reserve(plan.collect_bound));
+  PLVS_HIP_TRY(h->w_head_cnt.reserve(plan.collect_bound));
+  PLVS_HIP_TRY(h->w_head_key.reserve(plan.collect_bound));
   PLVS_HIP_TRY(h->w_part_item.reserve(plan.parts_cap));
   PLVS_HIP_TRY(h->w_phist.reserve(plan.parts_cap * kSlabVox));
   PLVS_HIP_TRY(hipMemsetAsync(h->w_run_matrix.p, 0, (size_t)rows * plan.collect_blocks * sizeof(uint32_t), h->side));
diff --git a/plvs_amd/csrc/tsdf_chisel_shard.hpp b/plvs_amd/csrc/tsdf_chisel_shard.hpp
--- a/plvs_amd/csrc/tsdf_chisel_shard.hpp
+++ b/plvs_amd/csrc/tsdf_chisel_shard.hpp
@@ -313,7 +313,7 @@
                      skeys, sval, &h->d_wctr[1].num_desc,
                      RunSrc{runs, kWireRun, 0u, TileMap{1u, 0u}, h->offsets.p, h->sh_nclouds, nullptr}, h->heads.p, c.d_rgb,
                      h->rgbw, &h->d_wctr[1].num_heads, h->sh_sat.p, reinterpret_cast<uint32_t*>(h->d_xcount + 2),
-                     (const uint32_t*)nullptr, GridSrc{});
+                     (const uint32_t*)nullptr, GridSrc{}, (const uint32_t*)nullptr, (const uint32_t*)nullptr);
   PLVS_KERNEL_CHECK();
   return PLVS_OK;
 }
diff --git a/plvs_amd/csrc/tsdf_fold_window.hpp b/plvs_amd/csrc/tsdf_fold_window.hpp
--- /dev/null
+++ b/plvs_amd/csrc/tsdf_fold_window.hpp
@@ -0,0 +1,27 @@
+#pragma once
+
+#include <cstdint>
+
+#if defined(__HIPCC__)
+#define PLVS_FOLD_FN __host__ __device__ __forceinline__
+#else
+#define PLVS_FOLD_FN inline
+#endif
+
+namespace plvs {
+namespace tsdf {
+
+constexpr uint32_t kFoldLanes = 8;
+
+PLVS_FOLD_FN uint32_t fold_window_index(uint32_t jn, uint32_t ahead, uint32_t sub, uint32_t end) {
+  const uint32_t d = ahead + sub;
+  return d < end - jn ? jn + d : end - 1u;
+}
+PLVS_FOLD_FN uint32_t fold_window_valid(uint32_t jn, uint32_t end) {
+  return jn >= end ? 0u : (end - jn < kFoldLanes ? end - jn : kFoldLanes);
+}
+PLVS_FOLD_FN uint32_t fold_window_src_lane(uint32_t take, uint32_t sub) { return (take + sub) & (kFoldLanes - 1u); }
+PLVS_FOLD_FN bool fold_window_src_upper(uint32_t take, uint32_t sub) { return take + sub >= kFoldLanes; }
+
+}
+}
diff --git a/plvs_amd/csrc/tsdf_walk.hpp b/plvs_amd/csrc/tsdf_walk.hpp
--- a/plvs_amd/csrc/tsdf_walk.hpp
+++ b/plvs_amd/csrc/tsdf_walk.hpp
@@ -6,6 +6,7 @@
 #include "tsdf_chisel_core.hpp"
 #include "tsdf_directory.hpp"
 #include "tsdf_tiles.hpp"
+#include "tsdf_fold_window.hpp"
 #include "tsdf_walk_table.hpp"
 
 namespace {
@@ -21,6 +22,10 @@
 using plvs::tsdf::kErrPoolFull;
 using plvs::tsdf::home_bucket;
 using plvs::tsdf::next_bucket;
+using plvs::tsdf::fold_window_index;
+using plvs::tsdf::fold_window_src_lane;
+using plvs::tsdf::fold_window_src_upper;
+using plvs::tsdf::fold_window_valid;
 
 constexpr int kWalkRays = 512;
 constexpr int kMaskWords = kWalkRays / 32;
@@ -2401,8 +2406,9 @@
                                                    const uint32_t* __restrict__ item_base, const uint32_t* __restrict__ item_cnt,
                                                    const uint32_t* __restrict__ phist, WalkCounters* __restrict__ ctr,
                                                    const uint32_t* __restrict__ tk, const uint32_t* __restrict__ tv,
-                                                   uint32_t* __restrict__ ok, uint32_t* __restrict__ ov,
-                                                   uint32_t* __restrict__ heads, const uint32_t* __restrict__ row_heads,
+                                                   uint32_t* __restrict__ ok, uint32_t* __restrict__ ov, uint32_t* __restrict__ heads,
+                                                   uint32_t* __restrict__ head_cnt, uint32_t* __restrict__ head_key,
+                                                   const uint32_t* __restrict__ active, const uint32_t* __restrict__ row_heads,
                                                    uint32_t rows_cap, const uint32_t* __restrict__ row_tot) {
   constexpr int kWaves = 8, kBatches = kCollectPart / (64 * kWaves);
   __shared__ uint32_t hist[kWaves][kSlabVox];
@@ -2471,7 +2477,12 @@
 #pragma unroll
       for (int w = 0; w < kWaves; ++w) hist[w][tid] += start + before;
       __syncthreads();
-      if (flag) heads[hbase + fb + finc - 1u] = base + start;
+      if (flag) {
+        const uint32_t hd = hbase + fb + finc - 1u;
+        heads[hd] = base + start;
+        head_cnt[hd] = all;
+        head_key[hd] = active[row / (uint32_t)kSlabs] * (uint32_t)kChunkVox + (row % (uint32_t)kSlabs) * (uint32_t)kSlabVox + tid;
+      }
     }
 #pragma unroll
     for (int b = 0; b < kBatches; ++b) {
@@ -2486,7 +2497,7 @@
       if (valid) {
         const uint32_t rank = (uint32_t)__popcll(same & ((1ull << lane) - 1ull));
         const uint32_t pos = hist[wid][d] + rank;
-        ok[base + pos] = k[b];
+        if (ok != nullptr) ok[base + pos] = k[b];
         ov[base + pos] = v[b];
         if ((same >> lane) == 1ull) hist[wid][d] = pos + 1u;
       }
@@ -2535,14 +2546,42 @@
   int nclouds;
   const uint32_t* tile_first;
 };
+#ifdef PLVS_WALK_PROF
+__device__ unsigned long long g_fold_prof[40];
+#define FOLD_PROF_BEGIN() long long fp_t = 0; unsigned long long fp_acc[4] = {0, 0, 0, 0}; uint32_t fp_rounds = 0
+#define FOLD_PROF_GROUP() do { fp_t = (long long)clock64(); fp_rounds = 0; } while (0)
+#define FOLD_PROF(k) do { const long long now = (long long)clock64(); fp_acc[k] += (unsigned long long)(now - fp_t); fp_t = now; } while (0)
+#define FOLD_PROF_ROUND() ++fp_rounds
+#define FOLD_PROF_TASK()                                                     \
+  do {                                                                       \
+    if (kGrid && lane == 0) {                                                \
+      atomicAdd(&g_fold_prof[4], 1ull);                                      \
+      atomicAdd(&g_fold_prof[5], (unsigned long long)fp_rounds);             \
+      atomicAdd(&g_fold_prof[8 + min(fp_rounds, 31u)], 1ull);                \
+    }                                                                        \
+  } while (0)
+#define FOLD_PROF_END()                                                      \
+  do {                                                                       \
+    if (kGrid && lane == 0)                                                  \
+      for (int k = 0; k < 4; ++k) atomicAdd(&g_fold_prof[k], fp_acc[k]);     \
+  } while (0)
+#else
+#define FOLD_PROF_BEGIN() do {} while (0)
+#define FOLD_PROF_GROUP() do {} while (0)
+#define FOLD_PROF(k) do {} while (0)
+#define FOLD_PROF_ROUND() do {} while (0)
+#define FOLD_PROF_TASK() do {} while (0)
+#define FOLD_PROF_END() do {} while (0)
+#endif
 constexpr int kFoldGroup = 8;
 constexpr int kFoldSteps = 256;
-template <bool kGrid>
+template <bool kGrid, bool kCounted = false>
 __global__ __launch_bounds__(64 * kFoldWaves) void fold_colours_masks(
     const uint32_t* __restrict__ skeys, const uint32_t* __restrict__ sorted_val, const uint32_t* __restrict__ nd_dev,
     RunSrc src, const uint32_t* __restrict__ vj0, const uint8_t* __restrict__ rgb, uint32_t* __restrict__ rgbw,
     const uint32_t* __restrict__ num_heads, uint32_t* __restrict__ sat_list, uint32_t* __restrict__ sat_count,
-    const uint32_t* __restrict__ skip, const GridSrc grid) {
+    const uint32_t* __restrict__ skip, const GridSrc grid, const uint32_t* __restrict__ vcnt, const uint32_t* __restrict__ vkey) {
+  static_assert(kGrid || !kCounted, "run counts come with the depth-image form only");
   if (skip != nullptr && *skip != 0u) return;
   __shared__ uint32_t stage[kFoldWaves][kFoldGroup][kFoldSteps];
   __shared__ float rcp[256];
@@ -2552,12 +2591,19 @@
   const int lane = threadIdx.x & 63, wid = threadIdx.x >> 6;
   const uint32_t nvox = *num_heads, nd = *nd_dev;
   const uint32_t ngroups = (nvox + kFoldGroup - 1) / kFoldGroup, nwaves = gridDim.x * kFoldWaves;
+  FOLD_PROF_BEGIN();
   for (uint32_t grp = blockIdx.x * kFoldWaves + wid; grp < ngroups; grp += nwaves) {
     const uint32_t v0 = grp * kFoldGroup, nv = min((uint32_t)kFoldGroup, nvox - v0);
-    uint32_t my_j0 = nd, my_key = 0, my_col = 0xFF000000u;
+    FOLD_PROF_GROUP();
+    uint32_t my_j0 = nd, my_key = 0, my_col = 0xFF000000u, my_cnt = 0;
     if ((uint32_t)lane < nv) {
       my_j0 = vj0[v0 + lane];
-      my_key = skeys[my_j0];
+      if constexpr (kCounted) {
+        my_cnt = vcnt[v0 + lane];
+        my_key = vkey[v0 + lane];
+      } else {
+        my_key = skeys[my_j0];
+      }
       my_col = rgbw[my_key];
     }
     if constexpr (kGrid) {
@@ -2568,6 +2614,16 @@
       uint32_t havev = 0, jn = j0v;
       bool open = (uint32_t)vl < nv && needv > 0u;
       const uint32_t gshift = 8u * (uint32_t)vl;
+      const uint32_t endv = kCounted ? j0v + (uint32_t)__shfl((int)my_cnt, vl) : 0u;
+      uint32_t lo = 0u, hi = 0u;
+      if constexpr (kCounted) {
+        open = open && endv > j0v;
+        if (open) {
+          lo = sorted_val[fold_window_index(jn, 0u, (uint32_t)sub, endv)];
+          hi = sorted_val[fold_window_index(jn, 8u, (uint32_t)sub, endv)];
+        }
+      }
+      FOLD_PROF(0);
       auto run_tile = [&](uint32_t j) { return src.tmap.tile_of(sorted_val[j] >> src.r1_log2); };
       auto stage_row = [&](uint32_t bits, const GridTile& t, uint32_t w) {
         const uint32_t cnt = (uint32_t)__popc(bits);
@@ -2588,14 +2644,28 @@
       };
       while (__any(open)) {
         const uint32_t j = jn + (uint32_t)sub;
-        const uint32_t jc = min(j, nd - 1u), j8 = min(jn + 8u, nd - 1u);
-        const uint32_t key_j = skeys[jc], val_j = sorted_val[jc], key_8 = skeys[j8], val_8 = sorted_val[j8];
-        const bool mine = open && j < nd && key_j == keyv;
+        FOLD_PROF_ROUND();
+        bool mine, more8;
+        uint32_t val_j, val_8, nx = 0u;
+        if constexpr (kCounted) {
+          if (open) nx = sorted_val[fold_window_index(jn, 16u, (uint32_t)sub, endv)];
+          mine = open && j < endv;
+          more8 = open && jn + 8u < endv;
+          val_j = lo;
+          val_8 = (uint32_t)__shfl((int)hi, 0, 8);
+        } else {
+          const uint32_t jc = min(j, nd - 1u), j8 = min(jn + 8u, nd - 1u);
+          const uint32_t key_j = skeys[jc], key_8 = skeys[j8];
+          val_j = sorted_val[jc];
+          val_8 = sorted_val[j8];
+          mine = open && j < nd && key_j == keyv;
+          more8 = open && jn + 8u < nd && key_8 == keyv;
+        }
         const uint32_t val = mine ? val_j : 0u;
         const uint32_t gtile = mine ? src.tmap.tile_of(val >> src.r1_log2) : 0u;
         const uint32_t band = mine ? grid_band(grid, gtile) : 0xFFFFFFFFu;
         uint32_t band8 = 0xFFFFFFFEu;
-        if (open && jn + 8u < nd && key_8 == keyv) band8 = grid_band(grid, src.tmap.tile_of(val_8 >> src.r1_log2));
+        if (more8) band8 = grid_band(grid, src.tmap.tile_of(val_8 >> src.r1_log2));
         const uint32_t bprev = (uint32_t)__shfl_up((int)band, 1, 8);
         const bool start = mine && (sub == 0 || band != bprev);
         const uint32_t minem = (uint32_t)(__ballot(mine) >> gshift) & 0xFFu, startm = (uint32_t)(__ballot(start) >> gshift) & 0xFFu;
@@ -2670,14 +2740,22 @@
             }
           }
           havev += (uint32_t)__shfl((int)inc, 7, 8);
+          if constexpr (kCounted) {
+            const int from = (int)fold_window_src_lane(take, (uint32_t)sub);
+            const uint32_t a = (uint32_t)__shfl((int)lo, from, 8), b = (uint32_t)__shfl((int)hi, from, 8);
+            const uint32_t c = (uint32_t)__shfl((int)nx, from, 8);
+            const bool upper = fold_window_src_upper(take, (uint32_t)sub);
+            lo = upper ? b : a;
+            hi = upper ? c : b;
+          }
           jn += take;
-          open = havev < needv && !(take == nvalid && nvalid < 8u);
+          open = kCounted ? havev < needv && jn < endv : havev < needv && !(take == nvalid && nvalid < 8u);
         } else {
           const uint32_t band0 = (uint32_t)__shfl((int)band, 0, 8);
           uint32_t nbt = 0u;
           for (;; nbt += 8u) {
             const uint32_t jc = jn + nbt + (uint32_t)sub;
-            const bool in = jc < nd && skeys[jc] == keyv && grid_band(grid, run_tile(jc)) == band0;
+            const bool in = (kCounted ? jc < endv : jc < nd && skeys[jc] == keyv) && grid_band(grid, run_tile(jc)) == band0;
             const uint32_t cm = (uint32_t)(__ballot(in) >> gshift) & 0xFFu;
             if (cm != 0xFFu) {
               nbt += (uint32_t)__popc(cm);
@@ -2697,8 +2775,16 @@
             }
           jn += nbt;
           open = havev < needv;
-        }
-      }
+          if constexpr (kCounted) {
+            open = open && jn < endv;
+            if (open) {
+              lo = sorted_val[fold_window_index(jn, 0u, (uint32_t)sub, endv)];
+              hi = sorted_val[fold_window_index(jn, 8u, (uint32_t)sub, endv)];
+            }
+          }
+        }
+      }
+      FOLD_PROF(1);
       if (sub == 0 && vl < kFoldGroup) have[wid][vl] = min(havev, needv);
     } else {
       const int vl = lane >> 3, sub = lane & 7;
@@ -2778,7 +2864,7 @@
     __builtin_amdgcn_wave_barrier();
 #pragma unroll
     for (int c = 0; c < kFoldGroup * kFoldSteps / 64 / 8; ++c) {
-      uint32_t idx[8], colr[8];
+      uint32_t idx[8], colr[8] = {0u, 0u, 0u, 0u, 0u, 0u, 0u, 0u};
       bool ok[8];
 #pragma unroll
       for (int u = 0; u < 8; ++u) {
@@ -2786,19 +2872,40 @@
         ok[u] = (uint32_t)k < have[wid][v];
         idx[u] = ok[u] ? stage[wid][v][k] : 0u;
       }
-#pragma unroll
-      for (int u = 0; u < 8; ++u) {
-        colr[u] = 0;
-        if (ok[u]) {
-          const uint8_t* px;
-          if constexpr (kGrid) {
+      if constexpr (kGrid) {
+        const bool any_ok = ok[0] || ok[1] || ok[2] || ok[3] || ok[4] || ok[5] || ok[6] || ok[7];
+        if (__any(any_ok)) {
+          const bool words = grid.gw > 1u;
+          uint32_t raw[8], back[8];
+          const uint8_t* px[8];
+#pragma unroll
+          for (int u = 0; u < 8; ++u) {
             const uint32_t r = idx[u] & ((1u << grid.key_bits) - 1u), m = r / grid.gw, n = r - m * grid.gw;
-            px = rgb + (size_t)(idx[u] >> grid.key_bits) * grid.bgr_image_stride + (size_t)(m * grid.step) * grid.bgr_pitch +
-                 (size_t)(n * grid.step) * 3u;
+            back[u] = (words && n != 0u) ? 1u : 0u;
+            px[u] = rgb + (size_t)(idx[u] >> grid.key_bits) * grid.bgr_image_stride + (size_t)(m * grid.step) * grid.bgr_pitch +
+                    (size_t)(n * grid.step) * 3u - back[u];
+          }
+          if (words) {
+#pragma unroll
+            for (int u = 0; u < 8; ++u) __builtin_memcpy(&raw[u], px[u], 4);
           } else {
-            px = rgb + 3 * (size_t)idx[u];
+#pragma unroll
+            for (int u = 0; u < 8; ++u) raw[u] = (uint32_t)px[u][0] | ((uint32_t)px[u][1] << 8) | ((uint32_t)px[u][2] << 16);
           }
-          colr[u] = colour_roundtrip(px[0]) | (colour_roundtrip(px[1]) << 8) | (colour_roundtrip(px[2]) << 16);
+#pragma unroll
+          for (int u = 0; u < 8; ++u) {
+            const uint32_t w = raw[u] >> (8u * back[u]);
+            colr[u] = colour_roundtrip(w & 255u) | (colour_roundtrip((w >> 8) & 255u) << 8) | (colour_roundtrip((w >> 16) & 255u) << 16);
+          }
+        }
+      } else {
+#pragma unroll
+        for (int u = 0; u < 8; ++u) {
+          colr[u] = 0;
+          if (ok[u]) {
+            const uint8_t* px = rgb + 3 * (size_t)idx[u];
+            colr[u] = colour_roundtrip(px[0]) | (colour_roundtrip(px[1]) << 8) | (colour_roundtrip(px[2]) << 16);
+          }
         }
       }
 #pragma unroll
@@ -2808,6 +2915,7 @@
       }
     }
     __builtin_amdgcn_wave_barrier();
+    FOLD_PROF(2);
     {
       const int fv = lane >> 2, fc = lane & 3;
       const uint32_t col0 = (uint32_t)__shfl((int)my_col, fv);
@@ -2830,7 +2938,10 @@
       }
     }
     __builtin_amdgcn_wave_barrier();
-  }
-}
-
-}
+    FOLD_PROF(3);
+    FOLD_PROF_TASK();
+  }
+  FOLD_PROF_END();
+}
+
+}
```

After: 87520 Mvoxels/s. -1.1%, worse.
